# lucidrains/phenaki-pytorch

Measured on AMD Instinct MI355X. Metric: cvivit_encode_frames_per_sec, higher is better.
Workload: dtype bf16; 1 GPU; BASELINE configs[1]: C-ViViT (dim 512, patch 32, tpatch 2, depth 4+4, LFQ 65536) encode video -> token ids, (8,3,17,256,256) f32 per GPU resident in HBM; global_batch=8, parallelism=batch-shard x1, no data-path collective, hip_graph=True

## Files before the change

### include/phenaki_hip.h

```cpp
#ifndef PHENAKI_HIP_H
#define PHENAKI_HIP_H

#ifdef __cplusplus
extern "C" {
#endif

#define PK_OK 0
#define PK_EINVAL (-1)
#define PK_EALIGN (-2)
#define PK_ELAUNCH (-3)

int pk_gemm(int dtype, int a_is_f32, const void* A, int lda, const void* W, int ldw, int M, int N, int K,
            const float* bias, const float* res, int ldr, void* C, int ldc, int out_is_f32, int act,
            const int* a_rows, void* stream);

int pk_gemm_ex(int dtype, int a_is_f32, const void* A, int lda, const void* W, int ldw, int M, int N, int K,
               const float* bias, const float* res, int ldr, void* C, int ldc, int out_is_f32, int act,
               const int* a_rows, int a_nrows, int variant, void* C2, int ldc2, const float* ln_s, const float* ln_t,
               float ln_eps, const int* row_off, const int* col_off, float* stats_out, const float* ln_stats, int dup_rows,
               void* stream);
int pk_gemm_auto_variant(int dtype, int a_is_f32, int M, int N, int K, int lda, int ldw, int a_nrows);

int pk_layernorm(const float* x, int ldx, const float* gamma, const float* beta, float eps, void* out, int ldo,
                 int out_kind, float* out2, int ldo2, void* raw, int ldraw, int M, int D, int grp, int gstride,
// ... 160 lines not shown
    const float* src; void* out; long long lds, ldo; int R, K, Kp, flags, tile0, tiles_x;
} PkPackJob;
int pk_pack_multi(const void* jobs, int count, void* stream);
int pk_pack_table_prepare(void* jobs, int count);
int pk_pack_table(const void* dev_table, int count, int tiles, void* stream);
int pk_scatter_rows(const float* src, long long lds, const int* rows, float* dst, long long ldd, int M, int D, void* stream);
int pk_colsum_parts(int M);
int pk_colsum(const float* src, long long ld, int M, int N, float scale, float* out, int accumulate, float* work, void* stream);
int pk_ln_bwd_parts(int M);
int pk_layernorm_bwd(const float* x, long long ldx, const float* gamma, const float* dy, long long lddy, const float* add, long long ldadd,
                     float* dx, long long lddx, float* pg, float* pb, float eps, int M, int D, void* stream);
int pk_geglu(const float* h, long long ldh, int goff, float* out, long long ldo, int M, int F, const pk_dropout* drop, void* stream);
int pk_geglu_bwd(const float* h, long long ldh, int goff, const float* dout, long long ldd, float* dh, long long lddh, int M, int F, const pk_dropout* drop,
                 void* stream);
int pk_dropout_mask(unsigned long long seed, unsigned long long offset, int keep_thr, long long rows, int cols, unsigned char* out, void* stream);
int pk_scaled_diff(const float* a, const float* b, float scale, const float* scale_dev, float* out, long long n, void* stream);
int pk_sign(const float* z, float value, float* out, long long n, void* stream);
int pk_mul(const float* a, const float* b, float* out, long long n, void* stream);
int pk_leaky_bwd(const float* y, long long ldy, const float* dy, long long lddy, float* dz, long long lddz, int M, int N, float slope, void* stream);
int pk_peg_adjoint(const float* dy, const float* wt, float* dx, int B, int T, int H, int W, int D, int causal, void* stream);
int pk_peg_wgrad_parts(long long rows);
int pk_peg_bwd(const float* dy, const float* x, const float* wt, float* dx, float* part, int B, int T, int H, int W, int D, int causal, void* stream);
int pk_embed_bwd(const float* dy, const long long* ids, float alpha, float* dtok, float* dpos, int S, int n, int D, void* stream);
int pk_bias_gather(const float* tab, int ldt, const int* code, int off, float* out, int heads, int n, void* stream);
int pk_bias_scatter(const float* dbias, const int* code, int off, float* dtab, int ldt, int heads, int n, void* stream);
int pk_sum_batch(const float* src, long long stride, int S, float* out, long long E, void* stream);
typedef struct PkColsumJob { const float* src; float* out; long long ld; int M, N, blk0; float scale; } PkColsumJob;
int pk_colsum_multi(const void* jobs, int count, void* stream);
int pk_reduce_multi(const void* sum_jobs, int nsum, const void* col_jobs, int ncol, void* stream);
typedef struct PkSumJob { const float* src; float* out; long long stride, E4; int S, blk0; } PkSumJob;
int pk_sum_batch_multi(const void* jobs, int count, void* stream);
int pk_bce_head(const float* e, long long lde, const float* w, const float* b, const float* labels, float scale, const float* scale_dev, float* logits, float* loss_rows,
                float* de, long long ldde, float* pw, float* pb, int M, int D, void* stream);
int pk_gemm_splitk(int dtype, const void* A, int lda, const void* W, int ldw, int M, int N, int K, int splits, float* C, int ldc,
                   const float* bias, int tile, void* stream);
int pk_adamw(float* p, const float* g, float* m, float* v, float lr, float beta1, float beta2, float eps, float wd, int step, long long n, void* stream);
int pk_adamw_multi(const long long* table, int count, float lr, float beta1, float beta2, float eps, float wd, int step, void* stream);
int pk_grad_sumsq_parts(const long long* table, int count);
int pk_grad_sumsq(const long long* table, int count, float* partials, long long nparts, void* stream);
int pk_grad_clip_coef(const float* partials, long long nparts, float max_norm, float* out, void* stream);
int pk_scale_multi(const long long* table, int count, const float* coef_dev, void* stream);
int pk_adamw_multi_scaled(const long long* table, int count, float lr, float beta1, float beta2, float eps, float wd, int step,
                          const float* gscale_dev, void* stream);
int pk_ema_multi(const long long* table, int count, float weight, void* stream);
int pk_attn_train_prep(const float* q, long long ldq, const float* kv, long long ldkv, const float* null_kv, const float* q_scale, const float* k_scale,
                       float scale, float* Qh, float* Kh, float* Vh, int S, int heads, int n, int n_kv, int nnull, void* stream);
int pk_attn_train_prep_bwd(const float* q, long long ldq, const float* kv, long long ldkv, const float* null_kv, const float* q_scale, const float* k_scale,
                           float scale, const float* dQh, const float* dKh, const float* dVh, float* dq, long long lddq, float* dkv, long long lddkv,
                           float* pq, float* pk, float* dnull, int S, int heads, int n, int n_kv, int nnull, void* stream);
int pk_attn_bwd_work(int S, int heads, int n, int n_kv, int nnull);
int pk_attn_bwd_ws(const float* Qh, const float* Kh, const float* Vh, const void* O, long long ldo, int o_bf16, const float* dO, long long lddo,
                   const float* bias, const unsigned char* kmask, const float* slopes, int causal, float* dQh, float* dKh, float* dVh, float* dS,
                   float* lse, float* Drow, int S, int heads, int n, int n_kv, int nnull, int split_bf16, float* work, long long work_floats,
                   const pk_dropout* drop, void* stream);

int pk_im2col(const float* x, int B, int H, int W, int C, int kh, int kw, int stride, int pad, float* cols, long long ldc, void* stream);
int pk_col2im(const float* cols, long long ldc, int B, int H, int W, int C, int kh, int kw, int stride, int pad, float* dx, void* stream);
int pk_nchw_to_rows(const float* img, int B, int C, int H, int W, int Cp, float* rows, void* stream);
int pk_rows_to_nchw(const float* rows, int B, int C, int H, int W, int Cp, float* img, void* stream);
int pk_pick_frames(float* video, const int* frame, int B, int C, int F, int H, int W, float* img, int place, void* stream);
int pk_bmm(const float* A, long long lda, long long sA, int tA, const float* B, long long ldb, long long sB, int tB, float* C, long long ldc,
           long long sC, int batch, int M, int N, int K, int accumulate, void* stream);
int pk_row_softmax(const float* a, const float* b, const float* c, float* out, long long M, int n, int mode, void* stream);
int pk_row_l2scale(const float* x, const float* sc, const float* dz, const float* gx, const float* gsc, float* o0, float* o1, float* o2,
                   long long M, int d, int mode, void* stream);
int pk_row_ln_bwd2(const float* x, const float* gamma, const float* dy, const float* u, const float* w, float eps, float* grad_x,
                   float* grad_gamma_rows, float* grad_dy, long long M, int D, void* stream);

int pk_conv3x3(int dtype, int a_is_f32, const void* x, int B, int H, int W, int C, const void* Wm, int ldw, int Co, const float* bias, int act,
               const void* gate, int ldg, int gate_is_f32, void* y, int ldy, int out_is_f32, int tile, void* stream);
int pk_maxpool2x2(int is_f32, const void* x, int B, int H, int W, int C, void* y, void* stream);
int pk_maxpool2x2_bwd(int is_f32, const void* x, const float* dy, int B, int H, int W, int C, float* dx, void* stream);
int pk_adaptive_avgpool(int is_f32, const void* x, int B, int H, int W, int C, float* out, void* stream);
int pk_adaptive_avgpool_bwd(const float* dy, int B, int H, int W, int C, float* dx, void* stream);

int pk_frame_sqerr_parts(int H, int W);
int pk_frame_ssim_parts(int H, int W);
int pk_frame_sqerr(const float* a, const float* b, int B, int C, int F, int H, int W, float clamp_hi, float data_range, double* partials,
                   long long nparts, float* mse, float* psnr, void* stream);
int pk_frame_ssim(const float* a, const float* b, int B, int C, int F, int H, int W, float clamp_hi, float data_range, double* partials,
                  long long nparts, float* ssim, void* stream);
int pk_code_usage(const int* counts, int V, double* out, void* stream);

#ifdef __cplusplus
}
#endif
#endif
```

### phenaki_pytorch_amd/_lib.py

```python
import ctypes
import os

import torch

_HERE = os.path.dirname(os.path.abspath(__file__))
LIB_PATH = os.environ.get('PK_LIB_PATH') or os.path.join(_HERE, 'libphenaki_hip.so')

_P = ctypes.c_void_p
_I = ctypes.c_int
_F = ctypes.c_float
_L = ctypes.c_long
_LL = ctypes.c_longlong
_ULL = ctypes.c_ulonglong

SIGNATURES = {
    'pk_gemm': [_I, _I, _P, _I, _P, _I, _I, _I, _I, _P, _P, _I, _P, _I, _I, _I, _P, _P],
    'pk_gemm_ex': [_I, _I, _P, _I, _P, _I, _I, _I, _I, _P, _P, _I, _P, _I, _I, _I, _P, _I, _I, _P, _I, _P, _P, _F, _P, _P, _P, _P, _I, _P],
    'pk_gemm_auto_variant': [_I, _I, _I, _I, _I, _I, _I, _I],
    'pk_layernorm': [_P, _I, _P, _P, _F, _P, _I, _I, _P, _I, _P, _I, _I, _I, _I, _I, _I, _I, _I, _P],
    'pk_rmsnorm': [_P, _I, _P, _F, _P, _P, _I, _I, _I, _I, _P],
    'pk_gated_gelu_tanh': [_P, _I, _P, _I, _I, _I, _I, _P],
    'pk_l2norm_rows': [_P, _I, _P, _I, _I, _I, _I, _P],
    'pk_patchify_ln': [_P, _I, _I, _I, _I, _I, _I, _I, _I, _I, _I, _P, _P, _F, _P, _I, _I, _P],
    'pk_patch_embed': [_P, _I, _I, _I, _I, _I, _I, _I, _I, _F, _I,
# ... 32 lines not shown
    'pk_cpb_input': [_P, _P, _P, _I, _I, _I, _I, _I, _P],
    'pk_attn_pads': [_I, _I, _I, ctypes.POINTER(_I), ctypes.POINTER(_I)],
    'pk_attn_prep': [_I, _P, _I, _P, _I, _P, _P, _P, _F, _P, _P, _P, _I, _I, _I, _I, _I, _P],
    'pk_attn_prep_dh': [_I, _I, _P, _I, _P, _I, _P, _P, _P, _F, _P, _P, _P, _I, _I, _I, _I, _I, _P],
    'pk_qkv_project': [_I, _P, _P, _I, _P, _P, _I, _I, _I, _I, _I, _P, _P, _F, _P, _P, _P, _I, _I, _P, _P],
    'pk_qkv_attn': [_I, _P, _P, _I, _P, _P, _I, _I, _I, _I, _I, _P, _P, _F, _P, _L, _I, _P, _I, _P, _I, _P, _P],
    'pk_q_attn_cached': [_I, _P, _I, _P, _I, _I, _I, _I, _I, _P, _F, _P, _P, _P, _I, _I, _I, _P, _P, _I, _P],
    'pk_attn_fwd': [_I, _P, _P, _P, _P, _L, _I, _P, _P, _I, _P, _I, _I, _I, _I, _I, _I, _I, _P, _I, _P, _I, _I, _F, _P],
    'pk_attn_fwd_dh': [_I, _I, _P, _P, _P, _P, _L, _I, _P, _P, _I, _P, _I, _I, _I, _I, _I, _I, _I, _P, _I, _P, _I, _I, _F, _P],
    'pk_attn_fwd_lse': [_I, _P, _P, _P, _P, _L, _I, _P, _P, _I, _P, _I, _I, _I, _I, _I, _I, _I, _P, _P, _P],
    'pk_attn_fwd_lse_dh': [_I, _I, _P, _P, _P, _P, _L, _I, _P, _P, _I, _P, _I, _I, _I, _I, _I, _I, _I, _P, _P, _P],
    'pk_attn_small': [_P, _I, _P, _I, _P, _P, _F, _P, _L, _I, _P, _P, _I, _P, _I, _I, _I, _I, _I, _P],
    'pk_cfg_mix': [_P, _I, _I, _I, _I, _P, _I, _F, _I, _P, _I, _I, _I, _P],
    'pk_vocab_ntiles': [_I],
    'pk_vocab_sample_philox': [_I, _P, _I, _P, _I, _P, _I, _I, _I, _F, _P, _ULL, _ULL, ctypes.c_uint, _I, _P, _P],
    'pk_vocab_sample': [_I, _P, _I, _P, _I, _P, _I, _I, _I, _F, _P, _P, _ULL, _P, _I, _P, _P],
    'pk_vocab_reduce': [_P, _I, _I, _P, _P, _P, _P, _P, _I, _P],
    'pk_vocab_ce': [_I, _P, _I, _I, _P, _I, _P, _I, _P, _I, _P, _P, _P, _P, _P],
    'pk_vocab_eval_words': [_I],
    'pk_vocab_eval': [_I, _P, _I, _P, _I, _P, _I, _I, _I, _P, _P, _P, _P],
    'pk_vocab_eval_reduce': [_P, _I, _I, _P, _P, _P, _P, _P, _P],
    'pk_ce_grad_slab': [_I, _P, _I, _P, _P, _P, _I, _I, _I, _F, _P, _P, _I, _P, _I, _P, _P],
    'pk_topk_mask': [_P, _I, _I, _I, _LL, _P, _P, _P, _P, _P],
    'pk_critic_head': [_P, _I, _P, _P, _I, _I, _I, _I, _I, _F, _P, _F, _ULL, _P, _P, _P],
    'pk_pack': [_P, _LL, _P, _I, _I, _I, _P, _LL, _I, _I, _P],
    'pk_scatter_rows': [_P, _LL, _P, _P, _LL, _I, _I, _P],
    'pk_colsum_parts': [_I],
    'pk_colsum': [_P, _LL, _I, _I, _F, _P, _I, _P, _P],
    'pk_ln_bwd_parts': [_I],
    'pk_layernorm_bwd': [_P, _LL, _P, _P, _LL, _P, _LL, _P, _LL, _P, _P, _F, _I, _I, _P],
    'pk_geglu': [_P, _LL, _I, _P, _LL, _I, _I, _P, _P],
    'pk_geglu_bwd': [_P, _LL, _I, _P, _LL, _P, _LL, _I, _I, _P, _P],
    'pk_dropout_mask': [_ULL, _ULL, _I, _LL, _I, _P, _P],
    'pk_leaky_bwd': [_P, _LL, _P, _LL, _P, _LL, _I, _I, _F, _P],
    'pk_scaled_diff': [_P, _P, _F, _P, _P, _LL, _P],
    'pk_sign': [_P, _F, _P, _LL, _P],
    'pk_mul': [_P, _P, _P, _LL, _P],
    'pk_peg_wgrad_parts': [_LL],
    'pk_peg_bwd': [_P, _P, _P, _P, _P, _I, _I, _I, _I, _I, _I, _P],
    'pk_embed_bwd': [_P, _P, _F, _P, _P, _I, _I, _I, _P],
    'pk_bias_gather': [_P, _I, _P, _I, _P, _I, _I, _P],
    'pk_bias_scatter': [_P, _P, _I, _P, _I, _I, _I, _P],
    'pk_sum_batch': [_P, _LL, _I, _P, _LL, _P],
    'pk_sum_batch_multi': [_P, _I, _P],
    'pk_peg_adjoint': [_P, _P, _P, _I, _I, _I, _I, _I, _I, _P],
    'pk_colsum_multi': [_P, _I, _P],
    'pk_reduce_multi': [_P, _I, _P, _I, _P],
    'pk_pack_multi': [_P, _I, _P],
    'pk_pack_table_prepare': [_P, _I],
    'pk_pack_table': [_P, _I, _I, _P],
    'pk_bce_head': [_P, _LL, _P, _P, _P, _F, _P, _P, _P, _P, _LL, _P, _P, _I, _I, _P],
    'pk_attn_train_prep': [_P, _LL, _P, _LL, _P, _P, _P, _F, _P, _P, _P, _I, _I, _I, _I, _I, _P],
    'pk_attn_train_prep_bwd': [_P, _LL, _P, _LL, _P, _P, _P, _F, _P, _P, _P, _P, _LL, _P, _LL, _P, _P, _P, _I, _I, _I, _I, _I, _P],
    'pk_gemm_splitk': [_I, _P, _I, _P, _I, _I, _I, _I, _I, _P, _I, _P, _I, _P],
    'pk_adamw': [_P, _P, _P, _P, _F, _F, _F, _F, _F, _I, _LL, _P],
    'pk_adamw_multi': [_P, _I, _F, _F, _F, _F, _F, _I, _P],
    'pk_grad_sumsq_parts': [_P, _I],
    'pk_grad_sumsq': [_P, _I, _P, _LL, _P],
    'pk_grad_clip_coef': [_P, _LL, _F, _P, _P],
    'pk_scale_multi': [_P, _I, _P, _P],
    'pk_adamw_multi_scaled': [_P, _I, _F, _F, _F, _F, _F, _I, _P, _P],
    'pk_ema_multi': [_P, _I, _F, _P],
    'pk_attn_bwd_ws': [_P, _P, _P, _P, _LL, _I, _P, _LL, _P, _P, _P, _I, _P, _P, _P, _P, _P, _P, _I, _I, _I, _I, _I, _I, _P, _LL, _P, _P],
    'pk_attn_bwd_work': [_I, _I, _I, _I, _I],
    'pk_im2col': [_P, _I, _I, _I, _I, _I, _I, _I, _I, _P, _LL, _P],
    'pk_col2im': [_P, _LL, _I, _I, _I, _I, _I, _I, _I, _I, _P, _P],
    'pk_nchw_to_rows': [_P, _I, _I, _I, _I, _I, _P, _P],
    'pk_rows_to_nchw': [_P, _I, _I, _I, _I, _I, _P, _P],
    'pk_pick_frames': [_P, _P, _I, _I, _I, _I, _I, _P, _I, _P],
    'pk_bmm': [_P, _LL, _LL, _I, _P, _LL, _LL, _I, _P, _LL, _LL, _I, _I, _I, _I, _I, _P],
    'pk_row_softmax': [_P, _P, _P, _P, _LL, _I, _I, _P],
    'pk_row_l2scale': [_P, _P, _P, _P, _P, _P, _P, _P, _LL, _I, _I, _P],
    'pk_row_ln_bwd2': [_P, _P, _P, _P, _P, _F, _P, _P, _P, _LL, _I, _P],
    'pk_conv3x3': [_I, _I, _P, _I, _I, _I, _I, _P, _I, _I, _P, _I, _P, _I, _I, _P, _I, _I, _I, _P],
    'pk_maxpool2x2': [_I, _P, _I, _I, _I, _I, _P, _P],
    'pk_maxpool2x2_bwd': [_I, _P, _P, _I, _I, _I, _I, _P, _P],
    'pk_adaptive_avgpool': [_I, _P, _I, _I, _I, _I, _P, _P],
    'pk_adaptive_avgpool_bwd': [_P, _I, _I, _I, _I, _P, _P],
    'pk_frame_sqerr_parts': [_I, _I],
    'pk_frame_ssim_parts': [_I, _I],
    'pk_frame_sqerr': [_P, _P, _I, _I, _I, _I, _I, _F, _F, _P, _LL, _P, _P, _P],
    'pk_frame_ssim': [_P, _P, _I, _I, _I, _I, _I, _F, _F, _P, _LL, _P, _P],
    'pk_code_usage': [_P, _I, _P, _P],
}

_ERR = {-1: 'PK_EINVAL (bad shape/size/flag)', -2: 'PK_EALIGN (pointer/stride alignment)', -3: 'PK_ELAUNCH (HIP launch failed)'}

_lib = None


def load():
    global _lib
    if _lib is None:
        if not os.path.exists(LIB_PATH):
            raise RuntimeError(f'{LIB_PATH} is missing: run `python -m phenaki_pytorch_amd.build` '
                               '(the MI355X build has no CPU / eager fallback)')
        lib = ctypes.CDLL(LIB_PATH)
        for name, args in SIGNATURES.items():
            fn = getattr(lib, name)
            fn.argtypes = args
            fn.restype = _I
        _lib = lib
    return _lib


def _check(rc, name):
    if rc != 0:
        raise RuntimeError(f'{name} failed: {_ERR.get(rc, rc)}')


def ptr(t):
    return None if t is None else t.data_ptr()


def f32p(t, name='parameter', rows_ok=False):
    if t is None:
        return None
    if t.dtype != torch.float32 or not (t.is_contiguous() or (rows_ok and t.stride(-1) == 1)):
        raise RuntimeError(f'{name}: the MI355X kernels read this tensor as contiguous float32, got {t.dtype} '
                           f'{"contiguous" if t.is_contiguous() else "strided"} (keep the module in float32; the compute '
                           'precision is chosen with set_compute_dtype, not with .half()/.bfloat16())')
    return t.data_ptr()


def stream(t=None):
    if t is None:
        return torch.cuda.current_stream().cuda_stream
    idx = t.device.index
    cur = _current_device()
    if idx is not None and idx != cur:
        raise RuntimeError(f'operand on cuda:{idx} but the current device is cuda:{cur}: '
                           'call torch.cuda.set_device(...) first (one process per GPU)')
    return _raw_stream(cur)


_raw_stream = getattr(torch._C, '_cuda_getCurrentRawStream', None) or (lambda i: torch.cuda.current_stream(i).cuda_stream)
_current_device = getattr(torch._C, '_cuda_getDevice', None) or torch.cuda.current_device


def require_device(t, name='tensor'):
    if not t.is_cuda:
        raise RuntimeError(f'{name} is on {t.device}: the MI355X build runs on HIP devices only (no CPU fallback)')


F32, BF16, BF16X3 = 0, 1, 2
ACT_NONE, ACT_GEGLU, ACT_LEAKY, ACT_RELU = 0, 1, 2, 3


def tdtype(dtype):
    return torch.bfloat16 if dtype == BF16 else torch.float32


def split_planes(w32):
    n, k = w32.shape
    assert k % 32 == 0 and w32.dtype == torch.float32
    hi = w32.to(torch.bfloat16)
    lo = (w32 - hi.float()).to(torch.bfloat16)
    img = torch.cat((hi.view(n, k // 32, 32), lo.view(n, k // 32, 32)), dim=-1).contiguous()
    return img.view(n, 2 * k).view(torch.float32)



def gemm(dtype, A, W, M, N, K, *, C, bias=None, res=None, act=ACT_NONE, a_rows=None, lda=None, ldc=None, variant=0, C2=None, ln=None,
         scatter=None, stats_out=None, ln_stats=None, dup_rows=0):
    a_is_f32 = 1 if A.dtype == torch.float32 else 0
    out_is_f32 = 1 if C.dtype == torch.float32 else 0
    lda = A.stride(-2) if lda is None else lda
    ldc = (C.stride(-2) if scatter is None else N) if ldc is None else ldc
    ldr = res.stride(-2) if res is not None else 0
    rc = load().pk_gemm_ex(dtype, a_is_f32, ptr(A), lda, ptr(W), W.stride(0), M, N, K, f32p(bias, 'bias'), f32p(res, 'residual'), ldr,
                           ptr(C), ldc, out_is_f32, act, ptr(a_rows), A.shape[0] if a_rows is not None else M, variant,
                           ptr(C2), C2.stride(-2) if C2 is not None else 0, ptr(ln[0]) if ln else None, ptr(ln[1]) if ln else None,
                           float(ln[2]) if ln else 0., ptr(scatter[0]) if scatter else None, ptr(scatter[1]) if scatter else None,
                           ptr(stats_out) if stats_out is not None else None, ptr(ln_stats) if ln_stats is not None else None, int(dup_rows), stream(C))
    _check(rc, 'pk_gemm_ex')
    return C


def layernorm(x, gamma, beta, M, D, *, out=None, out2=None, raw=None, eps=1e-5, remap=(0, 0, 0), perm=(0, 0), ldx=None):
    tt = out if out is not None else raw
    out_kind = 1 if (tt is not None and tt.dtype == torch.bfloat16) else 0
    rc = load().pk_layernorm(f32p(x, 'x', rows_ok=True), x.stride(-2) if ldx is None else ldx, f32p(gamma, 'LayerNorm gamma'), f32p(beta, 'LayerNorm beta'), eps,
                             ptr(out), out.stride(-2) if out is not None else 0, out_kind,
                             ptr(out2), out2.stride(-2) if out2 is not None else 0,
                             ptr(raw), raw.stride(-2) if raw is not None else 0, M, D, *remap, *perm, stream(x))
    _check(rc, 'pk_layernorm')


def patchify_ln(video, f0, nt, pt, ph, pw, weight, bias, out, eps=1e-5):
    B, C, F, H, W = video.shape
    rc = load().pk_patchify_ln(f32p(video, 'video'), B, C, F, H, W, f0, nt, pt, ph, pw, f32p(weight, 'LayerNorm weight'), f32p(bias, 'LayerNorm bias'), eps,
                               ptr(out), out.stride(0), 1 if out.dtype == torch.bfloat16 else 0, stream(video))
    _check(rc, 'pk_patchify_ln')


def patch_embed(video, ph, pw, N, groups, eps=1e-5):
    B, C, F, H, W = video.shape
    flat = []
    for (Wg, s, t, out, f0, nt, pt) in groups:
        flat += [ptr(Wg), Wg.stride(0), f32p(s, 'folded s'), f32p(t, 'folded t'), ptr(out), f0, nt, pt]
    if len(groups) == 1:
        flat += [None, 0, None, None, None, 0, 0, 0]
    ldo = groups[0][3].stride(0)
    rc = load().pk_patch_embed(f32p(video, 'video'), B, C, F, H, W, ph, pw, N, eps, len(groups), *flat, ldo, stream(video))
    _check(rc, 'pk_patch_embed')


def patch_embed_slices(K):
    return load().pk_patch_embed_slices(int(K))


def patch_embed_splitk(video, ph, pw, N, groups):
    B, C, F, H, W = video.shape
    flat = []
    for (Wg, part, stats, f0, nt, pt) in groups:
        flat += [ptr(Wg), Wg.stride(0), ptr(part), ptr(stats), f0, nt, pt]
    if len(groups) == 1:
        flat += [None, 0, None, None, 0, 0, 0]
    rc = load().pk_patch_embed_splitk(f32p(video, 'video'), B, C, F, H, W, ph, pw, N, len(groups), *flat, stream(video))
    _check(rc, 'pk_patch_embed_splitk')


def patch_embed_finish(part, stats, K, s, t, eps1, gamma2, beta2, eps2, *, out2=None, out=None, remap=(0, 0, 0)):
    nslices, rows, N = part.shape
    rc = load().pk_patch_embed_finish(ptr(part), ptr(stats), nslices, rows, N, int(K), f32p(s, 'folded s'), f32p(t, 'folded t'), float(eps1),
                                      f32p(gamma2, 'LayerNorm weight'), f32p(beta2, 'LayerNorm bias'), float(eps2),
                                      ptr(out2), out2.stride(-2) if out2 is not None else 0, ptr(out), out.stride(-2) if out is not None else 0,
                                      *remap, stream(part))
    _check(rc, 'pk_patch_embed_finish')


class _PatchFinishGroup(ctypes.Structure):
    _fields_ = [('part', _P), ('stats', _P), ('nslices', _I), ('rows', _I), ('K', _I), ('s', _P), ('t', _P), ('eps1', _F), ('gamma2', _P), ('beta2', _P),
                ('eps2', _F), ('remap_in', _I), ('remap_out', _I), ('remap_off', _I)]


def patch_embed_finish_groups(groups, *, out2=None, out=None):
    arr = (_PatchFinishGroup * len(groups))()
    for d, (part, stats, K, s, t, eps1, gamma2, beta2, eps2, remap) in zip(arr, groups):
        nslices, rows, N = part.shape
        d.part, d.stats, d.nslices, d.rows, d.K = ptr(part), ptr(stats), nslices, rows, int(K)
        d.s, d.t, d.eps1 = f32p(s, 'folded s'), f32p(t, 'folded t'), float(eps1)
        d.gamma2, d.beta2, d.eps2 = f32p(gamma2, 'LayerNorm weight'), f32p(beta2, 'LayerNorm bias'), float(eps2)
# ... 850 lines not shown
```

### phenaki_pytorch_amd/csrc/common.hpp

```cpp
#pragma once
#include <hip/hip_runtime.h>
#include <stdint.h>

namespace pk {

typedef float f32x4 __attribute__((ext_vector_type(4)));
typedef float f32x2 __attribute__((ext_vector_type(2)));
typedef __bf16 bf16x8_t __attribute__((ext_vector_type(8)));
typedef unsigned short u16;
typedef u16 u16x8 __attribute__((ext_vector_type(8)));
typedef u16 u16x4 __attribute__((ext_vector_type(4)));
typedef uint32_t u32x4 __attribute__((ext_vector_type(4)));
typedef uint32_t u32x2 __attribute__((ext_vector_type(2)));

struct bf16 { u16 v; };

struct bf16x3 { float v; };
struct bf16x3p { uint32_t v; };

typedef __bf16 bf16x2_native __attribute__((ext_vector_type(2)));
__device__ __forceinline__ u16 f2bf(float f) {
    return __builtin_bit_cast(u16, (__bf16)f);
}
__device__ __forceinline__ float bf2f(u16 h) {
// ... 37 lines not shown
__device__ __forceinline__ void split8(const f32x4& a, const f32x4& b, u32x4& hi, u32x4& lo) {
    const float x[8] = {a[0], a[1], a[2], a[3], b[0], b[1], b[2], b[3]};
#pragma unroll
    for (int i = 0; i < 4; ++i) {
        const uint32_t h = pack_bf2(x[2 * i], x[2 * i + 1]);
        hi[i] = h;
        const float h0 = __builtin_bit_cast(float, h << 16), h1 = __builtin_bit_cast(float, h & 0xFFFF0000u);
        lo[i] = pack_bf2(x[2 * i] - h0, x[2 * i + 1] - h1);
    }
}

__device__ __forceinline__ void frag_load(Frag<bf16>& f, const bf16* p) {
    f.v = *reinterpret_cast<const u32x4*>(p);
}
__device__ __forceinline__ void frag_load(Frag<float>& f, const float* p) {
    f.lo = *reinterpret_cast<const f32x4*>(p);
    f.hi = *reinterpret_cast<const f32x4*>(p + 4);
}
__device__ __forceinline__ const char* split_block(const void* p, int& pos2) {
    const uintptr_t a = reinterpret_cast<uintptr_t>(p);
    pos2 = (int)(a & 127) >> 1;
    return reinterpret_cast<const char*>(a & ~(uintptr_t)127);
}
__device__ __forceinline__ void frag_load(Frag<bf16x3p>& f, const bf16x3p* p) {
    int o;
    const char* blk = split_block(p, o);
    f.hi = *reinterpret_cast<const u32x4*>(blk + o);
    f.lo = *reinterpret_cast<const u32x4*>(blk + 64 + o);
}
__device__ __forceinline__ void frag_zero(Frag<bf16x3p>& f) { f.hi = u32x4{0, 0, 0, 0}; f.lo = f.hi; }
__device__ __forceinline__ void frag_zero(Frag<bf16x3>& f) { f.hi = u32x4{0, 0, 0, 0}; f.lo = f.hi; }
__device__ __forceinline__ void frag_zero(Frag<bf16>& f) { f.v = u32x4{0, 0, 0, 0}; }
__device__ __forceinline__ void frag_zero(Frag<float>& f) { f.lo = f32x4{0, 0, 0, 0}; f.hi = f.lo; }

__device__ __forceinline__ void frag_from_f32(Frag<bf16>& f, const float (&x)[8]) {
    f.v = u32x4{pack_bf2(x[0], x[1]), pack_bf2(x[2], x[3]), pack_bf2(x[4], x[5]), pack_bf2(x[6], x[7])};
}
__device__ __forceinline__ void frag_from_f32(Frag<float>& f, const float (&x)[8]) {
    f.lo = f32x4{x[0], x[1], x[2], x[3]};
    f.hi = f32x4{x[4], x[5], x[6], x[7]};
}

__device__ __forceinline__ void frag_from_f32(Frag<bf16x3p>& f, const float (&x)[8]) {
    split8(f32x4{x[0], x[1], x[2], x[3]}, f32x4{x[4], x[5], x[6], x[7]}, f.hi, f.lo);
}
__device__ __forceinline__ void frag_from_f32(Frag<bf16x3>& f, const float (&x)[8]) {
    split8(f32x4{x[0], x[1], x[2], x[3]}, f32x4{x[4], x[5], x[6], x[7]}, f.hi, f.lo);
}

__device__ __forceinline__ void store_elem(float* p, float v) { *p = v; }
__device__ __forceinline__ void store_elem(bf16* p, float v) { p->v = f2bf(v); }
__device__ __forceinline__ float load_elem(const float* p) { return *p; }
__device__ __forceinline__ float load_elem(const bf16* p) { return bf2f(p->v); }

__device__ __forceinline__ void store_elem(bf16x3* p, float v) { p->v = v; }
__device__ __forceinline__ float load_elem(const bf16x3* p) { return p->v; }
__device__ __forceinline__ void store4(bf16x3* p, f32x4 v) { *reinterpret_cast<f32x4*>(p) = v; }
__device__ __forceinline__ void store2(bf16x3* p, float a, float b) { *reinterpret_cast<f32x2*>(p) = f32x2{a, b}; }
__device__ __forceinline__ void store4(bf16x3p* p, f32x4 v) {
    const uintptr_t a = reinterpret_cast<uintptr_t>(p);
    char* blk = reinterpret_cast<char*>(a & ~(uintptr_t)127);
    const int o = (int)(a & 127) >> 1;
    const uint32_t h0 = pack_bf2(v[0], v[1]), h1 = pack_bf2(v[2], v[3]);
    const float r0 = v[0] - __builtin_bit_cast(float, h0 << 16), r1 = v[1] - __builtin_bit_cast(float, h0 & 0xFFFF0000u);
    const float r2 = v[2] - __builtin_bit_cast(float, h1 << 16), r3 = v[3] - __builtin_bit_cast(float, h1 & 0xFFFF0000u);
    *reinterpret_cast<u32x2*>(blk + o) = u32x2{h0, h1};
    *reinterpret_cast<u32x2*>(blk + 64 + o) = u32x2{pack_bf2(r0, r1), pack_bf2(r2, r3)};
}
__device__ __forceinline__ void store_elem(bf16x3p* p, float v) {
    const uintptr_t a = reinterpret_cast<uintptr_t>(p);
    char* blk = reinterpret_cast<char*>(a & ~(uintptr_t)127);
    const int o = (int)(a & 127) >> 1;
    const u16 h = f2bf(v);
    *reinterpret_cast<u16*>(blk + o) = h;
    *reinterpret_cast<u16*>(blk + 64 + o) = f2bf(v - bf2f(h));
}
__device__ __forceinline__ void store4(float* p, f32x4 v) { *reinterpret_cast<f32x4*>(p) = v; }
__device__ __forceinline__ void store4(bf16* p, f32x4 v) {
    *reinterpret_cast<u32x2*>(p) = u32x2{pack_bf2(v[0], v[1]), pack_bf2(v[2], v[3])};
}
__device__ __forceinline__ void store2(float* p, float a, float b) { *reinterpret_cast<f32x2*>(p) = f32x2{a, b}; }
__device__ __forceinline__ void store2(bf16* p, float a, float b) { *reinterpret_cast<uint32_t*>(p) = pack_bf2(a, b); }

__device__ __forceinline__ long xcd_contiguous_block(unsigned b, unsigned nblocks_padded) {
    return (long)(b & 7u) * (nblocks_padded >> 3) + (b >> 3);
}
__host__ __device__ inline unsigned xcd_padded_grid(long nblocks) { return (unsigned)(8 * ((nblocks + 7) / 8)); }

__device__ __forceinline__ float mul_rn(float a, float b) {
#pragma clang fp contract(off)
    return a * b;
}
__device__ __forceinline__ float add_rn(float a, float b) {
#pragma clang fp contract(off)
    return a + b;
}
__device__ __forceinline__ float wave_sum(float v) {
#pragma unroll
    for (int o = 32; o > 0; o >>= 1) v += __shfl_xor(v, o, 64);
    return v;
}
__device__ __forceinline__ float wave_max(float v) {
#pragma unroll
    for (int o = 32; o > 0; o >>= 1) v = fmaxf(v, __shfl_xor(v, o, 64));
    return v;
}

__device__ __forceinline__ float gelu_erf(float x) { return 0.5f * x * (1.0f + erff(x * 0.70710678118654752440f)); }
__device__ __forceinline__ float gelu_erf_fast(float x) {
    const float z = fabsf(x) * 0.70710678118654752440f;
    const float t = __frcp_rn(fmaf(0.3275911f, z, 1.0f));
    float p = fmaf(1.061405429f, t, -1.453152027f);
    p = fmaf(p, t, 1.421413741f);
    p = fmaf(p, t, -0.284496736f);
    p = fmaf(p, t, 0.254829592f);
    const float erfz = fmaf(-p * t, __expf(-z * z), 1.0f);
    return 0.5f * x * (1.0f + copysignf(erfz, x));
}
template <typename T> __device__ __forceinline__ float gelu_for(float x);
template <> __device__ __forceinline__ float gelu_for<float>(float x) { return gelu_erf(x); }
template <> __device__ __forceinline__ float gelu_for<bf16>(float x) { return gelu_erf_fast(x); }
#ifdef PK_X3_EXACT_GELU
template <> __device__ __forceinline__ float gelu_for<bf16x3>(float x) { return gelu_erf(x); }
#else
template <> __device__ __forceinline__ float gelu_for<bf16x3>(float x) { return gelu_erf_fast(x); }
#endif

__device__ __host__ __forceinline__ uint32_t mix32(uint32_t h) {
    h ^= h >> 16; h *= 0x85ebca6bu; h ^= h >> 13; h *= 0xc2b2ae35u; h ^= h >> 16;
    return h;
}
__device__ __host__ __forceinline__ float uniform24(uint32_t seed_lo, uint32_t seed_hi, uint32_t idx_lo, uint32_t idx_hi) {
    uint32_t h = mix32(idx_lo ^ seed_lo);
    h = mix32(h + 0x9e3779b9u * (idx_hi + 1u) + seed_hi);
    return (float)(h >> 8) * (1.0f / 16777216.0f);
}

__device__ __host__ __forceinline__ void uniform24x4(uint32_t seed_lo, uint32_t seed_hi, uint32_t q_lo, uint32_t q_hi, float (&u)[4]) {
    uint32_t h = mix32(q_lo ^ seed_lo);
    h = h + 0x9e3779b9u * (q_hi + 1u) + seed_hi;
    const uint32_t w0 = mix32(h), w1 = mix32(h + 0x85EBCA77u), w2 = mix32(h + 0x0BD794EEu);
    const float k = 1.0f / 16777216.0f;
    u[0] = (float)(w0 >> 8) * k;
    u[1] = (float)(w1 >> 8) * k;
    u[2] = (float)(w2 >> 8) * k;
    u[3] = (float)(((w0 & 0xFFu) << 16) | ((w1 & 0xFFu) << 8) | (w2 & 0xFFu)) * k;
}

struct DropArgs { uint32_t k0, k1, thr; float scale; };
__device__ __host__ __forceinline__ DropArgs drop_keys(uint64_t seed, uint64_t offset, int thr, float scale) {
    DropArgs d;
    d.k0 = mix32((uint32_t)seed ^ mix32((uint32_t)offset + 0x9e3779b9u));
    d.k1 = mix32((uint32_t)(seed >> 32) + 0x85ebca6bu * ((uint32_t)(offset >> 32) + 1u) + d.k0);
    d.thr = (uint32_t)thr;
    d.scale = scale;
    return d;
}
struct pk_dropout { unsigned long long seed, offset; int keep_thr; float scale; };
inline bool drop_site_bad(const pk_dropout* d) { return d && (d->keep_thr < 1 || d->keep_thr > 256); }
inline DropArgs drop_keys(const pk_dropout& d) { return drop_keys(d.seed, d.offset, d.keep_thr, d.scale); }
template <bool DROP> struct DropParam {};
template <> struct DropParam<true> : DropArgs { __device__ __host__ DropParam(const DropArgs& d) : DropArgs(d) {} };
__device__ __host__ __forceinline__ uint32_t drop_row(const DropArgs& d, uint32_t row) { return mix32(row ^ d.k0); }
__device__ __host__ __forceinline__ uint32_t drop_word(const DropArgs& d, uint32_t rowh, uint32_t grp) { return mix32(rowh + 0x9e3779b9u * grp + d.k1); }
__device__ __host__ __forceinline__ bool drop_keep(const DropArgs& d, uint32_t word, int e) { return ((word >> (8 * e)) & 255u) >= d.thr; }

// ... 45 lines not shown
```

### phenaki_pytorch_amd/csrc/elementwise.hip

```cpp
#include "common.hpp"

namespace pk {

__global__ __launch_bounds__(256) void peg_kernel(const float* __restrict__ x, const float* __restrict__ wt,
                                                  const float* __restrict__ bias, float* __restrict__ out, bf16* __restrict__ out_t,
                                                  int B, int T, int H, int W, int D, int tfront, long total_vec) {
    const int dv = D >> 2;
    for (long idx = (long)blockIdx.x * 256 + threadIdx.x; idx < total_vec; idx += (long)gridDim.x * 256) {
        const int c = (int)(idx % dv) * 4;
        long p = idx / dv;
        const int w = (int)(p % W); p /= W;
        const int h = (int)(p % H); p /= H;
        const int t = (int)(p % T); const int b = (int)(p / T);
        f32x4 acc = *reinterpret_cast<const f32x4*>(bias + c);
        f32x4 center = f32x4{0, 0, 0, 0};
#pragma unroll
        for (int dt = 0; dt < 3; ++dt) {
            const int ts = t + dt - tfront;
            if (ts < 0 || ts >= T) continue;
#pragma unroll
            for (int dh = 0; dh < 3; ++dh) {
                const int hs = h + dh - 1;
                if (hs < 0 || hs >= H) continue;
#pragma unroll
                for (int dw = 0; dw < 3; ++dw) {
                    const int ws = w + dw - 1;
                    if (ws < 0 || ws >= W) continue;
                    const f32x4 xv = *reinterpret_cast<const f32x4*>(x + ((((size_t)b * T + ts) * H + hs) * W + ws) * D + c);
                    const f32x4 kv = *reinterpret_cast<const f32x4*>(wt + (size_t)((dt * 3 + dh) * 3 + dw) * D + c);
                    acc += xv * kv;
                    if (ts == t && hs == h && ws == w) center = xv;
                }
            }
        }
        const size_t o = ((((size_t)b * T + t) * H + h) * W + w) * D + c;
        *reinterpret_cast<f32x4*>(out + o) = acc + center;
        if (out_t) store4(out_t + o, acc + center);
    }
}

template <int WW>
__global__ __launch_bounds__(256) void peg_row_kernel(const float* __restrict__ x, const float* __restrict__ wt,
                                                      const float* __restrict__ bias, float* __restrict__ out, bf16* __restrict__ out_t,
                                                      int B, int T, int H, int D, int tfront, long total, int flip = 0) {
    const int dv = D >> 2;
    const long idx = xcd_contiguous_block(blockIdx.x, gridDim.x) * 256 + threadIdx.x;
    if (idx >= total) return;
    const int c = (int)(idx % dv) * 4;
    long p = idx / dv;
    const int h = (int)(p % H); p /= H;
    const int t = (int)(p % T); const int b = (int)(p / T);
    const f32x4 bv = bias ? *reinterpret_cast<const f32x4*>(bias + c) : f32x4{0.f, 0.f, 0.f, 0.f};
    f32x4 acc[WW];
#pragma unroll
    for (int w = 0; w < WW; ++w) acc[w] = bv;
#pragma unroll
    for (int dt = 0; dt < 3; ++dt) {
        const int ts = t + dt - tfront;
        if (ts < 0 || ts >= T) continue;
#pragma unroll
        for (int dh = 0; dh < 3; ++dh) {
            const int hs = h + dh - 1;
            if (hs < 0 || hs >= H) continue;
            const float* row = x + (((size_t)b * T + ts) * H + hs) * WW * D + c;
            f32x4 xr[WW];
#pragma unroll
            for (int w = 0; w < WW; ++w) xr[w] = *reinterpret_cast<const f32x4*>(row + (size_t)w * D);
            const int tb = (dt * 3 + dh) * 3;
            const f32x4 k0 = *reinterpret_cast<const f32x4*>(wt + (size_t)(flip ? 26 - tb : tb) * D + c);
            const f32x4 k1 = *reinterpret_cast<const f32x4*>(wt + (size_t)(flip ? 25 - tb : tb + 1) * D + c);
            const f32x4 k2 = *reinterpret_cast<const f32x4*>(wt + (size_t)(flip ? 24 - tb : tb + 2) * D + c);
#pragma unroll
            for (int w = 0; w < WW; ++w) {
                if (w > 0) acc[w] += xr[w - 1] * k0;
                acc[w] += xr[w] * k1;
                if (w + 1 < WW) acc[w] += xr[w + 1] * k2;
                if (dt == tfront && dh == 1) acc[w] += xr[w];
            }
        }
    }
    const size_t o0 = (((size_t)b * T + t) * H + h) * WW * D + c;
#pragma unroll
    for (int w = 0; w < WW; ++w) *reinterpret_cast<f32x4*>(out + o0 + (size_t)w * D) = acc[w];
    if (out_t) {
#pragma unroll
        for (int w = 0; w < WW; ++w) store4(out_t + o0 + (size_t)w * D, acc[w]);
    }
}

template <int CD>
__global__ __launch_bounds__(256) void lfq_encode_kernel(const float* __restrict__ x, int ldx, const float* __restrict__ wp,
                                                         const float* __restrict__ bp, long long* __restrict__ ids,
                                                         float* __restrict__ proj, int M, int D) {
    const int lane = threadIdx.x & 63;
    const int row = blockIdx.x * 4 + (threadIdx.x >> 6);
    if (row >= M) return;
    float part[CD];
#pragma unroll
    for (int k = 0; k < CD; ++k) part[k] = 0.f;
    const float* xr = x + (size_t)row * ldx;
    for (int c = lane * 4; c < D; c += 256) {
        const f32x4 xv = *reinterpret_cast<const f32x4*>(xr + c);
#pragma unroll
        for (int k = 0; k < CD; ++k) {
            const f32x4 wv = *reinterpret_cast<const f32x4*>(wp + (size_t)k * D + c);
            part[k] += (xv[0] * wv[0] + xv[1] * wv[1]) + (xv[2] * wv[2] + xv[3] * wv[3]);
        }
    }
    long long id = 0;
#pragma unroll
    for (int k = 0; k < CD; ++k) {
        const float v = wave_sum(part[k]) + bp[k];
        if (proj && lane == 0) proj[(size_t)row * CD + k] = v;
        id |= (long long)(v > 0.f ? 1 : 0) << (CD - 1 - k);
    }
    if (lane == 0) ids[row] = id;
}

__device__ __forceinline__ long long lfq_row_id(const long long* __restrict__ ids_prime, int n_prime, const long long* __restrict__ ids, int n, int row) {
    if (!ids_prime) return ids[row];
    const int n_tot = n_prime + n, b = row / n_tot, i = row - b * n_tot;
    return i < n_prime ? ids_prime[(size_t)b * n_prime + i] : ids[(size_t)b * n + (i - n_prime)];
}
__device__ __forceinline__ int lfq_out_row(int r, int pb, int pc) {
    if (pb <= 0) return r;
    const int c = r % pc, ab = r / pc, b = ab % pb, a = ab / pb;
    return (a * pc + c) * pb + b;
}

template <int CD>
__global__ __launch_bounds__(256) void lfq_decode_kernel(const long long* __restrict__ ids_prime, int n_prime, const long long* __restrict__ ids, int n,
                                                         const float* __restrict__ wo,
                                                         const float* __restrict__ bo, float* __restrict__ out,
                                                         int M, int D, int row_stride, int pb, int pc) {
    const int dv = D >> 2;
    const int lanes = blockDim.x;
    const int cg = threadIdx.x % dv, rl = threadIdx.x / dv;
    float w[4][CD];
    f32x4 b4 = *reinterpret_cast<const f32x4*>(bo + cg * 4);
    {
        const f32x4* src = reinterpret_cast<const f32x4*>(wo + (size_t)cg * 4 * CD);
#pragma unroll
        for (int q = 0; q < CD; ++q) {
            const f32x4 t = src[q];
#pragma unroll
            for (int r = 0; r < 4; ++r) w[(q * 4 + r) / CD][(q * 4 + r) % CD] = t[r];
        }
    }
    for (int row = blockIdx.x * (lanes / dv) + rl; row < M; row += row_stride) {
        const unsigned long long id = (unsigned long long)lfq_row_id(ids_prime, n_prime, ids, n, row);
        f32x4 acc = b4;
#pragma unroll
        for (int k = 0; k < CD; ++k) {
            const bool on = (id >> (CD - 1 - k)) & 1ull;
#pragma unroll
            for (int e = 0; e < 4; ++e) acc[e] += on ? w[e][k] : -w[e][k];
        }
        *reinterpret_cast<f32x4*>(out + (size_t)lfq_out_row(row, pb, pc) * D + cg * 4) = acc;
    }
}

__global__ __launch_bounds__(256) void lfq_decode_generic_kernel(const long long* __restrict__ ids_prime, int n_prime, const long long* __restrict__ ids, int n,
                                                                 const float* __restrict__ wo,
                                                                 const float* __restrict__ bo, float* __restrict__ out,
                                                                 int M, int D, int cd, int pb, int pc) {
    const long total = (long)M * D;
    for (long idx = (long)blockIdx.x * 256 + threadIdx.x; idx < total; idx += (long)gridDim.x * 256) {
        const int d = (int)(idx % D);
        const int row = (int)(idx / D);
        const long long id = lfq_row_id(ids_prime, n_prime, ids, n, row);
// ... 15 lines not shown
        const int c = (int)(idx % dv) * 4;
        const long r = idx / dv;
        const int i = (int)(r % n_tot);
        const int b = (int)((r / n_tot) % nb);
        const long long id = i < n_prime ? ids_prime[(size_t)b * n_prime + i] : ids[(size_t)b * n + (i - n_prime)];
        const f32x4 a = *reinterpret_cast<const f32x4*>(pos + (size_t)i * D + c);
        const f32x4 t = *reinterpret_cast<const f32x4*>(tok + (size_t)id * D + c);
        *reinterpret_cast<f32x4*>(out + (size_t)r * D + c) = a + t;
        if (out_t) store4(out_t + (size_t)r * D + c, a + t);
    }
}

__global__ __launch_bounds__(256) void cpb_input_kernel(const float* __restrict__ w0, const float* __restrict__ b0,
                                                        float* __restrict__ out, int d0, int d1, int d2, int nd, int D, long total) {
    const int n = d0 * d1 * d2;
    for (long idx = (long)blockIdx.x * 256 + threadIdx.x; idx < total; idx += (long)gridDim.x * 256) {
        const int c = (int)(idx % D);
        const long pr = idx / D;
        const int j = (int)(pr % n), i = (int)(pr / n);
        int pi[3] = {i / (d1 * d2), (i / d2) % d1, i % d2};
        int pj[3] = {j / (d1 * d2), (j / d2) % d1, j % d2};
        float acc = b0[c];
        for (int a = 0; a < nd; ++a) {
            const int q = 3 - nd + a;
            const float rel = (float)(pi[q] - pj[q]);
            const float sg = rel > 0.f ? 1.f : (rel < 0.f ? -1.f : 0.f);
            acc += w0[(size_t)c * nd + a] * (sg * logf(fabsf(rel) + 1.f));
        }
        out[idx] = acc > 0.f ? acc : 0.1f * acc;
    }
}

__global__ __launch_bounds__(256) void critic_head_kernel(const float* __restrict__ x, int ldx, const float* __restrict__ w,
                                                          const float* __restrict__ bptr, int D, int nb, int n_tot, int n_prime, int has_null,
                                                          float scale, const float* __restrict__ u, float noise_mult,
                                                          unsigned long long seed, const unsigned long long* __restrict__ seed_dev,
                                                          float* __restrict__ out) {
    const int lane = threadIdx.x & 63;
    const int n = n_tot - n_prime;
    const int r = blockIdx.x * 4 + (threadIdx.x >> 6);
    if (r >= nb * n) return;
    const int bi = r / n, i = r % n + n_prime;
    const float b = bptr ? bptr[0] : 0.f;
    auto dot = [&](const float* xr) {
        float s = 0.f;
        for (int c = lane * 4; c < D; c += 256) {
            const f32x4 xv = *reinterpret_cast<const f32x4*>(xr + c);
            const f32x4 wv = *reinterpret_cast<const f32x4*>(w + c);
            s += (xv[0] * wv[0] + xv[1] * wv[1]) + (xv[2] * wv[2] + xv[3] * wv[3]);
        }
        return wave_sum(s) + b;
    };
    float s = dot(x + ((size_t)bi * n_tot + i) * ldx);
    if (has_null) {
        const float sn = dot(x + ((size_t)(nb + bi) * n_tot + i) * ldx);
        s = sn + (s - sn) * scale;
    }
    if (u) s += noise_mult * (u[r] - 0.5f);
    else if (noise_mult != 0.f) {
        const unsigned long long sd = seed + (seed_dev ? *seed_dev : 0ull);
        s += noise_mult * (uniform24((uint32_t)sd, (uint32_t)(sd >> 32), (uint32_t)r, 0xC817u) - 0.5f);
    }
    if (lane == 0) out[r] = s;
}

template <typename TO>
__global__ __launch_bounds__(256) void gated_gelu_tanh_kernel(const float* __restrict__ h, int ldh, TO* __restrict__ out, int ldo, int M, int Fd) {
    const int fv = Fd >> 2;
    const long total = (long)M * fv;
    for (long idx = (long)blockIdx.x * 256 + threadIdx.x; idx < total; idx += (long)gridDim.x * 256) {
        const int c = (int)(idx % fv) * 4;
        const long m = idx / fv;
        const f32x4 a = *reinterpret_cast<const f32x4*>(h + m * ldh + c), b = *reinterpret_cast<const f32x4*>(h + m * ldh + Fd + c);
        f32x4 y;
#pragma unroll
        for (int r = 0; r < 4; ++r) {
            const float x = a[r];
            y[r] = 0.5f * x * (1.0f + tanhf(0.7978845608028654f * (x + 0.044715f * x * x * x))) * b[r];
        }
        store4(out + m * ldo + c, y);
    }
}

}
using namespace pk;

static inline int nblocks(long total) { long b = (total + 255) / 256; return (int)(b < 16384 ? (b > 0 ? b : 1) : 16384); }
#define STREAM(s) reinterpret_cast<hipStream_t>(s)

extern "C" int pk_peg(const float* x, const float* wt, const float* bias, float* out, void* out_t, int B, int T, int H, int W, int D,
                      int causal, void* stream) {
    if (!x || !wt || !bias || !out || B <= 0 || T <= 0 || H <= 0 || W <= 0 || D <= 0) return PK_EINVAL;
    if (D & 3) return PK_EALIGN;
    if (x == out) return PK_EINVAL;
    const long total = (long)B * T * H * W * (D >> 2);
    const long rows = (long)B * T * H * (D >> 2);
    const dim3 rgrid(xcd_padded_grid((rows + 255) / 256));
    bf16* ot = reinterpret_cast<bf16*>(out_t);
    if (ot && (reinterpret_cast<uintptr_t>(ot) & 7)) return PK_EALIGN;
    if (W == 8) hipLaunchKernelGGL((peg_row_kernel<8>), rgrid, dim3(256), 0, STREAM(stream), x, wt, bias, out, ot, B, T, H, D, causal ? 2 : 1, rows);
    else if (W == 4) hipLaunchKernelGGL((peg_row_kernel<4>), rgrid, dim3(256), 0, STREAM(stream), x, wt, bias, out, ot, B, T, H, D, causal ? 2 : 1, rows);
    else if (W == 16) hipLaunchKernelGGL((peg_row_kernel<16>), rgrid, dim3(256), 0, STREAM(stream), x, wt, bias, out, ot, B, T, H, D, causal ? 2 : 1, rows);
    else hipLaunchKernelGGL(peg_kernel, dim3(nblocks(total)), dim3(256), 0, STREAM(stream), x, wt, bias, out, ot, B, T, H, W, D, causal ? 2 : 1, total);
    PK_CHECK_LAUNCH();
    return PK_OK;
}

extern "C" int pk_peg_adjoint(const float* dy, const float* wt, float* dx, int B, int T, int H, int W, int D, int causal, void* stream) {
    if (!dy || !wt || !dx || B <= 0 || T <= 0 || H <= 0 || D <= 0 || dy == dx) return PK_EINVAL;
    if (D & 3) return PK_EALIGN;
    const long rows = (long)B * T * H * (D >> 2);
    const dim3 rgrid(xcd_padded_grid((rows + 255) / 256));
    const int tf = 2 - (causal ? 2 : 1);
    if (W == 8) hipLaunchKernelGGL((peg_row_kernel<8>), rgrid, dim3(256), 0, STREAM(stream), dy, wt, nullptr, dx, nullptr, B, T, H, D, tf, rows, 1);
    else if (W == 4) hipLaunchKernelGGL((peg_row_kernel<4>), rgrid, dim3(256), 0, STREAM(stream), dy, wt, nullptr, dx, nullptr, B, T, H, D, tf, rows, 1);
    else if (W == 16) hipLaunchKernelGGL((peg_row_kernel<16>), rgrid, dim3(256), 0, STREAM(stream), dy, wt, nullptr, dx, nullptr, B, T, H, D, tf, rows, 1);
    else return PK_EINVAL;
    PK_CHECK_LAUNCH();
    return PK_OK;
}

extern "C" int pk_lfq_encode(const float* x, int ldx, const float* wp, const float* bp, long long* ids, float* proj,
                             int M, int D, int cd, void* stream) {
    if (!x || !wp || !bp || !ids || M <= 0 || D <= 0) return PK_EINVAL;
    if ((D & 3) || (ldx & 3)) return PK_EALIGN;
    dim3 grid((M + 3) / 4), block(256);
    hipStream_t s = STREAM(stream);
    switch (cd) {
#define PK_CASE(N) case N: hipLaunchKernelGGL((lfq_encode_kernel<N>), grid, block, 0, s, x, ldx, wp, bp, ids, proj, M, D); break;
        PK_CASE(4) PK_CASE(6) PK_CASE(8) PK_CASE(10) PK_CASE(12) PK_CASE(13) PK_CASE(14) PK_CASE(16) PK_CASE(18)
#undef PK_CASE
        default: return PK_EINVAL;
    }
    PK_CHECK_LAUNCH();
    return PK_OK;
}

extern "C" int pk_lfq_decode(const long long* ids, const float* wo, const float* bo, float* out, int M, int D, int cd,
                             const long long* ids_prime, int n_prime, int n, int pb, int pc, void* stream) {
    if (!ids || !wo || !bo || !out || M <= 0 || D <= 0 || cd <= 0 || cd > 62) return PK_EINVAL;
    if (ids_prime && (n_prime <= 0 || n <= 0 || M % (n_prime + n))) return PK_EINVAL;
    if (!ids_prime) { n_prime = 0; n = 0; }
    if ((pb > 0) != (pc > 0) || (pb > 0 && M % (pb * pc))) return PK_EINVAL;
    hipStream_t s = STREAM(stream);
    const int dv = D >> 2;
    const bool fast = (D & 3) == 0 && dv <= 256 && (256 % dv == 0 || dv == 256) && (cd == 8 || cd == 16) &&
                      (reinterpret_cast<uintptr_t>(out) & 15) == 0 && (reinterpret_cast<uintptr_t>(bo) & 15) == 0 &&
                      (reinterpret_cast<uintptr_t>(wo) & 15) == 0;
    if (fast) {
        const int rpb = 256 / dv;
        int blocks = (M + rpb - 1) / rpb;
        if (blocks > 512) blocks = 512;
        if (cd == 16) hipLaunchKernelGGL((lfq_decode_kernel<16>), dim3(blocks), dim3(256), 0, s, ids_prime, n_prime, ids, n, wo, bo, out, M, D, blocks * rpb, pb, pc);
        else hipLaunchKernelGGL((lfq_decode_kernel<8>), dim3(blocks), dim3(256), 0, s, ids_prime, n_prime, ids, n, wo, bo, out, M, D, blocks * rpb, pb, pc);
    } else {
        hipLaunchKernelGGL(lfq_decode_generic_kernel, dim3(nblocks((long)M * D)), dim3(256), 0, s, ids_prime, n_prime, ids, n, wo, bo, out, M, D, cd, pb, pc);
    }
    PK_CHECK_LAUNCH();
    return PK_OK;
}

extern "C" int pk_embed(const long long* ids_prime, int n_prime, const long long* ids, int n, int nb, const float* tok,
                        const float* pos, float* out, void* out_t, int S, int D, void* stream) {
    if (!ids || !tok || !pos || !out || S <= 0 || n <= 0 || nb <= 0 || D <= 0 || n_prime < 0 || (n_prime > 0 && !ids_prime)) return PK_EINVAL;
    if (D & 3) return PK_EALIGN;
    const long total = (long)S * (n_prime + n) * (D >> 2);
    hipLaunchKernelGGL(embed_kernel, dim3(nblocks(total)), dim3(256), 0, STREAM(stream), ids_prime, n_prime, ids, n, nb, tok, pos, out, reinterpret_cast<bf16*>(out_t), D, total);
    PK_CHECK_LAUNCH();
    return PK_OK;
}

extern "C" int pk_cpb_input(const float* w0, const float* b0, float* out, int d0, int d1, int d2, int nd, int D, void* stream) {
    if (!w0 || !b0 || !out || d0 <= 0 || d1 <= 0 || d2 <= 0 || nd < 1 || nd > 3 || D <= 0) return PK_EINVAL;
    const long n = (long)d0 * d1 * d2;
    const long total = n * n * D;
    hipLaunchKernelGGL(cpb_input_kernel, dim3(nblocks(total)), dim3(256), 0, STREAM(stream), w0, b0, out, d0, d1, d2, nd, D, total);
    PK_CHECK_LAUNCH();
    return PK_OK;
}

extern "C" int pk_critic_head(const float* x, int ldx, const float* w, const float* b, int D, int nb, int n_tot, int n_prime,
                              int has_null, float scale, const float* u, float noise_mult, unsigned long long seed,
                              const unsigned long long* seed_dev, float* out, void* stream) {
    if (!x || !w || !out || D <= 0 || nb <= 0 || n_tot <= n_prime || n_prime < 0) return PK_EINVAL;
    if ((D & 3) || (ldx & 3)) return PK_EALIGN;
// ... 17 lines not shown
```

### phenaki_pytorch_amd/csrc/gemm.hip

```cpp
#include "gemm_dma.hpp"
#include "gemm_p8.hpp"

namespace pk {

enum { ACT_NONE = 0, ACT_GEGLU = 1, ACT_LEAKY = 2, ACT_RELU = 3 };

struct GemmEpilogue {
    const float* bias;
    const float* res;
    void* C;
    int ldr, ldc;
    int out_f32;
    int act;
    int vec_ok;
    void* C2;
    int ldc2;
    const float* ln_s; const float* ln_t; float ln_eps;
    const int* row_off; const int* col_off;
    float* stats_out; const float* ln_stats; int stats_np;
    int dup_rows;
};

constexpr int STATS_CHUNK = 32;

template <typename T, int TM, int TN, int WN>
__device__ __forceinline__ void gemm_epilogue_scalar(const f32x4 (&acc)[TM][TN], int M, int N, const GemmEpilogue& e, int m0, int n0) {
    const int lane = threadIdx.x & 63, wave = threadIdx.x >> 6;
    const int wm = wave / WN, wn = wave % WN, g = lane >> 4, lr = lane & 15;
    float* Cf = reinterpret_cast<float*>(e.C);
    T* Ct = reinterpret_cast<T*>(e.C);
#pragma unroll
    for (int i = 0; i < TM; ++i) {
        const int m = m0 + wm * 16 * TM + i * 16 + lr;
        if (m >= M) continue;
#pragma unroll
        for (int j = 0; j < TN; ++j) {
            const int n = n0 + wn * 16 * TN + j * 16 + g * 4;
            const f32x4 v = acc[i][j];
#pragma unroll
            for (int r = 0; r < 4; ++r) {
                const int nn = n + r;
                if (nn >= N) break;
                float x = v[r] + (e.bias ? e.bias[nn] : 0.f);
                if (e.act == ACT_GEGLU) {
                    if (r & 1) continue;
                    const float gate = (nn + 1 < N) ? v[r + 1] + (e.bias ? e.bias[nn + 1] : 0.f) : 0.f;
                    x = gelu_for<T>(gate) * x;
                    const size_t o = (size_t)m * e.ldc + (nn >> 1);
                    if (e.out_f32) Cf[o] = x; else store_elem(Ct + o, x);
                    continue;
                }
                if (e.act == ACT_LEAKY) x = x > 0.f ? x : 0.1f * x;
                if (e.act == ACT_RELU) x = fmaxf(x, 0.f);
                if (e.res) x += e.res[(size_t)m * e.ldr + nn];
                const size_t o = (size_t)m * e.ldc + nn;
                if (e.out_f32) Cf[o] = x; else store_elem(Ct + o, x);
            }
        }
    }
}

template <int TM> constexpr int epi_rows_per_round() { return TM > 2 ? 2 : TM; }

template <typename T, int TM, int TN, int WN = 2, bool LNF = false>
__device__ __forceinline__ void gemm_epilogue(const f32x4 (&acc)[TM][TN], int M, int N, const GemmEpilogue& e, int m0, int n0,
                                              const float* rsum = nullptr, const float* rsq = nullptr, int K = 1) {
    if (!e.vec_ok) {
        if (!LNF) gemm_epilogue_scalar<T, TM, TN, WN>(acc, M, N, e, m0, n0);
        return;
    }
    const int lane = threadIdx.x & 63, wave = threadIdx.x >> 6;
    const int wm = wave / WN, wn = wave % WN, g = lane >> 4, lr = lane & 15;
    float* __restrict__ Cf = reinterpret_cast<float*>(e.C);
    T* __restrict__ Ct = reinterpret_cast<T*>(e.C);
    const int mb = m0 + wm * 16 * TM + lr, nb = n0 + wn * 16 * TN + g * 4;
    f32x4 b4[TN], s4[TN], t4[TN];
    int coff[TN];
#pragma unroll
    for (int j = 0; j < TN; ++j) {
        const int nj = min(nb + j * 16, N - 4);
        b4[j] = e.bias ? *reinterpret_cast<const f32x4*>(e.bias + nj) : f32x4{0, 0, 0, 0};
        if (LNF) {
            s4[j] = *reinterpret_cast<const f32x4*>(e.ln_s + nj);
            t4[j] = *reinterpret_cast<const f32x4*>(e.ln_t + nj);
        }
        coff[j] = e.row_off ? e.col_off[nj] : nj;
    }
    constexpr int IB = epi_rows_per_round<TM>();
#pragma unroll
    for (int i0 = 0; i0 < TM; i0 += IB) {
        f32x4 r4[IB][TN];
        int roff[IB];
#pragma unroll
        for (int ii = 0; ii < IB; ++ii) {
            const int mi = min(mb + (i0 + ii) * 16, M - 1);
            roff[ii] = e.row_off ? e.row_off[mi] : 0;
            if (!LNF && e.res && e.act != ACT_GEGLU) {
#pragma unroll
                for (int j = 0; j < TN; ++j) r4[ii][j] = *reinterpret_cast<const f32x4*>(e.res + (size_t)mi * e.ldr + min(nb + j * 16, N - 4));
            } else {
#pragma unroll
                for (int j = 0; j < TN; ++j) r4[ii][j] = f32x4{0, 0, 0, 0};
            }
        }
#pragma unroll
        for (int ii = 0; ii < IB; ++ii) {
            const int i = i0 + ii, m = mb + i * 16;
            float mean = 0.f, rstd = 1.f;
            if (LNF) {
                const float inv_k = 1.0f / (float)K;
                mean = rsum[i] * inv_k;
                rstd = __builtin_amdgcn_rsqf(fmaxf(rsq[i] * inv_k - mean * mean, 0.f) + e.ln_eps);
            }
            float ps = 0.f, pq = 0.f;
#pragma unroll
            for (int j = 0; j < TN; ++j) {
                const int n = nb + j * 16;
                const bool live = m < M && n < N;
                f32x4 v = acc[i][j];
                if (LNF) {
#pragma unroll
                    for (int r = 0; r < 4; ++r) v[r] = rstd * (v[r] - mean * s4[j][r]) + t4[j][r];
                }
                v += b4[j];
                if (e.act == ACT_GEGLU) {
                    const float o0 = gelu_for<T>(v[1]) * v[0], o1 = gelu_for<T>(v[3]) * v[2];
                    const size_t o = (size_t)m * e.ldc + (n >> 1);
                    if (live) { if (e.out_f32) store2(Cf + o, o0, o1); else store2(Ct + o, o0, o1); }
                    continue;
                }
                if (e.act == ACT_LEAKY) {
#pragma unroll
                    for (int r = 0; r < 4; ++r) v[r] = v[r] > 0.f ? v[r] : 0.1f * v[r];
                }
                if (e.act == ACT_RELU) {
#pragma unroll
                    for (int r = 0; r < 4; ++r) v[r] = fmaxf(v[r], 0.f);
                }
                if (!LNF) v += r4[ii][j];
                else if (e.res && live) v += *reinterpret_cast<const f32x4*>(e.res + (size_t)m * e.ldr + n);
                if (live) {
                    const size_t o = e.row_off ? (size_t)((long)roff[ii] + (long)coff[j]) : (size_t)m * e.ldc + n;
                    if (e.out_f32) store4(Cf + o, v); else store4(Ct + o, v);
                    if (e.C2) store4(reinterpret_cast<bf16*>(e.C2) + (size_t)m * e.ldc2 + n, v);
                    if (e.dup_rows) {
                        const size_t od = o + (size_t)e.dup_rows * e.ldc;
                        if (e.out_f32) store4(Cf + od, v); else store4(Ct + od, v);
                        if (e.C2) store4(reinterpret_cast<bf16*>(e.C2) + (size_t)(m + e.dup_rows) * e.ldc2 + n, v);
                    }
                    if (TN == 2 && e.stats_out) {
#pragma unroll
                        for (int r = 0; r < 4; ++r) {
                            const float x = (sizeof(T) == 2 && (e.C2 || !e.out_f32)) ? bf2f(f2bf(v[r])) : v[r];
                            ps += x; pq += x * x;
                        }
                    }
                }
            }
            if (TN == 2 && e.stats_out) {
                ps += __shfl_xor(ps, 16); pq += __shfl_xor(pq, 16);
                ps += __shfl_xor(ps, 32); pq += __shfl_xor(pq, 32);
                const int chunk = (n0 + wn * 16 * TN) / STATS_CHUNK;
                if (g == 0 && m < M && chunk < e.stats_np)
                    reinterpret_cast<float2*>(e.stats_out)[(size_t)m * e.stats_np + chunk] = float2{ps, pq};
            }
        }
    }
}

template <typename T, typename TA, int TM, int TN>
__global__ __launch_bounds__(256) void gemm_kernel(const GemmOperands p, const GemmEpilogue e) {
    using Tile = GemmTile<T, TA, TM, TN>;
    extern __shared__ __attribute__((aligned(16))) char smem[];
    const int m0 = blockIdx.x * Tile::BM, n0 = blockIdx.y * Tile::BN;
    f32x4 acc[TM][TN];
#pragma unroll
    for (int i = 0; i < TM; ++i)
#pragma unroll
        for (int j = 0; j < TN; ++j) acc[i][j] = f32x4{0, 0, 0, 0};
    Tile::run(p, m0, n0, smem, acc);
    gemm_epilogue<T, TM, TN>(acc, p.M, p.N, e, m0, n0);
}

template <typename Tile>
constexpr int lds_waves_per_simd() {
    const int wgs = 163840 / Tile::SMEM, w = wgs * (Tile::THREADS / 64) / 4;
    return w < 1 ? 1 : (w > 8 ? 8 : w);
}

template <typename T, int TM, int TN, int WM, int WN, int STAGES, int ROWB, int PW, int LNF = 0>
__global__ __launch_bounds__(64 * (WM * WN + PW))
__attribute__((amdgpu_waves_per_eu(lds_waves_per_simd<GemmDma<T, TM, TN, WM, WN, STAGES, ROWB, PW>>(), 8)))
void gemm_dma_kernel(const GemmOperands p, const GemmEpilogue e, int a_nrows) {
    using Tile = GemmDma<T, TM, TN, WM, WN, STAGES, ROWB, PW>;
    extern __shared__ __attribute__((aligned(16))) char smem[];
    const int MT = (p.M + Tile::BM - 1) / Tile::BM, cmax = (MT + 7) / 8, NTn = (p.N + Tile::BN - 1) / Tile::BN;
    const int xcd = blockIdx.x & 7, idx = blockIdx.x >> 3;
    const int mstart = xcd * MT / 8, mcount = (xcd + 1) * MT / 8 - mstart;
    int m0, n0;
    if (p.plain_map) {
        if ((int)blockIdx.x >= MT * NTn) return;
        m0 = (blockIdx.x % MT) * Tile::BM;
        n0 = (blockIdx.x / MT) * Tile::BN;
    } else {
        int ml, ntile;
        if (!xcd_panel_tile(idx, cmax, mcount, NTn, p.panel, ml, ntile)) return;
        m0 = (mstart + ml) * Tile::BM;
        n0 = ntile * Tile::BN;
    }
    PK_TL_KERNEL(0);
    f32x4 acc[TM][TN];
#pragma unroll
    for (int i = 0; i < TM; ++i)
#pragma unroll
        for (int j = 0; j < TN; ++j) acc[i][j] = f32x4{0, 0, 0, 0};
    if constexpr (LNF == 1) {
        float rsum[TM], rsq[TM];
        if (!Tile::template run_stats<2>(p, a_nrows, m0, n0, smem, acc, rsum, rsq)) return;
        gemm_epilogue<T, TM, TN, WN, true>(acc, p.M, p.N, e, m0, n0, rsum, rsq, p.K);
    } else if constexpr (LNF == 2) {
        constexpr int TPR = Tile::THREADS / Tile::BM;
        static_assert(Tile::THREADS == TPR * Tile::BM && (TPR == 2 || TPR == 4), "2 or 4 threads per tile row");
        constexpr int NPRE = 16 / TPR;
        const int srow = threadIdx.x / TPR, sq4 = threadIdx.x % TPR;
        const int per = (e.stats_np + TPR - 1) / TPR, c0 = sq4 * per, c1 = min(c0 + per, e.stats_np);
        const float2* st = reinterpret_cast<const float2*>(e.ln_stats) + (size_t)min(m0 + srow, p.M - 1) * e.stats_np;
        float su = 0.f, sq = 0.f;
        for (int c = c0 + NPRE; c < c1; ++c) { const float2 pr = st[c]; su += pr.x; sq += pr.y; }
        float2 pre[NPRE];
#pragma unroll
        for (int u = 0; u < NPRE; ++u) pre[u] = c0 + u < c1 ? st[c0 + u] : float2{0.f, 0.f};
        if (!Tile::run(p, a_nrows, m0, n0, smem, acc)) return;
#pragma unroll
        for (int u = 0; u < NPRE; ++u) { su += pre[u].x; sq += pre[u].y; }
        su += __shfl_xor(su, 1); sq += __shfl_xor(sq, 1);
        if (TPR == 4) { su += __shfl_xor(su, 2); sq += __shfl_xor(sq, 2); }
        __syncthreads();
        float2* ls = reinterpret_cast<float2*>(smem);
        if (sq4 == 0) ls[srow] = float2{su, sq};
        __syncthreads();
        float rsum[TM], rsq[TM];
        const int lane = threadIdx.x & 63, wm = (threadIdx.x >> 6) / WN;
#pragma unroll
        for (int i = 0; i < TM; ++i) { const float2 pr = ls[wm * 16 * TM + i * 16 + (lane & 15)]; rsum[i] = pr.x; rsq[i] = pr.y; }
        gemm_epilogue<T, TM, TN, WN, true>(acc, p.M, p.N, e, m0, n0, rsum, rsq, p.K);
    } else {
        if (!Tile::run(p, a_nrows, m0, n0, smem, acc)) return;
        PK_TL_KERNEL(1);
        gemm_epilogue<T, TM, TN, WN>(acc, p.M, p.N, e, m0, n0);
        asm volatile("s_waitcnt vmcnt(0)" ::: "memory");
        PK_TL_KERNEL(2);
    }
}

template <typename T, int TM, int TN, int WM, int WN, int STAGES>
__global__ __launch_bounds__(64 * WM * WN)
__attribute__((amdgpu_waves_per_eu(lds_waves_per_simd<GemmDma<T, TM, TN, WM, WN, STAGES, 128, 0>>(), 8)))
void gemm_dma_splitk_kernel(GemmOperands p, GemmEpilogue e, int a_nrows, long batch_a, long batch_w, long batch_c) {
    using Tile = GemmDma<T, TM, TN, WM, WN, STAGES, 128, 0>;
    extern __shared__ __attribute__((aligned(16))) char smem[];
    const int z = blockIdx.y;
    p.A = reinterpret_cast<const char*>(p.A) + (size_t)z * batch_a;
    p.W = reinterpret_cast<const char*>(p.W) + (size_t)z * batch_w;
    e.C = reinterpret_cast<char*>(e.C) + (size_t)z * batch_c;
    if (z != 0) e.bias = nullptr;
    const int MT = (p.M + Tile::BM - 1) / Tile::BM, NTn = (p.N + Tile::BN - 1) / Tile::BN;
    if ((int)blockIdx.x >= MT * NTn) return;
    const int m0 = (blockIdx.x % MT) * Tile::BM, n0 = (blockIdx.x / MT) * Tile::BN;
    f32x4 acc[TM][TN];
#pragma unroll
    for (int i = 0; i < TM; ++i)
#pragma unroll
        for (int j = 0; j < TN; ++j) acc[i][j] = f32x4{0, 0, 0, 0};
    if (!Tile::run(p, a_nrows, m0, n0, smem, acc)) return;
    gemm_epilogue<T, TM, TN, WN>(acc, p.M, p.N, e, m0, n0);
}

template <typename T, int TM = 2, int TN = 2>
static int launch_splitk(const GemmOperands& p, const GemmEpilogue& e, int a_nrows, int splits, long ba, long bw, long bc, hipStream_t s) {
    using Tile = GemmDma<T, TM, TN, 2, 2, 2, 128, 0>;
    constexpr int lds = Tile::SMEM;
    const int MT = (p.M + Tile::BM - 1) / Tile::BM, NT = (p.N + Tile::BN - 1) / Tile::BN;
    hipLaunchKernelGGL((gemm_dma_splitk_kernel<T, TM, TN, 2, 2, 2>), dim3(MT * NT, splits), dim3(Tile::THREADS), lds, s, p, e, a_nrows, ba, bw, bc);
    PK_CHECK_LAUNCH();
    return PK_OK;
}

template <typename T, typename TA, int TM, int TN>
static int launch_v1(const GemmOperands& p, const GemmEpilogue& e, hipStream_t s) {
    using Tile = GemmTile<T, TA, TM, TN>;
    dim3 grid((p.M + Tile::BM - 1) / Tile::BM, (p.N + Tile::BN - 1) / Tile::BN);
    hipLaunchKernelGGL((gemm_kernel<T, TA, TM, TN>), grid, dim3(256), Tile::SMEM, s, p, e);
    PK_CHECK_LAUNCH();
    return PK_OK;
}

template <typename T, int TM, int TN, int STAGES, int WM = 2, int WN = 2, int ROWB = 128, int PW = 0, int LNF = 0>
static int launch_dma(const GemmOperands& p, const GemmEpilogue& e, int a_nrows, hipStream_t s) {
    using Tile = GemmDma<T, TM, TN, WM, WN, STAGES, ROWB, PW>;
    if (Tile::SMEM > 65536) {
        static LdsOptIn lds;
        if (lds.raise(reinterpret_cast<const void*>(&gemm_dma_kernel<T, TM, TN, WM, WN, STAGES, ROWB, PW, LNF>), Tile::SMEM) != PK_OK) return PK_ELAUNCH;
    }
    const int MT = (p.M + Tile::BM - 1) / Tile::BM, NT = (p.N + Tile::BN - 1) / Tile::BN;
    dim3 grid(8 * ((MT + 7) / 8) * NT);
    GemmOperands pp = p;
    static const int panel_env = [] { const char* e_ = getenv("PK_GEMM_PANEL"); return e_ ? atoi(e_) : -1; }();
    pp.panel = panel_env >= 0 ? panel_env : xcd_panel_rows(Tile::BM, p.K, (int)sizeof(T));
    hipLaunchKernelGGL((gemm_dma_kernel<T, TM, TN, WM, WN, STAGES, ROWB, PW, LNF>), grid, dim3(Tile::THREADS), Tile::SMEM, s, pp, e, a_nrows);
    PK_CHECK_LAUNCH();
    return PK_OK;
}

__global__ __launch_bounds__(512) __attribute__((amdgpu_waves_per_eu(2, 2)))
void gemm_p8_kernel(const GemmOperands p, const GemmEpilogue e, int a_nrows) {
    using Tile = GemmP8;
    extern __shared__ __attribute__((aligned(16))) char smem[];
    const int MT = (p.M + Tile::BM - 1) / Tile::BM, cmax = (MT + 7) / 8, NTn = (p.N + Tile::BN - 1) / Tile::BN;
    const int xcd = blockIdx.x & 7, idx = blockIdx.x >> 3;
    const int mstart = xcd * MT / 8, mcount = (xcd + 1) * MT / 8 - mstart;
    int m0, n0;
    if (p.plain_map) {
        if ((int)blockIdx.x >= MT * NTn) return;
        m0 = (blockIdx.x % MT) * Tile::BM;
        n0 = (blockIdx.x / MT) * Tile::BN;
    } else {
        int ml, ntile;
        if (!xcd_panel_tile(idx, cmax, mcount, NTn, p.panel, ml, ntile)) return;
        m0 = (mstart + ml) * Tile::BM;
        n0 = ntile * Tile::BN;
    }
    Tile::Acc acc;
#pragma unroll
// ... 36 lines not shown
    if (z != 0) e.bias = nullptr;
    const int MT = (p.M + Tile::BM - 1) / Tile::BM, NTn = (p.N + Tile::BN - 1) / Tile::BN;
    if ((int)blockIdx.x >= MT * NTn) return;
    const int m0 = (blockIdx.x % MT) * Tile::BM, n0 = (blockIdx.x / MT) * Tile::BN;
    Tile::Acc acc;
#pragma unroll
    for (int a = 0; a < 2; ++a)
#pragma unroll
        for (int b = 0; b < 2; ++b)
#pragma unroll
            for (int i = 0; i < 4; ++i)
#pragma unroll
                for (int j = 0; j < 2; ++j) acc[a][b][i][j] = f32x4{0, 0, 0, 0};
    Tile::run(p, a_nrows, m0, n0, smem, acc);
    gemm_epilogue<bf16, 4, 2, 4>(acc[0][0], p.M, p.N, e, m0, n0);
    gemm_epilogue<bf16, 4, 2, 4>(acc[0][1], p.M, p.N, e, m0, n0 + 128);
    gemm_epilogue<bf16, 4, 2, 4>(acc[1][0], p.M, p.N, e, m0 + 128, n0);
    gemm_epilogue<bf16, 4, 2, 4>(acc[1][1], p.M, p.N, e, m0 + 128, n0 + 128);
}

static int launch_p8_splitk(const GemmOperands& p, const GemmEpilogue& e, int a_nrows, int splits, long ba, long bw, long bc, hipStream_t s) {
    using Tile = GemmP8;
    static LdsOptIn lds;
    if (lds.raise(reinterpret_cast<const void*>(&gemm_p8_splitk_kernel), Tile::SMEM) != PK_OK) return PK_ELAUNCH;
    const int MT = (p.M + Tile::BM - 1) / Tile::BM, NT = (p.N + Tile::BN - 1) / Tile::BN;
    hipLaunchKernelGGL(gemm_p8_splitk_kernel, dim3(MT * NT, splits), dim3(Tile::THREADS), Tile::SMEM, s, p, e, a_nrows, ba, bw, bc);
    PK_CHECK_LAUNCH();
    return PK_OK;
}

}

using namespace pk;

static inline bool al16(const void* p) { return (reinterpret_cast<uintptr_t>(p) & 15) == 0; }

static bool dma_possible(int dtype, int a_is_f32, int N, int K, int lda, int ldw, int a_nrows) {
    const int bk = dtype == 1 ? 64 : 32;
    const int kpad = (K + bk - 1) / bk * bk;
    const size_t el = dtype == 1 ? 2 : 4;
    return !(dtype == 1 && a_is_f32) && ldw >= kpad &&
           (size_t)a_nrows * lda * el < 0xFFFFFFF0ull && (size_t)N * ldw * el < 0xFFFFFFF0ull;
}

static int auto_variant(int dtype, int a_is_f32, int M, int N, int K, int lda, int ldw, int a_nrows) {
    const long blocks128 = (long)((M + 127) / 128) * ((N + 127) / 128);
    if (!dma_possible(dtype, a_is_f32, N, K, lda, ldw, a_nrows)) return blocks128 >= 384 ? 2 : 1;
    static const long t128 = getenv("PK_GEMM_T128") ? atol(getenv("PK_GEMM_T128")) : 256;
    if (dtype != 0 && blocks128 >= t128 && blocks128 < 384 && K <= 1024) return 27;
    if (dtype == 1 && K >= 2048 && (long)((M + 255) / 256) * ((N + 255) / 256) >= 512) return 50;
    if (blocks128 >= t128) return dtype == 2 ? 9 : 24;
    if (K >= 2048) return dtype == 1 ? 33 : 3;
    return 8;
}

extern "C" int pk_gemm_auto_variant(int dtype, int a_is_f32, int M, int N, int K, int lda, int ldw, int a_nrows) {
    return auto_variant(dtype, a_is_f32, M, N, K, lda, ldw, a_nrows);
}

extern "C" int pk_gemm_ex(int dtype, int a_is_f32, const void* A, int lda, const void* W, int ldw,
                          int M, int N, int K, const float* bias, const float* res, int ldr,
                          void* C, int ldc, int out_is_f32, int act, const int* a_rows, int a_nrows,
                          int variant, void* C2, int ldc2, const float* ln_s, const float* ln_t, float ln_eps,
                          const int* row_off, const int* col_off, float* stats_out, const float* ln_stats, int dup_rows, void* stream) {
    if (M <= 0 || N <= 0 || K <= 0 || !A || !W || !C) return PK_EINVAL;
    if (dtype != 0 && dtype != 1 && dtype != 2) return PK_EINVAL;
    if (act < 0 || act > 3) return PK_EINVAL;
    const int eps_w = dtype == 1 ? 8 : 4;
    const int eps_a = (dtype == 1 && !a_is_f32) ? 8 : 4;
    if (K % eps_w || ldw % eps_w || lda % eps_a) return PK_EALIGN;
    if (dtype == 1 && a_is_f32 && (K % 8)) return PK_EALIGN;
    if (!al16(A) || !al16(W)) return PK_EALIGN;
    if (dtype != 1 && !a_is_f32) return PK_EINVAL;
    if (dtype == 2 && C2) return PK_EINVAL;
    if (act == ACT_GEGLU && (N & 1)) return PK_EINVAL;
    if (a_rows && a_nrows <= 0) return PK_EINVAL;
    if (!a_rows) a_nrows = M;
    GemmOperands p{A, W, a_rows, lda, ldw, M, N, K, 0, N >= 8192 ? krot_default() : 0};
    GemmEpilogue e{bias, res, C, ldr, ldc, out_is_f32, act, 0, C2, ldc2, ln_s, ln_t, ln_eps, row_off, col_off, stats_out, ln_stats,
                   ((ln_stats ? K : N) + STATS_CHUNK - 1) / STATS_CHUNK, dup_rows};
    bool v = (N % 4 == 0) && (ldc % 4 == 0) && al16(C) && (!bias || al16(bias)) && (!res || (al16(res) && ldr % 4 == 0));
    if (act == ACT_GEGLU) v = v && (ldc % 2 == 0) && ((reinterpret_cast<uintptr_t>(C) & 7) == 0);
    e.vec_ok = v ? 1 : 0;
    if (C2 && (!v || !out_is_f32 || act == ACT_GEGLU || dtype != 1 || (ldc2 & 3) || (reinterpret_cast<uintptr_t>(C2) & 7))) return PK_EINVAL;
    if ((ln_s == nullptr) != (ln_t == nullptr)) return PK_EINVAL;
    if ((row_off == nullptr) != (col_off == nullptr)) return PK_EINVAL;
    if (row_off && (!v || !out_is_f32 || act == ACT_GEGLU || res || C2)) return PK_EINVAL;
    if (ln_stats && (!ln_s || stats_out || (reinterpret_cast<uintptr_t>(ln_stats) & 7))) return PK_EINVAL;
    if (stats_out && (!v || act == ACT_GEGLU || row_off || (reinterpret_cast<uintptr_t>(stats_out) & 7))) return PK_EINVAL;
    if (dup_rows < 0 || (dup_rows && (!v || act == ACT_GEGLU || row_off || stats_out || dup_rows < M))) return PK_EINVAL;
    hipStream_t s = reinterpret_cast<hipStream_t>(stream);

    const bool dma_ok = dma_possible(dtype, a_is_f32, N, K, lda, ldw, a_nrows);
    if (variant >= 100) { p.plain_map = 1; variant -= 100; }
    if (variant == 0) variant = auto_variant(dtype, a_is_f32, M, N, K, lda, ldw, a_nrows);
    if (variant >= 3 && !dma_ok) return PK_EINVAL;
    if (ln_s) {
        if (!dma_ok || !v || !al16(ln_s) || !al16(ln_t) || a_rows) return PK_EINVAL;
        const bool big = variant == 24 || variant == 2 || variant == 9 || variant == 50;
        if (ln_stats) {
            if (dtype == 1) return big ? launch_dma<bf16, 4, 2, 2, 2, 4, 128, 0, 2>(p, e, a_nrows, s) : launch_dma<bf16, 2, 2, 2, 2, 2, 128, 0, 2>(p, e, a_nrows, s);
            if (dtype == 2) return big ? launch_dma<bf16x3, 4, 4, 2, 2, 2, 128, 0, 2>(p, e, a_nrows, s) : launch_dma<bf16x3, 2, 2, 2, 2, 2, 128, 0, 2>(p, e, a_nrows, s);
            return big ? launch_dma<float, 4, 2, 2, 2, 4, 128, 0, 2>(p, e, a_nrows, s) : launch_dma<float, 2, 2, 2, 2, 2, 128, 0, 2>(p, e, a_nrows, s);
        }
        if (dtype == 1) return big ? launch_dma<bf16, 4, 2, 2, 2, 4, 128, 0, 1>(p, e, a_nrows, s) : launch_dma<bf16, 2, 2, 2, 2, 2, 128, 0, 1>(p, e, a_nrows, s);
        if (dtype == 2) return big ? launch_dma<bf16x3, 4, 4, 2, 2, 2, 128, 0, 1>(p, e, a_nrows, s) : launch_dma<bf16x3, 2, 2, 2, 2, 2, 128, 0, 1>(p, e, a_nrows, s);
        return big ? launch_dma<float, 4, 2, 2, 2, 4, 128, 0, 1>(p, e, a_nrows, s) : launch_dma<float, 2, 2, 2, 2, 2, 128, 0, 1>(p, e, a_nrows, s);
    }
    if (stats_out && !(dma_ok && (variant == 8 || variant == 24 || variant == 27 || variant == 33 || variant == 50 || (variant == 3 && dtype != 1)))) return PK_EINVAL;
    if (dtype == 1) {
        switch (variant) {
            case 1: return a_is_f32 ? launch_v1<bf16, float, 2, 2>(p, e, s) : launch_v1<bf16, bf16, 2, 2>(p, e, s);
            case 2: return a_is_f32 ? launch_v1<bf16, float, 4, 4>(p, e, s) : launch_v1<bf16, bf16, 4, 4>(p, e, s);
            case 8: return launch_dma<bf16, 2, 2, 2>(p, e, a_nrows, s);
            case 9: return launch_dma<bf16, 4, 4, 2>(p, e, a_nrows, s);
            case 24: return launch_dma<bf16, 4, 2, 2, 2, 4>(p, e, a_nrows, s);
            case 33: return launch_dma<bf16, 2, 2, 3, 2, 2, 128, 2>(p, e, a_nrows, s);
            case 27: return launch_dma<bf16, 4, 2, 2, 2, 2>(p, e, a_nrows, s);
            case 50: return launch_p8(p, e, a_nrows, s);
            default: return PK_EINVAL;
        }
    }
    if (dtype == 2) {
        if (!dma_ok) return PK_EINVAL;
        switch (variant) {
            case 3: return launch_dma<bf16x3, 2, 2, 4>(p, e, a_nrows, s);
            case 8: return launch_dma<bf16x3, 2, 2, 2>(p, e, a_nrows, s);
            case 9: return launch_dma<bf16x3, 4, 4, 2>(p, e, a_nrows, s);
            case 24: return launch_dma<bf16x3, 4, 2, 2, 2, 4>(p, e, a_nrows, s);
            case 27: return launch_dma<bf16x3, 4, 2, 2, 2, 2>(p, e, a_nrows, s);
            default: return PK_EINVAL;
        }
    }
    switch (variant) {
        case 1: return launch_v1<float, float, 2, 2>(p, e, s);
        case 2: return launch_v1<float, float, 4, 4>(p, e, s);
        case 3: return launch_dma<float, 2, 2, 4>(p, e, a_nrows, s);
        case 8: return launch_dma<float, 2, 2, 2>(p, e, a_nrows, s);
        case 9: return launch_dma<float, 4, 4, 2>(p, e, a_nrows, s);
        case 24: return launch_dma<float, 4, 2, 2, 2, 4>(p, e, a_nrows, s);
        default: return PK_EINVAL;
    }
}

#ifdef PK_TIMELINE
extern "C" int pk_debug_timeline(unsigned long long* out, int n) {
    if (hipDeviceSynchronize() != hipSuccess) return PK_ELAUNCH;
    return hipMemcpyFromSymbol(out, HIP_SYMBOL(pk_tl), sizeof(unsigned long long) * n) == hipSuccess ? PK_OK : PK_ELAUNCH;
}
extern "C" int pk_debug_timeline_clear() {
    static unsigned long long z[8 * 5 * 40] = {};
    return hipMemcpyToSymbol(HIP_SYMBOL(pk_tl), z, sizeof(z)) == hipSuccess ? PK_OK : PK_ELAUNCH;
}
#endif

extern "C" int pk_gemm(int dtype, int a_is_f32, const void* A, int lda, const void* W, int ldw,
                       int M, int N, int K, const float* bias, const float* res, int ldr,
                       void* C, int ldc, int out_is_f32, int act, const int* a_rows, void* stream) {
    if (a_rows) {
        const long blocks128 = (long)((M + 127) / 128) * ((N + 127) / 128);
        return pk_gemm_ex(dtype, a_is_f32, A, lda, W, ldw, M, N, K, bias, res, ldr, C, ldc, out_is_f32, act, a_rows,
                          0x7fffffff / (lda > 0 ? lda : 1) / 4, blocks128 >= 384 ? 2 : 1, nullptr, 0, nullptr, nullptr, 0.f, nullptr, nullptr, nullptr, nullptr, 0, stream);
    }
    return pk_gemm_ex(dtype, a_is_f32, A, lda, W, ldw, M, N, K, bias, res, ldr, C, ldc, out_is_f32, act, nullptr, M, 0,
                      nullptr, 0, nullptr, nullptr, 0.f, nullptr, nullptr, nullptr, nullptr, 0, stream);
}
// ... 25 lines not shown
```

### phenaki_pytorch_amd/csrc/norm.hip

```cpp
#include "common.hpp"

namespace pk {

struct LnArgs {
    const float* x; int ldx;
    const float* gamma; const float* beta; float eps;
    void* out; int ldo;
    float* out2; int ldo2;
    void* raw; int ldraw;
    int M, D;
    int grp, gstride, goff;
    int pb, pc;
};

template <typename TO, int VMAX>
__global__ __launch_bounds__(256) void ln_rows_kernel(const LnArgs p) {
    const int lane = threadIdx.x & 63;
    const int row = blockIdx.x * 4 + (threadIdx.x >> 6);
    if (row >= p.M) return;
    int orow = row;
    if (p.grp > 0) orow = (row / p.grp) * p.gstride + p.goff + row % p.grp;
    else if (p.pb > 0) {
        const int c = row % p.pc, b = (row / p.pc) % p.pb, a = row / (p.pc * p.pb);
        orow = (a * p.pc + c) * p.pb + b;
    }
    const float* xr = p.x + (size_t)row * p.ldx;
    TO* out = reinterpret_cast<TO*>(p.out);
    TO* raw = reinterpret_cast<TO*>(p.raw);
    const int nv = p.D >> 2;
    constexpr bool HOIST = VMAX <= 2;
    constexpr int NH = HOIST ? VMAX : 1;
    f32x4 v[VMAX], gm[NH], bt[NH];
    float s = 0.f;
#pragma unroll
    for (int i = 0; i < VMAX; ++i) {
        const int c = lane + i * 64;
        if (c < nv) {
            v[i] = *reinterpret_cast<const f32x4*>(xr + c * 4);
            if constexpr (HOIST) {
                gm[i] = *reinterpret_cast<const f32x4*>(p.gamma + c * 4);
                bt[i] = p.beta ? *reinterpret_cast<const f32x4*>(p.beta + c * 4) : f32x4{0, 0, 0, 0};
            }
        }
    }
#pragma unroll
    for (int i = 0; i < VMAX; ++i)
        if (lane + i * 64 < nv) s += (v[i][0] + v[i][1]) + (v[i][2] + v[i][3]);
    const float mean = wave_sum(s) / (float)p.D;
    float q = 0.f;
#pragma unroll
    for (int i = 0; i < VMAX; ++i) {
        const int c = lane + i * 64;
        if (c < nv) {
#pragma unroll
            for (int r = 0; r < 4; ++r) { const float d = v[i][r] - mean; q += d * d; }
        }
    }
    const float rstd = 1.0f / sqrtf(wave_sum(q) / (float)p.D + p.eps);
#pragma unroll
    for (int i = 0; i < VMAX; ++i) {
        const int c = lane + i * 64;
        if (c < nv) {
            f32x4 g4, b4;
            if constexpr (HOIST) { g4 = gm[i]; b4 = bt[i]; }
            else {
                g4 = *reinterpret_cast<const f32x4*>(p.gamma + c * 4);
                b4 = p.beta ? *reinterpret_cast<const f32x4*>(p.beta + c * 4) : f32x4{0, 0, 0, 0};
            }
            f32x4 y;
#pragma unroll
            for (int r = 0; r < 4; ++r) y[r] = (v[i][r] - mean) * rstd * g4[r] + b4[r];
            if (out) store4(out + (size_t)orow * p.ldo + c * 4, y);
            if (p.out2) store4(p.out2 + (size_t)orow * p.ldo2 + c * 4, y);
            if (raw) store4(raw + (size_t)orow * p.ldraw + c * 4, v[i]);
        }
    }
}

template <int VMAX, int R>
__global__ __launch_bounds__(256) void ln_lfq_kernel(const LnArgs p, const float* __restrict__ wp, const float* __restrict__ bp,
                                                      int cd, long long* __restrict__ ids, float* __restrict__ proj) {
    const int lane = threadIdx.x & 63;
    const int row0 = (blockIdx.x * 4 + (threadIdx.x >> 6)) * R;
    if (row0 >= p.M) return;
    const int nv = p.D >> 2;
    f32x4 y[R][VMAX];
    float mean[R], rstd[R];
#pragma unroll
    for (int r = 0; r < R; ++r) {
        const int row = row0 + r < p.M ? row0 + r : p.M - 1;
        const float* xr = p.x + (size_t)row * p.ldx;
#pragma unroll
        for (int i = 0; i < VMAX; ++i) {
            const int c = lane + i * 64;
            y[r][i] = c < nv ? *reinterpret_cast<const f32x4*>(xr + c * 4) : f32x4{0, 0, 0, 0};
        }
    }
#pragma unroll
    for (int r = 0; r < R; ++r) {
        float s = 0.f;
#pragma unroll
        for (int i = 0; i < VMAX; ++i) s += (y[r][i][0] + y[r][i][1]) + (y[r][i][2] + y[r][i][3]);
        mean[r] = wave_sum(s) / (float)p.D;
        float q = 0.f;
#pragma unroll
        for (int i = 0; i < VMAX; ++i)
            if (lane + i * 64 < nv) {
#pragma unroll
                for (int e = 0; e < 4; ++e) { const float d = y[r][i][e] - mean[r]; q += d * d; }
            }
        rstd[r] = 1.0f / sqrtf(wave_sum(q) / (float)p.D + p.eps);
    }
#pragma unroll
    for (int i = 0; i < VMAX; ++i) {
        const int c = lane + i * 64;
        if (c < nv) {
            const f32x4 g4 = *reinterpret_cast<const f32x4*>(p.gamma + c * 4);
            const f32x4 b4 = p.beta ? *reinterpret_cast<const f32x4*>(p.beta + c * 4) : f32x4{0, 0, 0, 0};
#pragma unroll
            for (int r = 0; r < R; ++r)
#pragma unroll
                for (int e = 0; e < 4; ++e) y[r][i][e] = (y[r][i][e] - mean[r]) * rstd[r] * g4[e] + b4[e];
        } else {
#pragma unroll
            for (int r = 0; r < R; ++r) y[r][i] = f32x4{0, 0, 0, 0};
        }
    }
    float part[R][16];
#pragma unroll
    for (int r = 0; r < R; ++r)
#pragma unroll
        for (int k = 0; k < 16; ++k) part[r][k] = 0.f;
#pragma unroll
    for (int k = 0; k < 16; ++k) {
        if (k < cd) {
#pragma unroll
            for (int i = 0; i < VMAX; ++i) {
                const int c = lane + i * 64;
                const f32x4 wv = c < nv ? *reinterpret_cast<const f32x4*>(wp + (size_t)k * p.D + c * 4) : f32x4{0, 0, 0, 0};
#pragma unroll
                for (int r = 0; r < R; ++r)
                    part[r][k] += (y[r][i][0] * wv[0] + y[r][i][1] * wv[1]) + (y[r][i][2] * wv[2] + y[r][i][3] * wv[3]);
            }
        }
    }
#pragma unroll
    for (int r = 0; r < R; ++r) {
        const int row = row0 + r;
        if (row >= p.M) break;
        int orow = row;
        if (p.pb > 0) {
            const int c = row % p.pc, b = (row / p.pc) % p.pb, a = row / (p.pc * p.pb);
            orow = (a * p.pc + c) * p.pb + b;
        }
        if (p.out2) {
#pragma unroll
            for (int i = 0; i < VMAX; ++i)
                if (lane + i * 64 < nv) store4(p.out2 + (size_t)orow * p.ldo2 + (lane + i * 64) * 4, y[r][i]);
        }
        float h8[8], h4[4], h2[2], h1;
        {
            const bool hi = lane & 32;
#pragma unroll
            for (int i = 0; i < 8; ++i) {
                const float keep = hi ? part[r][i + 8] : part[r][i], send = hi ? part[r][i] : part[r][i + 8];
                h8[i] = keep + __shfl_xor(send, 32, 64);
            }
        }
        {
            const bool hi = lane & 16;
#pragma unroll
            for (int i = 0; i < 4; ++i) {
                const float keep = hi ? h8[i + 4] : h8[i], send = hi ? h8[i] : h8[i + 4];
                h4[i] = keep + __shfl_xor(send, 16, 64);
            }
        }
        {
            const bool hi = lane & 8;
#pragma unroll
            for (int i = 0; i < 2; ++i) {
                const float keep = hi ? h4[i + 2] : h4[i], send = hi ? h4[i] : h4[i + 2];
                h2[i] = keep + __shfl_xor(send, 8, 64);
            }
        }
        {
            const bool hi = lane & 4;
            const float keep = hi ? h2[1] : h2[0], send = hi ? h2[0] : h2[1];
            h1 = keep + __shfl_xor(send, 4, 64);
        }
        h1 += __shfl_xor(h1, 2, 64);
        h1 += __shfl_xor(h1, 1, 64);
        const int k = lane >> 2;
        const float val = h1 + (k < cd ? bp[k] : 0.f);
        if (proj && k < cd && (lane & 3) == 0) proj[(size_t)orow * cd + k] = val;
        const unsigned long long bal = __ballot(val > 0.f);
        if (lane == 0) {
            long long id = 0;
            for (int kk = 0; kk < cd; ++kk) id |= (long long)((bal >> (4 * kk)) & 1ull) << (cd - 1 - kk);
            ids[orow] = id;
        }
    }
}

template <typename TO>
__global__ __launch_bounds__(256) void l2norm_rows_kernel(const float* __restrict__ x, int ldx, TO* __restrict__ out, int ldo, int M, int D) {
    const int lane = threadIdx.x & 63;
    const int row = blockIdx.x * 4 + (threadIdx.x >> 6);
    if (row >= M) return;
    const float* xr = x + (size_t)row * ldx;
    float ss = 0.f;
    for (int c = lane * 4; c < D; c += 256) {
        const f32x4 v = *reinterpret_cast<const f32x4*>(xr + c);
        ss += (v[0] * v[0] + v[1] * v[1]) + (v[2] * v[2] + v[3] * v[3]);
    }
    const float inv = 1.0f / fmaxf(sqrtf(wave_sum(ss)), 1e-12f);
    for (int c = lane * 4; c < D; c += 256) {
        const f32x4 v = *reinterpret_cast<const f32x4*>(xr + c);
        store4(out + (size_t)row * ldo + c, v * inv);
    }
}

template <typename TO>
__global__ __launch_bounds__(256) void rmsnorm_rows_kernel(const float* __restrict__ x, int ldx, const float* __restrict__ w, float eps,
                                                           const unsigned char* __restrict__ rowmask, TO* __restrict__ out, int ldo, int M, int D) {
    const int lane = threadIdx.x & 63;
    const int row = blockIdx.x * 4 + (threadIdx.x >> 6);
    if (row >= M) return;
    const float* xr = x + (size_t)row * ldx;
    const bool keep = !rowmask || rowmask[row] != 0;
    float q = 0.f;
    for (int c = lane * 4; c < D; c += 256) {
        const f32x4 v = *reinterpret_cast<const f32x4*>(xr + c);
        q += (v[0] * v[0] + v[1] * v[1]) + (v[2] * v[2] + v[3] * v[3]);
    }
    const float rstd = 1.0f / sqrtf(wave_sum(q) / (float)D + eps);
    for (int c = lane * 4; c < D; c += 256) {
        const f32x4 v = *reinterpret_cast<const f32x4*>(xr + c), g = *reinterpret_cast<const f32x4*>(w + c);
        f32x4 y;
#pragma unroll
        for (int r = 0; r < 4; ++r) y[r] = keep ? v[r] * rstd * g[r] : 0.f;
        store4(out + (size_t)row * ldo + c, y);
    }
}

}
using namespace pk;

extern "C" int pk_rmsnorm(const float* x, int ldx, const float* w, float eps, const unsigned char* rowmask, void* out, int ldo,
                          int out_kind, int M, int D, void* stream) {
    if (!x || !w || !out || M <= 0 || D <= 0) return PK_EINVAL;
    if ((D & 3) || (ldx & 3) || (ldo & 3) || (reinterpret_cast<uintptr_t>(x) & 15) || (reinterpret_cast<uintptr_t>(w) & 15)) return PK_EALIGN;
    hipStream_t s = reinterpret_cast<hipStream_t>(stream);
    dim3 grid((M + 3) / 4), block(256);
    if (out_kind == 0) hipLaunchKernelGGL((rmsnorm_rows_kernel<float>), grid, block, 0, s, x, ldx, w, eps, rowmask, (float*)out, ldo, M, D);
    else hipLaunchKernelGGL((rmsnorm_rows_kernel<bf16>), grid, block, 0, s, x, ldx, w, eps, rowmask, (bf16*)out, ldo, M, D);
    PK_CHECK_LAUNCH();
    return PK_OK;
}

extern "C" int pk_l2norm_rows(const float* x, int ldx, void* out, int ldo, int out_kind, int M, int D, void* stream) {
    if (!x || !out || M <= 0 || D <= 0) return PK_EINVAL;
    if ((D & 3) || (ldx & 3) || (ldo & 3)) return PK_EALIGN;
    hipStream_t s = reinterpret_cast<hipStream_t>(stream);
    dim3 grid((M + 3) / 4), block(256);
    if (out_kind == 0) hipLaunchKernelGGL((l2norm_rows_kernel<float>), grid, block, 0, s, x, ldx, (float*)out, ldo, M, D);
    else hipLaunchKernelGGL((l2norm_rows_kernel<bf16>), grid, block, 0, s, x, ldx, (bf16*)out, ldo, M, D);
    PK_CHECK_LAUNCH();
    return PK_OK;
}


extern "C" int pk_layernorm_lfq(const float* x, int ldx, const float* gamma, const float* beta, float eps, const float* wp,
                                const float* bp, long long* ids, float* tokens, int ldt, float* proj, int M, int D, int cd,
                                int pb, int pc, void* stream) {
    if (M <= 0 || D <= 0 || !x || !gamma || !wp || !bp || !ids || cd <= 0 || cd > 16) return PK_EINVAL;
    if ((D & 3) || (ldx & 3) || (tokens && (ldt & 3))) return PK_EALIGN;
    if (D > 64 * 4 * 8) return PK_EINVAL;
    if (pb > 0 && (pc <= 0 || M % (pb * pc))) return PK_EINVAL;
    LnArgs p{x, ldx, gamma, beta, eps, nullptr, 0, tokens, ldt, nullptr, 0, M, D, 0, 0, 0, pb, pc};
    hipStream_t s = reinterpret_cast<hipStream_t>(stream);
    dim3 block(256);
    if (D <= 64 * 4 * 2 && M >= 32768) hipLaunchKernelGGL((ln_lfq_kernel<2, 2>), dim3((M + 7) / 8), block, 0, s, p, wp, bp, cd, ids, proj);
    else if (D <= 64 * 4 * 2) hipLaunchKernelGGL((ln_lfq_kernel<2, 1>), dim3((M + 3) / 4), block, 0, s, p, wp, bp, cd, ids, proj);
    else hipLaunchKernelGGL((ln_lfq_kernel<8, 1>), dim3((M + 3) / 4), block, 0, s, p, wp, bp, cd, ids, proj);
    PK_CHECK_LAUNCH();
    return PK_OK;
}

extern "C" int pk_layernorm(const float* x, int ldx, const float* gamma, const float* beta, float eps,
                            void* out, int ldo, int out_kind, float* out2, int ldo2, void* raw, int ldraw,
                            int M, int D, int grp, int gstride, int goff, int pb, int pc, void* stream) {
    if (M <= 0 || D <= 0 || !x || !gamma || (!out && !out2)) return PK_EINVAL;
    if ((D & 3) || (ldx & 3) || (out && (ldo & 3)) || (out2 && (ldo2 & 3)) || (raw && (ldraw & 3))) return PK_EALIGN;
    if (D > 64 * 4 * 8) return PK_EINVAL;
    if (pb > 0 && (pc <= 0 || M % (pb * pc))) return PK_EINVAL;
    if (grp > 0 && pb > 0) return PK_EINVAL;
    LnArgs p{x, ldx, gamma, beta, eps, out, ldo, out2, ldo2, raw, ldraw, M, D, grp, gstride, goff, pb, pc};
    hipStream_t s = reinterpret_cast<hipStream_t>(stream);
    dim3 grid((M + 3) / 4), block(256);
    const bool small = D <= 64 * 4 * 2;
    if (out_kind == 0) {
        if (small) hipLaunchKernelGGL((ln_rows_kernel<float, 2>), grid, block, 0, s, p);
        else hipLaunchKernelGGL((ln_rows_kernel<float, 8>), grid, block, 0, s, p);
    } else {
        if (small) hipLaunchKernelGGL((ln_rows_kernel<bf16, 2>), grid, block, 0, s, p);
        else hipLaunchKernelGGL((ln_rows_kernel<bf16, 8>), grid, block, 0, s, p);
    }
    PK_CHECK_LAUNCH();
    return PK_OK;
}
```

### phenaki_pytorch_amd/csrc/patch_embed.hip

```cpp
#include <cstdlib>
#include "gemm_dma.hpp"

extern "C" {
typedef struct {
    const float* part; const float* stats; int nslices, rows, K;
    const float* s; const float* t; float eps1;
    const float* gamma2; const float* beta2; float eps2;
    int remap_in, remap_out, remap_off;
} pk_patch_finish_group;
}

namespace pk {

struct PatchGroup {
    const void* W;
    const float* s;
    const float* t;
    float* out;
    int ldw, K;
    int f0, nt, pt;
    int rows;
    int mtiles;
};

struct PatchEmbedArgs {
    const float* video;
    int B, C, F, H, W, ph, pw, nh, nw;
    int N, ldo;
    float eps;
    uint32_t video_bytes;
    int ngroups;
    int rot_mult;
    PatchGroup g[2];
};

constexpr int PE_BM = 128, PE_WAVES = 8, PE_ASTAGE = PE_BM * 128, PE_WRING = 4;
template <int TN> struct PeGeom {
    static constexpr int BN = 32 * TN, WSTAGE = BN * 128, IW = BN / 64, SMEM = 2 * PE_ASTAGE + PE_WRING * WSTAGE, WAITN = 2 * (IW + 4);
};

typedef __attribute__((address_space(3))) void* pe_lds_ptr;

__device__ __forceinline__ void pe_load16(f32x4& dst, uint32_t voff, const u32x4& rsrc, uint32_t soff) {
    asm volatile("buffer_load_dwordx4 %0, %1, %2, %3 offen" : "=v"(dst) : "v"(voff), "s"(rsrc), "s"(soff) : "memory");
}
template <int N>
__device__ __forceinline__ void pe_wait(f32x4 (&r)[4]) {
    asm volatile("s_waitcnt vmcnt(%[cnt])" : "+v"(r[0]), "+v"(r[1]), "+v"(r[2]), "+v"(r[3]) : [cnt] "n"(N) : "memory");
}

template <int TN>
__device__ __forceinline__ void patch_embed_body(const PatchEmbedArgs& a, char* smem) {
    constexpr int PE_BN = PeGeom<TN>::BN, PE_WSTAGE = PeGeom<TN>::WSTAGE, IW = PeGeom<TN>::IW, WAITN = PeGeom<TN>::WAITN;
    const int tid = threadIdx.x, lane = tid & 63;
    const int wave = __builtin_amdgcn_readfirstlane(tid >> 6);
    const int NT = (a.N + PE_BN - 1) / PE_BN;
    const int MT = a.g[0].mtiles + (a.ngroups > 1 ? a.g[1].mtiles : 0), cmax = (MT + 7) / 8;
    const int xcd = blockIdx.x & 7, idx = blockIdx.x >> 3;
    const int mstart = xcd * MT / 8, mcount = (xcd + 1) * MT / 8 - mstart;
    const int ml = idx % cmax;
    if (ml >= mcount) return;
    int mt = mstart + ml;
    const int n0 = (idx / cmax) * PE_BN;
    const int gi = (a.ngroups > 1 && mt >= a.g[0].mtiles) ? 1 : 0;
    if (gi) mt -= a.g[0].mtiles;
    const PatchGroup& G = a.g[gi];
    const int m0 = mt * PE_BM;
    const int K = G.K, nt = K >> 6;
    const int rot = (mt * a.rot_mult) % nt;

    const int o = lane >> 3, p = lane & 7;
    const int rr = ((o & 1) << 2) | (o >> 1);
    const int pw = a.pw;
    const int dline = pw < 32 ? (p * 4) / pw : 0, xin = pw < 32 ? (p * 4) % pw : p * 4;
    const int per_b = G.nt * a.nh * a.nw;
    uint32_t rowoff[2];
    float cen[2];
#pragma unroll
    for (int hrow = 0; hrow < 2; ++hrow) {
        const int r = m0 + wave * 16 + hrow * 8 + rr;
        const bool ok = r < G.rows;
        const int rc = ok ? r : 0;
        const int b = rc / per_b, rem = rc - b * per_b;
        const int tt = rem / (a.nh * a.nw), hw = rem - tt * (a.nh * a.nw);
        const int hh = hw / a.nw, ww = hw - hh * a.nw;
        const uint32_t org = (((uint32_t)(b * a.C) * a.F + (G.f0 + tt * G.pt)) * a.H + hh * a.ph) * a.W + ww * a.pw;
        const f32x4 c4 = *reinterpret_cast<const f32x4*>(a.video + org + (uint32_t)dline * a.W + xin);
        float cs = (c4[0] + c4[1]) + (c4[2] + c4[3]);
#pragma unroll
        for (int off = 1; off < 8; off <<= 1) cs += __shfl_xor(cs, off, 64);
        cen[hrow] = ok ? cs * (1.0f / 32.0f) : 0.f;
        rowoff[hrow] = ok ? (org + (uint32_t)dline * a.W + xin) * 4u : a.video_bytes;
    }
    const uintptr_t vb = reinterpret_cast<uintptr_t>(a.video);
    const u32x4 rsrc = u32x4{(uint32_t)vb, (uint32_t)(vb >> 32) & 0xFFFFu, a.video_bytes, 0x00020000u};

    const int lph = pw < 32 ? 32 / pw : 1;
    int hx0, hy, hdt, hcc;
    {
        const int e0 = rot * 64, line0 = e0 / pw;
        hx0 = e0 - line0 * pw;
        hy = line0 % a.ph;
        const int r2 = line0 / a.ph;
        hdt = r2 % G.pt; hcc = r2 / G.pt;
    }
    auto next_soff = [&]() {
        const uint32_t so = ((((uint32_t)hcc * a.F + hdt) * a.H + hy) * a.W + hx0) * 4u;
        hx0 += 32;
        if (hx0 >= pw) {
            hx0 = 0; hy += lph;
            if (hy >= a.ph) { hy = 0; if (++hdt == G.pt) { hdt = 0; if (++hcc == a.C) hcc = 0; } }
        }
        return so;
    };
    auto issue_a = [&](f32x4 (&r)[4]) {
#pragma unroll
        for (int half = 0; half < 2; ++half) {
            const uint32_t so = next_soff();
            pe_load16(r[half * 2 + 0], rowoff[0], rsrc, so);
            pe_load16(r[half * 2 + 1], rowoff[1], rsrc, so);
        }
    };

    char* const wring = smem + 2 * PE_ASTAGE;
    const int lrow = lane >> 3, lslot = lane & 7;
    const uint32_t bytesW = (uint32_t)a.N * (uint32_t)G.ldw * 2u;
    __amdgpu_buffer_rsrc_t rsW = __builtin_amdgcn_make_buffer_rsrc(const_cast<void*>(G.W), 0, bytesW, 0x00020000);
// ... 70 lines not shown
    auto iteration = [&](int j, f32x4 (&nxt_regs)[4], f32x4 (&wait_regs)[4]) {
        if (j + 1 < nt) convert_store(nxt_regs, (j + 1) & 1);
        issue_w(j + 3);
        issue_a(nxt_regs);
        compute(j);
        pe_wait<WAITN>(wait_regs);
        asm volatile("s_waitcnt lgkmcnt(0)" ::: "memory");
        __builtin_amdgcn_s_barrier();
        __builtin_amdgcn_sched_barrier(0);
    };
    for (int j = 0; j < nt; j += 3) {
        iteration(j, r1, r2);
        iteration(j + 1, r2, r0);
        iteration(j + 2, r0, r1);
    }
    pe_wait<0>(r0);
    pe_wait<0>(r1);
    pe_wait<0>(r2);
    __builtin_amdgcn_sched_barrier(0);

    float2* st = reinterpret_cast<float2*>(smem);
#pragma unroll
    for (int hrow = 0; hrow < 2; ++hrow) {
        float s = rs[hrow], q = rq[hrow];
#pragma unroll
        for (int off = 1; off < 8; off <<= 1) { s += __shfl_xor(s, off, 64); q += __shfl_xor(q, off, 64); }
        const float inv_k = 1.0f / (float)K;
        const float mean = s * inv_k;
        const float rstd = __builtin_amdgcn_rsqf(fmaxf(q * inv_k - mean * mean, 0.f) + a.eps);
        if (p == 0) st[wave * 16 + hrow * 8 + rr] = float2{mean, rstd};
    }
    __syncthreads();
    f32x4 s4[TN], t4[TN];
#pragma unroll
    for (int j = 0; j < TN; ++j) {
        const int n = min(n0 + wn * 16 * TN + j * 16 + g * 4, a.N - 4);
        s4[j] = *reinterpret_cast<const f32x4*>(G.s + n);
        t4[j] = *reinterpret_cast<const f32x4*>(G.t + n);
    }
#pragma unroll
    for (int i = 0; i < 2; ++i) {
        const int rl = wm * 32 + i * 16 + lr, m = m0 + rl;
        const float2 ms = st[rl];
#pragma unroll
        for (int j = 0; j < TN; ++j) {
            const int n = n0 + wn * 16 * TN + j * 16 + g * 4;
            if (m < G.rows && n < a.N) {
                f32x4 v;
#pragma unroll
                for (int r = 0; r < 4; ++r) v[r] = ms.y * (acc[i][j][r] - ms.x * s4[j][r]) + t4[j][r];
                store4(G.out + (size_t)m * a.ldo + n, v);
            }
        }
    }
}

__global__ __launch_bounds__(64 * PE_WAVES) __attribute__((amdgpu_waves_per_eu(4, 8)))
void patch_embed_kernel_n64(const PatchEmbedArgs a) {
    extern __shared__ __attribute__((aligned(16))) char smem[];
    patch_embed_body<2>(a, smem);
}
__global__ __launch_bounds__(64 * PE_WAVES) __attribute__((amdgpu_waves_per_eu(2, 8)))
void patch_embed_kernel_n128(const PatchEmbedArgs a) {
    extern __shared__ __attribute__((aligned(16))) char smem[];
    patch_embed_body<4>(a, smem);
}


constexpr int PW_BN = 512, PW_WSTAGE = PW_BN * 128, PW_KS = 1024, PW_SMEM = 2 * PE_ASTAGE + 2 * PW_WSTAGE;

struct PatchWideGroup {
    const void* W; int ldw, K;
    int f0, nt, pt, rows, mtiles, nslices;
    float* part;
    float* stats;
};
struct PatchWideArgs {
    const float* video;
    int B, C, F, H, W, ph, pw, nh, nw;
    int N;
    uint32_t video_bytes;
    int ngroups;
    int dbg;
    PatchWideGroup g[2];
};

__device__ __forceinline__ void patch_embed_wide_body(const PatchWideArgs& a, char* smem) {
    const int tid = threadIdx.x, lane = tid & 63;
    const int wave = __builtin_amdgcn_readfirstlane(tid >> 6);
    const int n0w = a.g[0].mtiles * a.g[0].nslices;
    const int nwork = n0w + (a.ngroups > 1 ? a.g[1].mtiles * a.g[1].nslices : 0);
    const int xcd = blockIdx.x & 7, idx = blockIdx.x >> 3;
    const int wstart = xcd * nwork / 8, wcount = (xcd + 1) * nwork / 8 - wstart;
    if (idx >= wcount) return;
    int w = wstart + idx;
    const int gi = (a.ngroups > 1 && w >= n0w) ? 1 : 0;
    if (gi) w -= n0w;
    const PatchWideGroup& G = a.g[gi];
    const int slice = w / G.mtiles, mt = w - slice * G.mtiles;
    const int m0 = mt * PE_BM;
    const int K = G.K, ntk = K >> 6;
    const int kt0 = slice * (PW_KS >> 6);
    const int nts = min(PW_KS >> 6, ntk - kt0);

    const int o = lane >> 3, p = lane & 7;
    const int rr = ((o & 1) << 2) | (o >> 1);
    const int pw = a.pw;
    const int dline = pw < 32 ? (p * 4) / pw : 0, xin = pw < 32 ? (p * 4) % pw : p * 4;
    const int per_b = G.nt * a.nh * a.nw;
    uint32_t rowoff[2];
    float cen[2];
#pragma unroll
    for (int hrow = 0; hrow < 2; ++hrow) {
        const int r = m0 + wave * 16 + hrow * 8 + rr;
        const bool ok = r < G.rows;
        const int rc = ok ? r : 0;
        const int b = rc / per_b, rem = rc - b * per_b;
        const int tt = rem / (a.nh * a.nw), hw = rem - tt * (a.nh * a.nw);
        const int hh = hw / a.nw, ww = hw - hh * a.nw;
        const uint32_t org = (((uint32_t)(b * a.C) * a.F + (G.f0 + tt * G.pt)) * a.H + hh * a.ph) * a.W + ww * a.pw;
        const f32x4 c4 = *reinterpret_cast<const f32x4*>(a.video + org + (uint32_t)dline * a.W + xin);
        float cs = (c4[0] + c4[1]) + (c4[2] + c4[3]);
#pragma unroll
        for (int off = 1; off < 8; off <<= 1) cs += __shfl_xor(cs, off, 64);
        cen[hrow] = ok ? cs * (1.0f / 32.0f) : 0.f;
        rowoff[hrow] = ok ? (org + (uint32_t)dline * a.W + xin) * 4u : a.video_bytes;
    }
    const uintptr_t vb = reinterpret_cast<uintptr_t>(a.video);
    const u32x4 rsrc = u32x4{(uint32_t)vb, (uint32_t)(vb >> 32) & 0xFFFFu, a.video_bytes, 0x00020000u};
    const int lph = pw < 32 ? 32 / pw : 1;
    int hx0, hy, hdt, hcc;
    {
        const int e0 = kt0 * 64, line0 = e0 / pw;
        hx0 = e0 - line0 * pw;
        hy = line0 % a.ph;
        const int r2 = line0 / a.ph;
        hdt = r2 % G.pt; hcc = r2 / G.pt;
    }
    auto next_soff = [&]() {
        const uint32_t so = ((((uint32_t)hcc * a.F + hdt) * a.H + hy) * a.W + hx0) * 4u;
        hx0 += 32;
        if (hx0 >= pw) {
            hx0 = 0; hy += lph;
            if (hy >= a.ph) { hy = 0; if (++hdt == G.pt) { hdt = 0; if (++hcc == a.C) hcc = 0; } }
        }
        return so;
    };
    auto issue_a = [&](f32x4 (&r)[4]) {
#pragma unroll
        for (int half = 0; half < 2; ++half) {
            const uint32_t so = next_soff();
            pe_load16(r[half * 2 + 0], rowoff[0], rsrc, so);
            pe_load16(r[half * 2 + 1], rowoff[1], rsrc, so);
        }
    };

    char* const wring = smem + 2 * PE_ASTAGE;
    const int lrow = lane >> 3, lslot = lane & 7;
    const uint32_t bytesW = (uint32_t)a.N * (uint32_t)G.ldw * 2u;
    __amdgpu_buffer_rsrc_t rsW = __builtin_amdgcn_make_buffer_rsrc(const_cast<void*>(G.W), 0, bytesW, 0x00020000);
    uint32_t offW[8];
#pragma unroll
    for (int i = 0; i < 8; ++i) {
        const int gn = (wave * 8 + i) * 8 + lrow;
        offW[i] = gn < a.N ? (uint32_t)gn * (uint32_t)G.ldw * 2u + (uint32_t)((lslot ^ (lrow & 7)) * 16) : bytesW;
    }
    int wk = kt0;
    auto issue_w = [&](int j) {
#pragma unroll
        for (int i = 0; i < 8; ++i)
            __builtin_amdgcn_raw_ptr_buffer_load_lds(rsW, (pe_lds_ptr)(wring + (j & 1) * PW_WSTAGE + (wave * 8 + i) * 1024), 16, offW[i], wk * 128, 0, 0);
        if (++wk == ntk) wk = 0;
    };

    float rs[2] = {0.f, 0.f}, rq[2] = {0.f, 0.f};
    auto convert_store = [&](const f32x4 (&r)[4], int stage) {
        char* at = smem + stage * PE_ASTAGE;
#pragma unroll
        for (int half = 0; half < 2; ++half)
#pragma unroll
            for (int hrow = 0; hrow < 2; ++hrow) {
                f32x4 x = r[half * 2 + hrow];
#pragma unroll
                for (int e = 0; e < 4; ++e) {
                    x[e] -= cen[hrow];
                    rs[hrow] += x[e];
                    rq[hrow] = fmaf(x[e], x[e], rq[hrow]);
                }
                const int row = wave * 16 + hrow * 8 + rr;
                const int slot = (half * 4 + (p >> 1)) ^ (row & 7);
                *reinterpret_cast<u32x2*>(at + row * 128 + (slot << 4) + ((p & 1) << 3)) = u32x2{pack_bf2(x[0], x[1]), pack_bf2(x[2], x[3])};
            }
    };

    const int g = lane >> 4, lr = lane & 15;
    const int wm = wave >> 2, wn = wave & 3;
    f32x4 acc[4][8];
#pragma unroll
    for (int i = 0; i < 4; ++i)
#pragma unroll
        for (int j = 0; j < 8; ++j) acc[i][j] = f32x4{0, 0, 0, 0};
    auto compute_half = [&](int j, int c) {
        const char* at = smem + (j & 1) * PE_ASTAGE;
        const char* wt = wring + (j & 1) * PW_WSTAGE;
        Frag<bf16> fa[4];
#pragma unroll
        for (int i = 0; i < 4; ++i) lds_frag(fa[i], at, wm * 64 + i * 16 + lr, c, g);
#pragma unroll
        for (int jj = 0; jj < 8; ++jj) {
            Frag<bf16> fw;
            lds_frag(fw, wt, wn * 128 + jj * 16 + lr, c, g);
#pragma unroll
            for (int i = 0; i < 4; ++i) acc[i][jj] = mma(fw, fa[i], acc[i][jj]);
        }
    };

    f32x4 r0[4], r1[4], r2[4];
    issue_a(r0);
    issue_w(0);
    issue_a(r1);
    issue_a(r2);
    pe_wait<8>(r0);
    __builtin_amdgcn_sched_barrier(0);
    convert_store(r0, 0);
    issue_a(r0);
    pe_wait<8>(r1);
    asm volatile("s_waitcnt lgkmcnt(0)" ::: "memory");
    __builtin_amdgcn_s_barrier();
    __builtin_amdgcn_sched_barrier(0);
    auto iteration = [&](int j, f32x4 (&nxt_regs)[4], f32x4 (&wait_regs)[4]) {
        if (j + 1 < nts && !(a.dbg & 4)) convert_store(nxt_regs, (j + 1) & 1);
        if (!(a.dbg & 2)) issue_w(j + 1);
        issue_a(nxt_regs);
        if (j < nts && !(a.dbg & 1)) { compute_half(j, 0); compute_half(j, 1); }
        pe_wait<4>(wait_regs);
        asm volatile("s_waitcnt lgkmcnt(0)" ::: "memory");
        __builtin_amdgcn_s_barrier();
        __builtin_amdgcn_sched_barrier(0);
    };
    for (int j = 0; j < nts; j += 3) {
        iteration(j, r1, r2);
        iteration(j + 1, r2, r0);
        iteration(j + 2, r0, r1);
    }
    pe_wait<0>(r0);
    pe_wait<0>(r1);
    pe_wait<0>(r2);
    __builtin_amdgcn_sched_barrier(0);

#pragma unroll
    for (int hrow = 0; hrow < 2; ++hrow) {
        float s = rs[hrow], q = rq[hrow];
#pragma unroll
        for (int off = 1; off < 8; off <<= 1) { s += __shfl_xor(s, off, 64); q += __shfl_xor(q, off, 64); }
        const int m = m0 + wave * 16 + hrow * 8 + rr;
        if (p == 0 && m < G.rows) reinterpret_cast<float2*>(G.stats)[(size_t)slice * G.rows + m] = float2{s, q};
    }
    float* part = G.part + (size_t)slice * G.rows * a.N;
#pragma unroll
    for (int i = 0; i < 4; ++i) {
        const int m = m0 + wm * 64 + i * 16 + lr;
        if (m >= G.rows) continue;
#pragma unroll
        for (int j = 0; j < 8; ++j) {
            const int n = wn * 128 + j * 16 + g * 4;
            if (n < a.N) store4(part + (size_t)m * a.N + n, acc[i][j]);
        }
    }
}

__global__ __launch_bounds__(64 * PE_WAVES) __attribute__((amdgpu_waves_per_eu(2, 2)))
void patch_embed_wide_kernel(const PatchWideArgs a) {
    extern __shared__ __attribute__((aligned(16))) char smem[];
    patch_embed_wide_body(a, smem);
}

struct PatchFinishArgs {
    const float* part; const float* stats; int nslices, rows, N, K;
    const float* s; const float* t; float eps1;
    const float* gamma2; const float* beta2; float eps2;
    float* out2; bf16* out; int ldo2, ldo;
    int remap_in, remap_out, remap_off;
};
__device__ __forceinline__ void patch_embed_finish_rows(const PatchFinishArgs& a, int block) {
    const int lane = threadIdx.x & 63;
    const int row = block * 4 + (threadIdx.x >> 6);
    if (row >= a.rows) return;
    float su = 0.f, sq = 0.f;
    for (int sl = 0; sl < a.nslices; ++sl) {
        const float2 st = reinterpret_cast<const float2*>(a.stats)[(size_t)sl * a.rows + row];
        su += st.x; sq += st.y;
    }
    const float inv_k = 1.0f / (float)a.K;
    const float mean = su * inv_k;
    const float rstd = 1.0f / sqrtf(fmaxf(sq * inv_k - mean * mean, 0.f) + a.eps1);
    f32x4 y[2];
    float ls = 0.f;
#pragma unroll
    for (int q = 0; q < 2; ++q) {
        const int n = lane * 4 + q * 256;
        y[q] = f32x4{0, 0, 0, 0};
        if (n < a.N) {
            f32x4 acc = f32x4{0, 0, 0, 0};
            for (int sl = 0; sl < a.nslices; ++sl) acc += *reinterpret_cast<const f32x4*>(a.part + ((size_t)sl * a.rows + row) * a.N + n);
            const f32x4 s4 = *reinterpret_cast<const f32x4*>(a.s + n), t4 = *reinterpret_cast<const f32x4*>(a.t + n);
#pragma unroll
            for (int r = 0; r < 4; ++r) { y[q][r] = rstd * (acc[r] - mean * s4[r]) + t4[r]; ls += y[q][r]; }
        }
    }
    const float m2 = wave_sum(ls) / (float)a.N;
    float lq = 0.f;
#pragma unroll
    for (int q = 0; q < 2; ++q)
        if (lane * 4 + q * 256 < a.N)
#pragma unroll
            for (int r = 0; r < 4; ++r) { const float d = y[q][r] - m2; lq = fmaf(d, d, lq); }
    const float r2 = 1.0f / sqrtf(wave_sum(lq) / (float)a.N + a.eps2);
    const int orow = a.remap_in > 0 ? (row / a.remap_in) * a.remap_out + a.remap_off + row % a.remap_in : row;
#pragma unroll
    for (int q = 0; q < 2; ++q) {
        const int n = lane * 4 + q * 256;
        if (n >= a.N) continue;
        const f32x4 g4 = *reinterpret_cast<const f32x4*>(a.gamma2 + n), b4 = *reinterpret_cast<const f32x4*>(a.beta2 + n);
        f32x4 v;
#pragma unroll
        for (int r = 0; r < 4; ++r) v[r] = (y[q][r] - m2) * r2 * g4[r] + b4[r];
        if (a.out2) store4(a.out2 + (size_t)orow * a.ldo2 + n, v);
        if (a.out) store4(a.out + (size_t)orow * a.ldo + n, v);
    }
}
__global__ __launch_bounds__(256) void patch_embed_finish_kernel(const PatchFinishArgs a) { patch_embed_finish_rows(a, blockIdx.x); }
struct PatchFinishPair { PatchFinishArgs g[2]; int blocks0; };
__global__ __launch_bounds__(256) void patch_embed_finish_pair_kernel(const PatchFinishPair p) {
    if ((int)blockIdx.x < p.blocks0) patch_embed_finish_rows(p.g[0], blockIdx.x);
    else patch_embed_finish_rows(p.g[1], blockIdx.x - p.blocks0);
}

}
using namespace pk;

extern "C" int pk_patch_embed(const float* video, int B, int C, int F, int H, int W, int ph, int pw, int N, float eps, int ngroups,
                              const void* W0, int ldw0, const float* s0, const float* t0, float* out0, int f00, int nt0, int pt0,
                              const void* W1, int ldw1, const float* s1, const float* t1, float* out1, int f01, int nt1, int pt1,
                              int ldo, void* stream) {
    if (!video || B <= 0 || C <= 0 || F <= 0 || H <= 0 || W <= 0 || ph <= 0 || pw <= 0 || N <= 0 || (ngroups != 1 && ngroups != 2)) return PK_EINVAL;
    if (H % ph || W % pw || (pw & (pw - 1)) || pw < 8 || pw > 128 || (W & 3) || (N & 3) || (ldo & 3)) return PK_EINVAL;
    if (pw < 32 && ph % (32 / pw)) return PK_EINVAL;
    const size_t vbytes = (size_t)B * C * F * H * W * 4;
    if (vbytes >= 0xFFFFFFF0ull) return PK_EINVAL;
    auto mis = [](const void* p) { return (reinterpret_cast<uintptr_t>(p) & 15) != 0; };
    PatchEmbedArgs a;
    a.video = video; a.B = B; a.C = C; a.F = F; a.H = H; a.W = W; a.ph = ph; a.pw = pw; a.nh = H / ph; a.nw = W / pw;
    a.N = N; a.ldo = ldo; a.eps = eps; a.video_bytes = (uint32_t)vbytes; a.ngroups = ngroups;
    static const int rot_env = [] { const char* e = getenv("PK_PATCH_ROT"); return e ? atoi(e) : 0; }();
    a.rot_mult = rot_env;
    const void* Ws[2] = {W0, W1}; const int ldws[2] = {ldw0, ldw1}; const float* ss[2] = {s0, s1}; const float* ts[2] = {t0, t1};
    float* outs[2] = {out0, out1}; const int f0s[2] = {f00, f01}, nts[2] = {nt0, nt1}, pts[2] = {pt0, pt1};
    int MT = 0;
    for (int gi = 0; gi < ngroups; ++gi) {
        PatchGroup& G = a.g[gi];
        if (!Ws[gi] || !ss[gi] || !ts[gi] || !outs[gi] || nts[gi] <= 0 || pts[gi] <= 0 || f0s[gi] < 0 || f0s[gi] + nts[gi] * pts[gi] > F) return PK_EINVAL;
        if (mis(video) || mis(Ws[gi]) || mis(ss[gi]) || mis(ts[gi]) || mis(outs[gi])) return PK_EALIGN;
        G.W = Ws[gi]; G.s = ss[gi]; G.t = ts[gi]; G.out = outs[gi]; G.ldw = ldws[gi];
        G.K = C * pts[gi] * ph * pw;
        if (G.K % 192 || G.ldw < G.K || (G.ldw & 7) || (size_t)N * G.ldw * 2 >= 0xFFFFFFF0ull) return PK_EINVAL;
        G.f0 = f0s[gi]; G.nt = nts[gi]; G.pt = pts[gi];
        G.rows = B * nts[gi] * a.nh * a.nw;
        G.mtiles = (G.rows + PE_BM - 1) / PE_BM;
        MT += G.mtiles;
    }
    if (ngroups == 1) a.g[1] = a.g[0];
    static const int tn_env = [] { const char* e = getenv("PK_PATCH_TN"); return e ? atoi(e) : 0; }();
    const bool wide = tn_env ? tn_env == 4 : N >= 128;
    hipStream_t st = reinterpret_cast<hipStream_t>(stream);
    if (wide) {
        static pk::LdsOptIn lds;
        if (lds.raise(reinterpret_cast<const void*>(&patch_embed_kernel_n128), PeGeom<4>::SMEM) != PK_OK) return PK_ELAUNCH;
        const int NT = (N + PeGeom<4>::BN - 1) / PeGeom<4>::BN;
        hipLaunchKernelGGL(patch_embed_kernel_n128, dim3(8 * ((MT + 7) / 8) * NT), dim3(64 * PE_WAVES), PeGeom<4>::SMEM, st, a);
    } else {
        const int NT = (N + PeGeom<2>::BN - 1) / PeGeom<2>::BN;
        hipLaunchKernelGGL(patch_embed_kernel_n64, dim3(8 * ((MT + 7) / 8) * NT), dim3(64 * PE_WAVES), PeGeom<2>::SMEM, st, a);
    }
    PK_CHECK_LAUNCH();
    return PK_OK;
}


extern "C" int pk_patch_embed_slices(int K) { return K <= 0 ? 0 : (K + PW_KS - 1) / PW_KS; }

extern "C" int pk_patch_embed_splitk(const float* video, int B, int C, int F, int H, int W, int ph, int pw, int N, int ngroups,
                                     const void* W0, int ldw0, float* part0, float* stats0, int f00, int nt0, int pt0,
                                     const void* W1, int ldw1, float* part1, float* stats1, int f01, int nt1, int pt1, void* stream) {
    if (!video || B <= 0 || C <= 0 || F <= 0 || H <= 0 || W <= 0 || ph <= 0 || pw <= 0 || N <= 0 || N > PW_BN || (ngroups != 1 && ngroups != 2)) return PK_EINVAL;
    if (H % ph || W % pw || (pw & (pw - 1)) || pw < 8 || pw > 128 || (W & 3) || (N & 3)) return PK_EINVAL;
    if (pw < 32 && ph % (32 / pw)) return PK_EINVAL;
    const size_t vbytes = (size_t)B * C * F * H * W * 4;
    if (vbytes >= 0xFFFFFFF0ull) return PK_EINVAL;
    auto mis = [](const void* p) { return (reinterpret_cast<uintptr_t>(p) & 15) != 0; };
    PatchWideArgs a;
    a.video = video; a.B = B; a.C = C; a.F = F; a.H = H; a.W = W; a.ph = ph; a.pw = pw; a.nh = H / ph; a.nw = W / pw;
    a.N = N; a.video_bytes = (uint32_t)vbytes; a.ngroups = ngroups;
    static const int dbg_env = [] { const char* e = getenv("PK_PATCH_DBG"); return e ? atoi(e) : 0; }();
    a.dbg = dbg_env;
    const void* Ws[2] = {W0, W1}; const int ldws[2] = {ldw0, ldw1}; float* parts[2] = {part0, part1}; float* stt[2] = {stats0, stats1};
    const int f0s[2] = {f00, f01}, nts[2] = {nt0, nt1}, pts[2] = {pt0, pt1};
    int work = 0;
    for (int gi = 0; gi < ngroups; ++gi) {
        PatchWideGroup& G = a.g[gi];
        if (!Ws[gi] || !parts[gi] || !stt[gi] || nts[gi] <= 0 || pts[gi] <= 0 || f0s[gi] < 0 || f0s[gi] + nts[gi] * pts[gi] > F) return PK_EINVAL;
        if (mis(video) || mis(Ws[gi]) || mis(parts[gi]) || (reinterpret_cast<uintptr_t>(stt[gi]) & 7)) return PK_EALIGN;
        G.W = Ws[gi]; G.ldw = ldws[gi]; G.part = parts[gi]; G.stats = stt[gi];
        G.K = C * pts[gi] * ph * pw;
        if (G.K % 64 || G.ldw < G.K || (G.ldw & 7) || (size_t)N * G.ldw * 2 >= 0xFFFFFFF0ull) return PK_EINVAL;
        G.f0 = f0s[gi]; G.nt = nts[gi]; G.pt = pts[gi];
        G.rows = B * nts[gi] * a.nh * a.nw;
        G.mtiles = (G.rows + PE_BM - 1) / PE_BM;
        G.nslices = (G.K + PW_KS - 1) / PW_KS;
        work += G.mtiles * G.nslices;
    }
    if (ngroups == 1) a.g[1] = a.g[0];
    static pk::LdsOptIn lds;
    if (lds.raise(reinterpret_cast<const void*>(&patch_embed_wide_kernel), PW_SMEM) != PK_OK) return PK_ELAUNCH;
    hipLaunchKernelGGL(patch_embed_wide_kernel, dim3(8 * ((work + 7) / 8)), dim3(64 * PE_WAVES), PW_SMEM, reinterpret_cast<hipStream_t>(stream), a);
    PK_CHECK_LAUNCH();
    return PK_OK;
}

extern "C" int pk_patch_embed_finish(const float* part, const float* stats, int nslices, int rows, int N, int K, const float* s, const float* t,
                                     float eps1, const float* gamma2, const float* beta2, float eps2, float* out2, int ldo2, void* out, int ldo,
                                     int remap_in, int remap_out, int remap_off, void* stream) {
    if (!part || !stats || !s || !t || !gamma2 || !beta2 || (!out2 && !out) || nslices <= 0 || rows <= 0 || N <= 0 || N > 512 || (N & 3) || K <= 0) return PK_EINVAL;
    auto mis = [](const void* p) { return (reinterpret_cast<uintptr_t>(p) & 15) != 0; };
    if (mis(part) || mis(s) || mis(t) || mis(gamma2) || mis(beta2) || (out2 && (mis(out2) || (ldo2 & 3))) || (out && ((reinterpret_cast<uintptr_t>(out) & 7) || (ldo & 3))) ||
        (reinterpret_cast<uintptr_t>(stats) & 7)) return PK_EALIGN;
    if (remap_in < 0 || (remap_in > 0 && (remap_out < remap_in || remap_off < 0))) return PK_EINVAL;
    PatchFinishArgs a{part, stats, nslices, rows, N, K, s, t, eps1, gamma2, beta2, eps2, out2, reinterpret_cast<bf16*>(out), ldo2, ldo, remap_in, remap_out, remap_off};
    hipLaunchKernelGGL(patch_embed_finish_kernel, dim3((rows + 3) / 4), dim3(256), 0, reinterpret_cast<hipStream_t>(stream), a);
    PK_CHECK_LAUNCH();
    return PK_OK;
}

extern "C" int pk_patch_embed_finish_groups(const pk_patch_finish_group* g, int ngroups, int N, float* out2, int ldo2, void* out, int ldo, void* stream) {
    if (!g || (ngroups != 1 && ngroups != 2) || (!out2 && !out) || N <= 0 || N > 512 || (N & 3)) return PK_EINVAL;
    auto mis = [](const void* p) { return (reinterpret_cast<uintptr_t>(p) & 15) != 0; };
    if ((out2 && (mis(out2) || (ldo2 & 3))) || (out && ((reinterpret_cast<uintptr_t>(out) & 7) || (ldo & 3)))) return PK_EALIGN;
    PatchFinishPair p;
    for (int i = 0; i < ngroups; ++i) {
        const pk_patch_finish_group& d = g[i];
        if (!d.part || !d.stats || !d.s || !d.t || !d.gamma2 || !d.beta2 || d.nslices <= 0 || d.rows <= 0 || d.K <= 0) return PK_EINVAL;
        if (mis(d.part) || mis(d.s) || mis(d.t) || mis(d.gamma2) || mis(d.beta2) || (reinterpret_cast<uintptr_t>(d.stats) & 7)) return PK_EALIGN;
        if (d.remap_in < 0 || (d.remap_in > 0 && (d.remap_out < d.remap_in || d.remap_off < 0))) return PK_EINVAL;
        p.g[i] = PatchFinishArgs{d.part, d.stats, d.nslices, d.rows, N, d.K, d.s, d.t, d.eps1, d.gamma2, d.beta2, d.eps2, out2, reinterpret_cast<bf16*>(out), ldo2, ldo,
                                 d.remap_in, d.remap_out, d.remap_off};
    }
    if (ngroups == 1) p.g[1] = p.g[0];
    p.blocks0 = (p.g[0].rows + 3) / 4;
    const int blocks = p.blocks0 + (ngroups == 2 ? (p.g[1].rows + 3) / 4 : 0);
    hipLaunchKernelGGL(patch_embed_finish_pair_kernel, dim3(blocks), dim3(256), 0, reinterpret_cast<hipStream_t>(stream), p);
    PK_CHECK_LAUNCH();
    return PK_OK;
}
```

### phenaki_pytorch_amd/csrc/qkv_attn.hip

```cpp
#include "gemm_dma.hpp"

namespace pk {

struct QkvAttnArgs {
    const void* xq; const void* xkv;
    const void* wq; const void* wkv;
    int ld, ldw;
    int S, n, h, K;
    int spt;
    const float* q_scale; const float* k_scale; float scale;
    const float* bias; long bias_hstride; int bias_ld;
    const float* slopes; int causal;
    void* O; int ldo;
    uint32_t recip;
    const float* q_ln_s;
};

template <typename T> using QaTile = GemmDma<T, 1, 4, 4, 1, 2, 128>;
template <typename T> using QaKvTile = GemmDma<T, 1, 8, 4, 1, 2, 128>;
constexpr int QA_SMEM = QaKvTile<bf16>::SMEM;
static_assert(QaKvTile<bf16x3>::SMEM == QA_SMEM, "the split-bf16 ring has the same bytes");

constexpr int QA_PLANE = 8192;
template <typename T> struct QaImg { static constexpr int PLANES = 1; };
template <> struct QaImg<bf16x3> { static constexpr int PLANES = 2; };
__device__ __forceinline__ void qa_put4(bf16, char* img, int off, f32x4 v) {
    *reinterpret_cast<u32x2*>(img + off) = u32x2{pack_bf2(v[0], v[1]), pack_bf2(v[2], v[3])};
}
__device__ __forceinline__ void qa_put4(bf16x3, char* img, int off, f32x4 v) {
    const uint32_t h0 = pack_bf2(v[0], v[1]), h1 = pack_bf2(v[2], v[3]);
    const float r0 = v[0] - __builtin_bit_cast(float, h0 << 16), r1 = v[1] - __builtin_bit_cast(float, h0 & 0xFFFF0000u);
    const float r2 = v[2] - __builtin_bit_cast(float, h1 << 16), r3 = v[3] - __builtin_bit_cast(float, h1 & 0xFFFF0000u);
    *reinterpret_cast<u32x2*>(img + off) = u32x2{h0, h1};
    *reinterpret_cast<u32x2*>(img + QA_PLANE + off) = u32x2{pack_bf2(r0, r1), pack_bf2(r2, r3)};
}
__device__ __forceinline__ void qa_put1(bf16, char* img, int off, float v) { *reinterpret_cast<u16*>(img + off) = f2bf(v); }
__device__ __forceinline__ void qa_put1(bf16x3, char* img, int off, float v) {
    const u16 h = f2bf(v);
    *reinterpret_cast<u16*>(img + off) = h;
    *reinterpret_cast<u16*>(img + QA_PLANE + off) = f2bf(v - bf2f(h));
}
__device__ __forceinline__ void qa_get(Frag<bf16>& f, const char* img, int off) { f.v = *reinterpret_cast<const u32x4*>(img + off); }
__device__ __forceinline__ void qa_get(Frag<bf16x3>& f, const char* img, int off) {
    f.hi = *reinterpret_cast<const u32x4*>(img + off);
    f.lo = *reinterpret_cast<const u32x4*>(img + QA_PLANE + off);
}

__device__ __forceinline__ int qa_kperm(int f, int i) { return (f >> 1) * 32 + (i >> 2) * 8 + (f & 1) * 4 + (i & 3); }
__device__ __forceinline__ int qa_ksw(int row) { return ((row >> 1) & 1) | (((row >> 3) & 3) << 1); }

template <typename T>
__device__ __forceinline__ void qa_project_q(const GemmOperands& p, int M, int m0, int hh, int K, const float* q_scale, float scale,
                                             const float* q_ln_s, char* smem, char* Qs) {
    const int lane = threadIdx.x & 63, g = lane >> 4, lr = lane & 15;
    const int rq = __builtin_amdgcn_readfirstlane(threadIdx.x >> 6) * 16 + lr;
    f32x4 acc[1][4];
#pragma unroll
    for (int j = 0; j < 4; ++j) acc[0][j] = f32x4{0, 0, 0, 0};
    if (q_ln_s) {
        float rsum[1], rsq[1];
        (void)QaTile<T>::template run_stats<1>(p, M, m0, hh * 64, smem, acc, rsum, rsq);
        const float mean = rsum[0] / (float)K;
#pragma unroll
        for (int j = 0; j < 4; ++j) {
            const f32x4 s4 = *reinterpret_cast<const f32x4*>(q_ln_s + hh * 64 + j * 16 + g * 4);
#pragma unroll
            for (int r = 0; r < 4; ++r) acc[0][j][r] -= mean * s4[r];
        }
    } else {
        (void)QaTile<T>::run(p, M, m0, hh * 64, smem, acc);
    }
    float ss = 0.f;
#pragma unroll
    for (int j = 0; j < 4; ++j)
#pragma unroll
        for (int r = 0; r < 4; ++r) ss += acc[0][j][r] * acc[0][j][r];
    ss += __shfl_xor(ss, 16, 64);
    ss += __shfl_xor(ss, 32, 64);
    const float inv = scale / fmaxf(sqrtf(ss), 1e-12f);
#pragma unroll
    for (int j = 0; j < 4; ++j) {
        const f32x4 sc = *reinterpret_cast<const f32x4*>(q_scale + j * 16 + g * 4);
        f32x4 v = acc[0][j];
#pragma unroll
        for (int r = 0; r < 4; ++r) v[r] *= inv * sc[r];
        const int slot = (2 * j + (g >> 1)) ^ (rq & 7);
        qa_put4(T{}, Qs, rq * 128 + (slot << 4) + (g & 1) * 8, v);
    }
}

template <typename T>
__global__ __launch_bounds__(256) void qkv_attn_kernel(const QkvAttnArgs a) {
    extern __shared__ __attribute__((aligned(16))) char smem[];
    constexpr int NPL = QaImg<T>::PLANES;
    char* Qs = smem;
    char* Ks = smem;
    char* Vts = smem + NPL * QA_PLANE;
    const int R = a.spt * a.n;
// ... 53 lines not shown
            for (int r = 0; r < 4; ++r) {
                const int d = j * 16 + g * 4 + r;
                qa_put1(T{}, Vts, d * 128 + ((((rq >> 3) ^ (d & 7))) << 4) + (rq & 7) * 2, acc[0][4 + j][r]);
            }
    }
    asm volatile("s_waitcnt lgkmcnt(0)" ::: "memory");
    __builtin_amdgcn_s_barrier();

    f32x4 st[4];
#pragma unroll
    for (int f = 0; f < 4; ++f) st[f] = f32x4{0, 0, 0, 0};
#pragma unroll
    for (int f = 0; f < 4; ++f) {
        const int krow = qa_kperm(f, lr);
#pragma unroll
        for (int c = 0; c < 2; ++c) {
            Frag<T> fk;
            qa_get(fk, Ks, krow * 128 + (((c * 4 + g) ^ qa_ksw(krow)) << 4));
            st[f] = mma(fk, fq[c], st[f]);
        }
    }
    const int seq_q = (int)(((uint32_t)rq * a.recip) >> 16), pos_q = rq - seq_q * a.n;
    const bool qvalid = rq < R && tile * a.spt + seq_q < a.S;
    const float slope = (a.causal && a.slopes) ? a.slopes[hh] : 0.f;
    const float* brow = a.bias ? a.bias + (size_t)hh * a.bias_hstride + (size_t)pos_q * a.bias_ld : nullptr;
    const bool whole = a.n == 64 && !a.causal;
    float pr[16];
    float mx = -INFINITY;
#pragma unroll
    for (int f = 0; f < 4; ++f) {
        const int k0 = qa_kperm(f, g * 4);
        f32x4 bz = f32x4{0, 0, 0, 0};
        if (whole && brow && (a.bias_ld & 3) == 0) bz = *reinterpret_cast<const f32x4*>(brow + k0);
#pragma unroll
        for (int r = 0; r < 4; ++r) {
            float sv = st[f][r];
            if (whole) {
                if (brow) sv += (a.bias_ld & 3) == 0 ? bz[r] : brow[k0 + r];
            } else {
                const int kk = k0 + r;
                const int seq_k = (int)(((uint32_t)kk * a.recip) >> 16), pos_k = kk - seq_k * a.n;
                if (kk >= R || seq_k != seq_q) sv = -INFINITY;
                else {
                    if (brow) sv += brow[pos_k];
                    if (a.causal) {
                        const int dj = pos_k - pos_q;
                        sv -= fabsf((float)dj) * slope;
                        if (dj > 0) sv = NEG_MAX;
                    }
                }
            }
            pr[f * 4 + r] = sv;
            mx = fmaxf(mx, sv);
        }
    }
    mx = fmaxf(mx, __shfl_xor(mx, 16, 64));
    mx = fmaxf(mx, __shfl_xor(mx, 32, 64));
    if (!qvalid) mx = 0.f;
    float ls = 0.f;
#pragma unroll
    for (int e = 0; e < 16; ++e) { pr[e] = __expf(pr[e] - mx); ls += pr[e]; }
    ls += __shfl_xor(ls, 16, 64);
    ls += __shfl_xor(ls, 32, 64);
    f32x4 o[4];
#pragma unroll
    for (int df = 0; df < 4; ++df) o[df] = f32x4{0, 0, 0, 0};
#pragma unroll
    for (int kc = 0; kc < 2; ++kc) {
        Frag<T> fp;
        {
            const float p8[8] = {pr[kc * 8 + 0], pr[kc * 8 + 1], pr[kc * 8 + 2], pr[kc * 8 + 3], pr[kc * 8 + 4], pr[kc * 8 + 5], pr[kc * 8 + 6], pr[kc * 8 + 7]};
            frag_from_f32(fp, p8);
        }
#pragma unroll
        for (int df = 0; df < 4; ++df) {
            const int d = df * 16 + lr;
            Frag<T> fv;
            qa_get(fv, Vts, d * 128 + (((kc * 4 + g) ^ (d & 7)) << 4));
            o[df] = mma(fv, fp, o[df]);
        }
    }
    if (!qvalid) return;
    const float inv = 1.0f / ls;
    T* orow = reinterpret_cast<T*>(a.O) + (size_t)(m0 + rq) * a.ldo + hh * 64;
#pragma unroll
    for (int df = 0; df < 4; ++df) store4(orow + df * 16 + g * 4, o[df] * inv);
}

struct QAttnCachedArgs {
    const void* xq; const void* wq; int ld, ldw;
    int S, n, h, K;
    const float* q_scale; float scale; const float* q_ln_s;
    const void* Kp; const void* Vt; int nk_pad, nk, nnull;
    const unsigned char* kmask; int n_kv;
    void* O; int ldo;
};

template <typename T, bool NK64>
__global__ __launch_bounds__(256) void q_attn_cached_kernel(const QAttnCachedArgs a) {
    extern __shared__ __attribute__((aligned(16))) char smem[];
    constexpr int NPL = QaImg<T>::PLANES;
    char* Qs = smem + QaTile<T>::SMEM;
    char* Ks = Qs + NPL * QA_PLANE;
    char* Vts = smem;
    const int M = a.S * a.n;
    const int tiles = M / 64;
    const int xcd = blockIdx.x & 7, idx = blockIdx.x >> 3;
    const int tile = (idx / a.h) * 8 + xcd, hh = idx % a.h;
    if (tile >= tiles) return;
    const int m0 = tile * 64;
    const int s = m0 / a.n;
    const int lane = threadIdx.x & 63, g = lane >> 4, lr = lane & 15;
    const int wave = __builtin_amdgcn_readfirstlane(threadIdx.x >> 6);
    const int rq = wave * 16 + lr;

    GemmOperands p;
    p.a_rows = nullptr;
    p.lda = a.ld; p.ldw = a.ldw;
    p.M = M; p.K = a.K;
    p.plain_map = 0; p.krot = 0;
    p.w_gap_from = 0; p.w_gap_rows = 0;
    p.A = a.xq; p.W = a.wq; p.N = a.h * 64;
    qa_project_q<T>(p, M, m0, hh, a.K, a.q_scale, a.scale, a.q_ln_s, smem, Qs);

    {
        const size_t sh = (size_t)s * a.h + hh;
        const int row = threadIdx.x >> 2, part = threadIdx.x & 3;
        const u32x4 zero = u32x4{0, 0, 0, 0};
        if constexpr (NPL == 1) {
            const bf16* krow = reinterpret_cast<const bf16*>(a.Kp) + (sh * a.nk_pad + row) * 64;
            const bf16* vrow = reinterpret_cast<const bf16*>(a.Vt) + (sh * 64 + row) * a.nk_pad;
#pragma unroll
            for (int q = 0; q < 2; ++q) {
                const int slot = part * 2 + q;
                const u32x4 kv = row < a.nk_pad ? *reinterpret_cast<const u32x4*>(krow + slot * 8) : zero;
                *reinterpret_cast<u32x4*>(Ks + row * 128 + ((slot ^ qa_ksw(row)) << 4)) = kv;
                const u32x4 vv = slot * 8 < a.nk_pad ? *reinterpret_cast<const u32x4*>(vrow + slot * 8) : zero;
                *reinterpret_cast<u32x4*>(Vts + row * 128 + ((slot ^ (row & 7)) << 4)) = vv;
            }
        } else {
            const char* krow = reinterpret_cast<const char*>(a.Kp) + (sh * a.nk_pad + row) * 256;
            const char* vrow = reinterpret_cast<const char*>(a.Vt) + (sh * 64 + row) * (size_t)a.nk_pad * 4;
            u32x4 kv[4], vv[4];
#pragma unroll
            for (int q = 0; q < 4; ++q) {
                const int sp = part * 4 + q;
                kv[q] = row < a.nk_pad ? *reinterpret_cast<const u32x4*>(krow + sp * 16) : zero;
                vv[q] = (sp >> 3) * 32 < a.nk_pad ? *reinterpret_cast<const u32x4*>(vrow + sp * 16) : zero;
            }
#pragma unroll
            for (int q = 0; q < 4; ++q) {
                const int sp = part * 4 + q;
                const int plane = (sp >> 2) & 1, slot = (sp >> 3) * 4 + (sp & 3);
                *reinterpret_cast<u32x4*>(Ks + plane * QA_PLANE + row * 128 + ((slot ^ qa_ksw(row)) << 4)) = kv[q];
                *reinterpret_cast<u32x4*>(Vts + plane * QA_PLANE + row * 128 + ((slot ^ (row & 7)) << 4)) = vv[q];
            }
        }
    }
    asm volatile("s_waitcnt lgkmcnt(0)" ::: "memory");
    __builtin_amdgcn_s_barrier();

    constexpr int NF = NK64 ? 4 : 2;
    Frag<T> fq[2];
#pragma unroll
    for (int c = 0; c < 2; ++c) qa_get(fq[c], Qs, rq * 128 + (((c * 4 + g) ^ (rq & 7)) << 4));
    f32x4 st[NF];
#pragma unroll
    for (int f = 0; f < NF; ++f) {
        st[f] = f32x4{0, 0, 0, 0};
        const int krow = qa_kperm(f, lr);
#pragma unroll
        for (int c = 0; c < 2; ++c) {
            Frag<T> fk;
            qa_get(fk, Ks, krow * 128 + (((c * 4 + g) ^ qa_ksw(krow)) << 4));
            st[f] = mma(fk, fq[c], st[f]);
        }
    }
    const unsigned char* km = a.kmask ? a.kmask + (size_t)s * a.n_kv : nullptr;
    float pr[4 * NF];
    float mx = -INFINITY;
#pragma unroll
    for (int f = 0; f < NF; ++f)
#pragma unroll
        for (int r = 0; r < 4; ++r) {
            const int kk = qa_kperm(f, g * 4 + r);
            float sv = st[f][r];
            if (kk >= a.nk) sv = -INFINITY;
            else if (km && kk >= a.nnull && !km[kk - a.nnull]) sv = NEG_MAX;
            pr[f * 4 + r] = sv;
            mx = fmaxf(mx, sv);
        }
    mx = fmaxf(mx, __shfl_xor(mx, 16, 64));
    mx = fmaxf(mx, __shfl_xor(mx, 32, 64));
    float ls = 0.f;
#pragma unroll
    for (int e = 0; e < 4 * NF; ++e) { pr[e] = __expf(pr[e] - mx); ls += pr[e]; }
    ls += __shfl_xor(ls, 16, 64);
    ls += __shfl_xor(ls, 32, 64);
    f32x4 o[4];
#pragma unroll
    for (int df = 0; df < 4; ++df) o[df] = f32x4{0, 0, 0, 0};
#pragma unroll
    for (int kc = 0; kc < NF / 2; ++kc) {
        Frag<T> fp;
        {
            const float p8[8] = {pr[kc * 8 + 0], pr[kc * 8 + 1], pr[kc * 8 + 2], pr[kc * 8 + 3], pr[kc * 8 + 4], pr[kc * 8 + 5], pr[kc * 8 + 6], pr[kc * 8 + 7]};
            frag_from_f32(fp, p8);
        }
#pragma unroll
        for (int df = 0; df < 4; ++df) {
            const int d = df * 16 + lr;
            Frag<T> fv;
            qa_get(fv, Vts, d * 128 + (((kc * 4 + g) ^ (d & 7)) << 4));
            o[df] = mma(fv, fp, o[df]);
        }
    }
    const float inv = 1.0f / ls;
    T* orow = reinterpret_cast<T*>(a.O) + (size_t)(m0 + rq) * a.ldo + hh * 64;
#pragma unroll
    for (int df = 0; df < 4; ++df) store4(orow + df * 16 + g * 4, o[df] * inv);
}

}
using namespace pk;

extern "C" int pk_qkv_attn(int dtype, const void* xq, const void* xkv, int ld, const void* wq, const void* wkv, int ldw, int S, int n, int h,
                           int K, const float* q_scale, const float* k_scale, float scale, const float* bias, long bias_hstride,
                           int bias_ld, const float* slopes, int causal, void* O, int ldo, const float* q_ln_s, void* stream) {
    if (dtype != 1 && dtype != 2) return PK_EINVAL;
    if (!xq || !xkv || !wq || !wkv || !q_scale || !k_scale || !O || S <= 0 || n <= 0 || n > 64 || h <= 0 || K <= 0) return PK_EINVAL;
    auto mis = [](const void* ptr) { return (reinterpret_cast<uintptr_t>(ptr) & 15) != 0; };
    const int q = dtype == 1 ? 7 : 3, bk = dtype == 1 ? 64 : 32, esz = dtype == 1 ? 2 : 4;
    if ((K & q) || (ld & q) || (ldw & q) || (ldo & 3) || mis(xq) || mis(xkv) || mis(wq) || mis(wkv) || mis(q_scale) || mis(k_scale) ||
        (reinterpret_cast<uintptr_t>(O) & (dtype == 1 ? 7 : 15)) || (bias && mis(bias))) return PK_EALIGN;
    if (ldw < (K + bk - 1) / bk * bk) return PK_EINVAL;
    const long M = (long)S * n;
    if ((size_t)M * ld * esz >= 0xFFFFFFF0ull || (size_t)2 * h * 64 * ldw * esz >= 0xFFFFFFF0ull) return PK_EINVAL;
    QkvAttnArgs a;
    a.xq = xq; a.xkv = xkv; a.wq = wq; a.wkv = wkv; a.ld = ld; a.ldw = ldw;
    a.S = S; a.n = n; a.h = h; a.K = K; a.spt = 64 / n;
    a.q_scale = q_scale; a.k_scale = k_scale; a.scale = scale;
    a.bias = bias; a.bias_hstride = bias_hstride; a.bias_ld = bias_ld;
    a.slopes = slopes; a.causal = causal;
    a.O = O; a.ldo = ldo;
    a.recip = (65536u + (uint32_t)n - 1u) / (uint32_t)n;
    a.q_ln_s = q_ln_s;
    if (q_ln_s && mis(q_ln_s)) return PK_EALIGN;
    const int tiles = (S + a.spt - 1) / a.spt;
    dim3 grid(8 * ((tiles + 7) / 8) * h);
    hipStream_t st = reinterpret_cast<hipStream_t>(stream);
    if (dtype == 1) hipLaunchKernelGGL(qkv_attn_kernel<bf16>, grid, dim3(256), QA_SMEM, st, a);
    else hipLaunchKernelGGL(qkv_attn_kernel<bf16x3>, grid, dim3(256), QA_SMEM, st, a);
    PK_CHECK_LAUNCH();
    return PK_OK;
}

extern "C" int pk_q_attn_cached(int dtype, const void* xq, int ld, const void* wq, int ldw, int S, int n, int h, int K, const float* q_scale,
                                float scale, const float* q_ln_s, const void* Kp, const void* Vt, int nk_pad, int n_kv, int nnull,
                                const unsigned char* kmask, void* O, int ldo, void* stream) {
    if (dtype != 1 && dtype != 2) return PK_EINVAL;
    if (!xq || !wq || !q_scale || !Kp || !Vt || !O || S <= 0 || n <= 0 || (n & 63) || h <= 0 || K <= 0 || n_kv <= 0 || nnull < 0) return PK_EINVAL;
    const int nk = nnull + n_kv;
    if (nk > 64 || nk_pad < nk || nk_pad > 64 || (nk_pad & 31)) return PK_EINVAL;
    auto mis = [](const void* ptr) { return (reinterpret_cast<uintptr_t>(ptr) & 15) != 0; };
    const int q = dtype == 1 ? 7 : 3, bk = dtype == 1 ? 64 : 32, esz = dtype == 1 ? 2 : 4;
    if ((K & q) || (ld & q) || (ldw & q) || (ldo & 3) || mis(xq) || mis(wq) || mis(q_scale) || mis(Kp) || mis(Vt) ||
        (reinterpret_cast<uintptr_t>(O) & (dtype == 1 ? 7 : 15)) || (q_ln_s && mis(q_ln_s))) return PK_EALIGN;
    if (dtype == 2 && ((reinterpret_cast<uintptr_t>(Kp) | reinterpret_cast<uintptr_t>(Vt)) & 127)) return PK_EALIGN;
    if (ldw < (K + bk - 1) / bk * bk) return PK_EINVAL;
    const long M = (long)S * n;
    if ((size_t)M * ld * esz >= 0xFFFFFFF0ull || (size_t)h * 64 * ldw * esz >= 0xFFFFFFF0ull) return PK_EINVAL;
    QAttnCachedArgs a{xq, wq, ld, ldw, S, n, h, K, q_scale, scale, q_ln_s, Kp, Vt, nk_pad, nk, nnull, kmask, n_kv, O, ldo};
    const int tiles = (int)(M / 64);
    dim3 grid(8 * ((tiles + 7) / 8) * h);
    hipStream_t st = reinterpret_cast<hipStream_t>(stream);
    if (dtype == 1) {
        constexpr int lds = QaTile<bf16>::SMEM + 2 * QA_PLANE;
        if (nk_pad > 32) hipLaunchKernelGGL((q_attn_cached_kernel<bf16, true>), grid, dim3(256), lds, st, a);
        else hipLaunchKernelGGL((q_attn_cached_kernel<bf16, false>), grid, dim3(256), lds, st, a);
    } else {
        constexpr int lds = QaTile<bf16x3>::SMEM + 4 * QA_PLANE;
        if (nk_pad > 32) hipLaunchKernelGGL((q_attn_cached_kernel<bf16x3, true>), grid, dim3(256), lds, st, a);
        else hipLaunchKernelGGL((q_attn_cached_kernel<bf16x3, false>), grid, dim3(256), lds, st, a);
    }
    PK_CHECK_LAUNCH();
    return PK_OK;
}
```

Baseline: 169,000 frames/s.

## Add per-site cache-policy stores/loads with nontemporal video loads by default

Adds a runtime-configurable cache policy mask (env var or API) that selects plain, write-through (buffer store with cache bits) or nontemporal stores and loads at several kernel sites: GEMM epilogue, attention output, PEG, patch-embed partials and finish, and residual loads. The default enables only nontemporal loads of the input video in the patch-embed kernel, which streams the large video once and should pollute the cache less. It also drops an unconditional s_waitcnt at the end of the GEMM epilogue outside timeline builds. Every kernel gains template branches on a runtime policy, which adds code size and complexity.

New measurement: 174,400 frames/s, median of 6. 1.03x the previous value.

```diff
diff --git a/include/phenaki_hip.h b/include/phenaki_hip.h
--- a/include/phenaki_hip.h
+++ b/include/phenaki_hip.h
@@ -266,6 +266,9 @@
                   long long nparts, float* ssim, void* stream);
 int pk_code_usage(const int* counts, int V, double* out, void* stream);
 
+int pk_set_cache_policy(unsigned mask);
+int pk_get_cache_policy();
+
 #ifdef __cplusplus
 }
 #endif
diff --git a/phenaki_pytorch_amd/_lib.py b/phenaki_pytorch_amd/_lib.py
--- a/phenaki_pytorch_amd/_lib.py
+++ b/phenaki_pytorch_amd/_lib.py
@@ -138,11 +138,14 @@
     'pk_frame_sqerr': [_P, _P, _I, _I, _I, _I, _I, _F, _F, _P, _LL, _P, _P, _P],
     'pk_frame_ssim': [_P, _P, _I, _I, _I, _I, _I, _F, _F, _P, _LL, _P, _P],
     'pk_code_usage': [_P, _I, _P, _P],
+    'pk_set_cache_policy': [ctypes.c_uint],
+    'pk_get_cache_policy': [],
 }
 
 _ERR = {-1: 'PK_EINVAL (bad shape/size/flag)', -2: 'PK_EALIGN (pointer/stride alignment)', -3: 'PK_ELAUNCH (HIP launch failed)'}
 
 _lib = None
+_AB_OPTIONAL = ('pk_set_cache_policy', 'pk_get_cache_policy')
 
 
 def load():
@@ -153,6 +156,8 @@
                                '(the MI355X build has no CPU / eager fallback)')
         lib = ctypes.CDLL(LIB_PATH)
         for name, args in SIGNATURES.items():
+            if name in _AB_OPTIONAL and 'PK_LIB_PATH' in os.environ and not hasattr(lib, name):
+                continue
             fn = getattr(lib, name)
             fn.argtypes = args
             fn.restype = _I
@@ -215,6 +220,27 @@
     img = torch.cat((hi.view(n, k // 32, 32), lo.view(n, k // 32, 32)), dim=-1).contiguous()
     return img.view(n, 2 * k).view(torch.float32)
 
+
+
+CP_PLAIN, CP_WT, CP_NT = 0, 1, 2
+CP_STORE_SITES = ('gemm', 'qkv_attn', 'peg', 'ln', 'patch_wide', 'patch_finish')
+CP_LOAD_SITES = ('ld_video', 'ld_partials', 'ld_residual')
+CP_SITES = CP_STORE_SITES + CP_LOAD_SITES
+
+
+def cache_policy_mask(**sites):
+    mask = 0
+    for name, pol in sites.items():
+        mask |= int(pol) << (2 * CP_SITES.index(name))
+    return mask
+
+
+def set_cache_policy(mask):
+    _check(load().pk_set_cache_policy(int(mask)), 'pk_set_cache_policy')
+
+
+def get_cache_policy():
+    return load().pk_get_cache_policy()
 
 
 def gemm(dtype, A, W, M, N, K, *, C, bias=None, res=None, act=ACT_NONE, a_rows=None, lda=None, ldc=None, variant=0, C2=None, ln=None,
diff --git a/phenaki_pytorch_amd/csrc/common.hpp b/phenaki_pytorch_amd/csrc/common.hpp
--- a/phenaki_pytorch_amd/csrc/common.hpp
+++ b/phenaki_pytorch_amd/csrc/common.hpp
@@ -143,6 +143,67 @@
 __device__ __forceinline__ void store2(float* p, float a, float b) { *reinterpret_cast<f32x2*>(p) = f32x2{a, b}; }
 __device__ __forceinline__ void store2(bf16* p, float a, float b) { *reinterpret_cast<uint32_t*>(p) = pack_bf2(a, b); }
 
+enum { CP_PLAIN = 0, CP_WT = 1, CP_NT = 2 };
+enum {
+    CPS_GEMM = 0,
+    CPS_QKV_ATTN = 1,
+    CPS_PEG = 2,
+    CPS_LN = 3,
+    CPS_PATCH_WIDE = 4,
+    CPS_PATCH_FINISH = 5,
+    CPS_LD_VIDEO = 6,
+    CPS_LD_PART = 7,
+    CPS_LD_RES = 8,
+    CPS_COUNT = 9
+};
+unsigned cache_policy_mask();
+inline int cache_policy(int site) { return (int)((cache_policy_mask() >> (2 * site)) & 3u); }
+inline int cache_policy_for(int site, size_t bytes) {
+    const int pol = cache_policy(site);
+    return (pol == CP_WT && bytes >= 0xFFFFFFF0ull) ? CP_PLAIN : pol;
+}
+
+struct CpOn { static constexpr bool on = true; };
+struct CpOff { static constexpr bool on = false; };
+template <typename C> __device__ __forceinline__ int cp_pick(C, int pol) { return C::on ? pol : (int)CP_PLAIN; }
+
+typedef uint32_t u32x4_gcc __attribute__((__vector_size__(16)));
+struct PolOut { __amdgpu_buffer_rsrc_t rs; int pol; };
+__device__ __forceinline__ PolOut pol_out(void* base, int pol) {
+    return PolOut{__builtin_amdgcn_make_buffer_rsrc(base, 0, (int)0xFFFFFFFFu, 0x00020000), pol};
+}
+__device__ __forceinline__ void pol_store16(const PolOut& po, void* base, size_t boff, u32x4 v) {
+    if (po.pol == CP_WT) __builtin_amdgcn_raw_buffer_store_b128(__builtin_bit_cast(u32x4_gcc, v), po.rs, (int)(uint32_t)boff, 0, 16);
+    else if (po.pol == CP_NT) __builtin_nontemporal_store(v, reinterpret_cast<u32x4*>(reinterpret_cast<char*>(base) + boff));
+    else *reinterpret_cast<u32x4*>(reinterpret_cast<char*>(base) + boff) = v;
+}
+__device__ __forceinline__ void pol_store8(int pol, void* p, u32x2 v) {
+    if (pol == CP_WT) __hip_atomic_store(reinterpret_cast<unsigned long long*>(p), __builtin_bit_cast(unsigned long long, v), __ATOMIC_RELAXED, __HIP_MEMORY_SCOPE_AGENT);
+    else if (pol == CP_NT) __builtin_nontemporal_store(v, reinterpret_cast<u32x2*>(p));
+    else *reinterpret_cast<u32x2*>(p) = v;
+}
+__device__ __forceinline__ void pol_store4(int pol, void* p, uint32_t v) {
+    if (pol == CP_WT) __hip_atomic_store(reinterpret_cast<uint32_t*>(p), v, __ATOMIC_RELAXED, __HIP_MEMORY_SCOPE_AGENT);
+    else if (pol == CP_NT) __builtin_nontemporal_store(v, reinterpret_cast<uint32_t*>(p));
+    else *reinterpret_cast<uint32_t*>(p) = v;
+}
+__device__ __forceinline__ void store4(const PolOut& po, float* base, size_t o, f32x4 v) { pol_store16(po, base, o * 4, __builtin_bit_cast(u32x4, v)); }
+__device__ __forceinline__ void store4(const PolOut& po, bf16x3* base, size_t o, f32x4 v) { pol_store16(po, base, o * 4, __builtin_bit_cast(u32x4, v)); }
+__device__ __forceinline__ void store4(int pol, bf16* base, size_t o, f32x4 v) {
+    pol_store8(pol, base + o, u32x2{pack_bf2(v[0], v[1]), pack_bf2(v[2], v[3])});
+}
+__device__ __forceinline__ void store2(int pol, float* base, size_t o, float a, float b) {
+    pol_store8(pol, base + o, u32x2{__builtin_bit_cast(uint32_t, a), __builtin_bit_cast(uint32_t, b)});
+}
+__device__ __forceinline__ void store2(int pol, bf16x3* base, size_t o, float a, float b) { store2(pol, reinterpret_cast<float*>(base), o, a, b); }
+__device__ __forceinline__ void store2(int pol, bf16* base, size_t o, float a, float b) { pol_store4(pol, base + o, pack_bf2(a, b)); }
+__device__ __forceinline__ void store4(const PolOut& po, bf16* base, size_t o, f32x4 v) { store4(po.pol, base, o, v); }
+template <typename T> __device__ __forceinline__ void store2(const PolOut& po, T* base, size_t o, float a, float b) { store2(po.pol, base, o, a, b); }
+__device__ __forceinline__ f32x4 pol_load16(int pol, const float* p) {
+    if (pol == CP_NT) return __builtin_nontemporal_load(reinterpret_cast<const f32x4*>(p));
+    return *reinterpret_cast<const f32x4*>(p);
+}
+
 __device__ __forceinline__ long xcd_contiguous_block(unsigned b, unsigned nblocks_padded) {
     return (long)(b & 7u) * (nblocks_padded >> 3) + (b >> 3);
 }
diff --git a/phenaki_pytorch_amd/csrc/elementwise.hip b/phenaki_pytorch_amd/csrc/elementwise.hip
--- a/phenaki_pytorch_amd/csrc/elementwise.hip
+++ b/phenaki_pytorch_amd/csrc/elementwise.hip
@@ -42,7 +42,7 @@
 template <int WW>
 __global__ __launch_bounds__(256) void peg_row_kernel(const float* __restrict__ x, const float* __restrict__ wt,
                                                       const float* __restrict__ bias, float* __restrict__ out, bf16* __restrict__ out_t,
-                                                      int B, int T, int H, int D, int tfront, long total, int flip = 0) {
+                                                      int B, int T, int H, int D, int tfront, long total, int flip = 0, int pol = CP_PLAIN) {
     const int dv = D >> 2;
     const long idx = xcd_contiguous_block(blockIdx.x, gridDim.x) * 256 + threadIdx.x;
     if (idx >= total) return;
@@ -80,12 +80,16 @@
         }
     }
     const size_t o0 = (((size_t)b * T + t) * H + h) * WW * D + c;
-#pragma unroll
-    for (int w = 0; w < WW; ++w) *reinterpret_cast<f32x4*>(out + o0 + (size_t)w * D) = acc[w];
-    if (out_t) {
-#pragma unroll
-        for (int w = 0; w < WW; ++w) store4(out_t + o0 + (size_t)w * D, acc[w]);
-    }
+    auto emit = [&](auto polc) {
+        const PolOut po = pol_out(out, cp_pick(polc, pol));
+#pragma unroll
+        for (int w = 0; w < WW; ++w) store4(po, out, o0 + (size_t)w * D, acc[w]);
+        if (out_t) {
+#pragma unroll
+            for (int w = 0; w < WW; ++w) store4(po, out_t, o0 + (size_t)w * D, acc[w]);
+        }
+    };
+    if (pol) emit(CpOn{}); else emit(CpOff{});
 }
 
 template <int CD>
@@ -267,8 +271,34 @@
     }
 }
 
+constexpr unsigned CACHE_POLICY_DEFAULT = (unsigned)CP_NT << (2 * CPS_LD_VIDEO);
+static bool cache_policy_ok(unsigned mask) {
+    if (mask >> (2 * CPS_COUNT)) return false;
+    for (int s = 0; s < CPS_COUNT; ++s) {
+        const unsigned pol = (mask >> (2 * s)) & 3u;
+        if (pol == 3u || (s >= CPS_LD_VIDEO && pol == CP_WT)) return false;
+    }
+    return true;
+}
+static unsigned& cache_policy_word() {
+    static unsigned mask = [] {
+        const char* e = getenv("PK_CACHE_POLICY");
+        const unsigned m = e ? (unsigned)strtoul(e, nullptr, 0) : CACHE_POLICY_DEFAULT;
+        return cache_policy_ok(m) ? m : CACHE_POLICY_DEFAULT;
+    }();
+    return mask;
+}
+unsigned cache_policy_mask() { return cache_policy_word(); }
+
 }
 using namespace pk;
+
+extern "C" int pk_set_cache_policy(unsigned mask) {
+    if (!cache_policy_ok(mask)) return PK_EINVAL;
+    cache_policy_word() = mask;
+    return PK_OK;
+}
+extern "C" int pk_get_cache_policy() { return (int)cache_policy_word(); }
 
 static inline int nblocks(long total) { long b = (total + 255) / 256; return (int)(b < 16384 ? (b > 0 ? b : 1) : 16384); }
 #define STREAM(s) reinterpret_cast<hipStream_t>(s)
@@ -283,9 +313,10 @@
     const dim3 rgrid(xcd_padded_grid((rows + 255) / 256));
     bf16* ot = reinterpret_cast<bf16*>(out_t);
     if (ot && (reinterpret_cast<uintptr_t>(ot) & 7)) return PK_EALIGN;
-    if (W == 8) hipLaunchKernelGGL((peg_row_kernel<8>), rgrid, dim3(256), 0, STREAM(stream), x, wt, bias, out, ot, B, T, H, D, causal ? 2 : 1, rows);
-    else if (W == 4) hipLaunchKernelGGL((peg_row_kernel<4>), rgrid, dim3(256), 0, STREAM(stream), x, wt, bias, out, ot, B, T, H, D, causal ? 2 : 1, rows);
-    else if (W == 16) hipLaunchKernelGGL((peg_row_kernel<16>), rgrid, dim3(256), 0, STREAM(stream), x, wt, bias, out, ot, B, T, H, D, causal ? 2 : 1, rows);
+    const int pol = cache_policy_for(CPS_PEG, (size_t)total * 16);
+    if (W == 8) hipLaunchKernelGGL((peg_row_kernel<8>), rgrid, dim3(256), 0, STREAM(stream), x, wt, bias, out, ot, B, T, H, D, causal ? 2 : 1, rows, 0, pol);
+    else if (W == 4) hipLaunchKernelGGL((peg_row_kernel<4>), rgrid, dim3(256), 0, STREAM(stream), x, wt, bias, out, ot, B, T, H, D, causal ? 2 : 1, rows, 0, pol);
+    else if (W == 16) hipLaunchKernelGGL((peg_row_kernel<16>), rgrid, dim3(256), 0, STREAM(stream), x, wt, bias, out, ot, B, T, H, D, causal ? 2 : 1, rows, 0, pol);
     else hipLaunchKernelGGL(peg_kernel, dim3(nblocks(total)), dim3(256), 0, STREAM(stream), x, wt, bias, out, ot, B, T, H, W, D, causal ? 2 : 1, total);
     PK_CHECK_LAUNCH();
     return PK_OK;
diff --git a/phenaki_pytorch_amd/csrc/gemm.hip b/phenaki_pytorch_amd/csrc/gemm.hip
--- a/phenaki_pytorch_amd/csrc/gemm.hip
+++ b/phenaki_pytorch_amd/csrc/gemm.hip
@@ -19,6 +19,7 @@
     const int* row_off; const int* col_off;
     float* stats_out; const float* ln_stats; int stats_np;
     int dup_rows;
+    int pol, pol_res;
 };
 
 constexpr int STATS_CHUNK = 32;
@@ -62,18 +63,17 @@
 
 template <int TM> constexpr int epi_rows_per_round() { return TM > 2 ? 2 : TM; }
 
-template <typename T, int TM, int TN, int WN = 2, bool LNF = false>
-__device__ __forceinline__ void gemm_epilogue(const f32x4 (&acc)[TM][TN], int M, int N, const GemmEpilogue& e, int m0, int n0,
-                                              const float* rsum = nullptr, const float* rsq = nullptr, int K = 1) {
-    if (!e.vec_ok) {
-        if (!LNF) gemm_epilogue_scalar<T, TM, TN, WN>(acc, M, N, e, m0, n0);
-        return;
-    }
+template <typename T, int TM, int TN, int WN, bool LNF, typename POLC>
+__device__ __forceinline__ void gemm_epilogue_vec(const f32x4 (&acc)[TM][TN], int M, int N, const GemmEpilogue& e, int m0, int n0,
+                                                  const float* rsum, const float* rsq, int K) {
+    const int e_pol = cp_pick(POLC{}, e.pol), e_pol_res = cp_pick(POLC{}, e.pol_res);
     const int lane = threadIdx.x & 63, wave = threadIdx.x >> 6;
     const int wm = wave / WN, wn = wave % WN, g = lane >> 4, lr = lane & 15;
     float* __restrict__ Cf = reinterpret_cast<float*>(e.C);
     T* __restrict__ Ct = reinterpret_cast<T*>(e.C);
     const int mb = m0 + wm * 16 * TM + lr, nb = n0 + wn * 16 * TN + g * 4;
+    const PolOut po = pol_out(e.C, e_pol);
+    bf16* const C2 = reinterpret_cast<bf16*>(e.C2);
     f32x4 b4[TN], s4[TN], t4[TN];
     int coff[TN];
 #pragma unroll
@@ -97,7 +97,7 @@
             roff[ii] = e.row_off ? e.row_off[mi] : 0;
             if (!LNF && e.res && e.act != ACT_GEGLU) {
 #pragma unroll
-                for (int j = 0; j < TN; ++j) r4[ii][j] = *reinterpret_cast<const f32x4*>(e.res + (size_t)mi * e.ldr + min(nb + j * 16, N - 4));
+                for (int j = 0; j < TN; ++j) r4[ii][j] = pol_load16(e_pol_res, e.res + (size_t)mi * e.ldr + min(nb + j * 16, N - 4));
             } else {
 #pragma unroll
                 for (int j = 0; j < TN; ++j) r4[ii][j] = f32x4{0, 0, 0, 0};
@@ -126,7 +126,7 @@
                 if (e.act == ACT_GEGLU) {
                     const float o0 = gelu_for<T>(v[1]) * v[0], o1 = gelu_for<T>(v[3]) * v[2];
                     const size_t o = (size_t)m * e.ldc + (n >> 1);
-                    if (live) { if (e.out_f32) store2(Cf + o, o0, o1); else store2(Ct + o, o0, o1); }
+                    if (live) { if (e.out_f32) store2(po, Cf, o, o0, o1); else store2(po, Ct, o, o0, o1); }
                     continue;
                 }
                 if (e.act == ACT_LEAKY) {
@@ -138,15 +138,16 @@
                     for (int r = 0; r < 4; ++r) v[r] = fmaxf(v[r], 0.f);
                 }
                 if (!LNF) v += r4[ii][j];
-                else if (e.res && live) v += *reinterpret_cast<const f32x4*>(e.res + (size_t)m * e.ldr + n);
+                else if (e.res && live) v += pol_load16(e_pol_res, e.res + (size_t)m * e.ldr + n);
                 if (live) {
                     const size_t o = e.row_off ? (size_t)((long)roff[ii] + (long)coff[j]) : (size_t)m * e.ldc + n;
-                    if (e.out_f32) store4(Cf + o, v); else store4(Ct + o, v);
-                    if (e.C2) store4(reinterpret_cast<bf16*>(e.C2) + (size_t)m * e.ldc2 + n, v);
+                    if (POLC::on && e.row_off && o >= ((size_t)1 << 30)) store4(Cf + o, v);
+                    else if (e.out_f32) store4(po, Cf, o, v); else store4(po, Ct, o, v);
+                    if (e.C2) store4(e_pol, C2, (size_t)m * e.ldc2 + n, v);
                     if (e.dup_rows) {
                         const size_t od = o + (size_t)e.dup_rows * e.ldc;
-                        if (e.out_f32) store4(Cf + od, v); else store4(Ct + od, v);
-                        if (e.C2) store4(reinterpret_cast<bf16*>(e.C2) + (size_t)(m + e.dup_rows) * e.ldc2 + n, v);
+                        if (e.out_f32) store4(po, Cf, od, v); else store4(po, Ct, od, v);
+                        if (e.C2) store4(e_pol, C2, (size_t)(m + e.dup_rows) * e.ldc2 + n, v);
                     }
                     if (TN == 2 && e.stats_out) {
 #pragma unroll
@@ -162,10 +163,21 @@
                 ps += __shfl_xor(ps, 32); pq += __shfl_xor(pq, 32);
                 const int chunk = (n0 + wn * 16 * TN) / STATS_CHUNK;
                 if (g == 0 && m < M && chunk < e.stats_np)
-                    reinterpret_cast<float2*>(e.stats_out)[(size_t)m * e.stats_np + chunk] = float2{ps, pq};
+                    store2(e_pol, e.stats_out, ((size_t)m * e.stats_np + chunk) * 2, ps, pq);
             }
         }
     }
+}
+
+template <typename T, int TM, int TN, int WN = 2, bool LNF = false>
+__device__ __forceinline__ void gemm_epilogue(const f32x4 (&acc)[TM][TN], int M, int N, const GemmEpilogue& e, int m0, int n0,
+                                              const float* rsum = nullptr, const float* rsq = nullptr, int K = 1) {
+    if (!e.vec_ok) {
+        if (!LNF) gemm_epilogue_scalar<T, TM, TN, WN>(acc, M, N, e, m0, n0);
+        return;
+    }
+    if (e.pol | e.pol_res) gemm_epilogue_vec<T, TM, TN, WN, LNF, CpOn>(acc, M, N, e, m0, n0, rsum, rsq, K);
+    else gemm_epilogue_vec<T, TM, TN, WN, LNF, CpOff>(acc, M, N, e, m0, n0, rsum, rsq, K);
 }
 
 template <typename T, typename TA, int TM, int TN>
@@ -248,7 +260,9 @@
         if (!Tile::run(p, a_nrows, m0, n0, smem, acc)) return;
         PK_TL_KERNEL(1);
         gemm_epilogue<T, TM, TN, WN>(acc, p.M, p.N, e, m0, n0);
+#ifdef PK_TIMELINE
         asm volatile("s_waitcnt vmcnt(0)" ::: "memory");
+#endif
         PK_TL_KERNEL(2);
     }
 }
@@ -451,6 +465,8 @@
     bool v = (N % 4 == 0) && (ldc % 4 == 0) && al16(C) && (!bias || al16(bias)) && (!res || (al16(res) && ldr % 4 == 0));
     if (act == ACT_GEGLU) v = v && (ldc % 2 == 0) && ((reinterpret_cast<uintptr_t>(C) & 7) == 0);
     e.vec_ok = v ? 1 : 0;
+    e.pol = cache_policy_for(CPS_GEMM, row_off ? 0 : ((size_t)(M - 1 + dup_rows) * ldc + N) * (size_t)(out_is_f32 || dtype != 1 ? 4 : 2));
+    e.pol_res = cache_policy(CPS_LD_RES);
     if (C2 && (!v || !out_is_f32 || act == ACT_GEGLU || dtype != 1 || (ldc2 & 3) || (reinterpret_cast<uintptr_t>(C2) & 7))) return PK_EINVAL;
     if ((ln_s == nullptr) != (ln_t == nullptr)) return PK_EINVAL;
     if ((row_off == nullptr) != (col_off == nullptr)) return PK_EINVAL;
diff --git a/phenaki_pytorch_amd/csrc/norm.hip b/phenaki_pytorch_amd/csrc/norm.hip
--- a/phenaki_pytorch_amd/csrc/norm.hip
+++ b/phenaki_pytorch_amd/csrc/norm.hip
@@ -11,6 +11,7 @@
     int M, D;
     int grp, gstride, goff;
     int pb, pc;
+    int pol;
 };
 
 template <typename TO, int VMAX>
@@ -57,24 +58,29 @@
         }
     }
     const float rstd = 1.0f / sqrtf(wave_sum(q) / (float)p.D + p.eps);
-#pragma unroll
-    for (int i = 0; i < VMAX; ++i) {
-        const int c = lane + i * 64;
-        if (c < nv) {
-            f32x4 g4, b4;
-            if constexpr (HOIST) { g4 = gm[i]; b4 = bt[i]; }
-            else {
-                g4 = *reinterpret_cast<const f32x4*>(p.gamma + c * 4);
-                b4 = p.beta ? *reinterpret_cast<const f32x4*>(p.beta + c * 4) : f32x4{0, 0, 0, 0};
-            }
-            f32x4 y;
-#pragma unroll
-            for (int r = 0; r < 4; ++r) y[r] = (v[i][r] - mean) * rstd * g4[r] + b4[r];
-            if (out) store4(out + (size_t)orow * p.ldo + c * 4, y);
-            if (p.out2) store4(p.out2 + (size_t)orow * p.ldo2 + c * 4, y);
-            if (raw) store4(raw + (size_t)orow * p.ldraw + c * 4, v[i]);
-        }
-    }
+    auto emit = [&](auto polc) {
+        const int pol = cp_pick(polc, p.pol);
+        const PolOut po = pol_out(p.out, pol), po2 = pol_out(p.out2, pol), por = pol_out(p.raw, pol);
+#pragma unroll
+        for (int i = 0; i < VMAX; ++i) {
+            const int c = lane + i * 64;
+            if (c < nv) {
+                f32x4 g4, b4;
+                if constexpr (HOIST) { g4 = gm[i]; b4 = bt[i]; }
+                else {
+                    g4 = *reinterpret_cast<const f32x4*>(p.gamma + c * 4);
+                    b4 = p.beta ? *reinterpret_cast<const f32x4*>(p.beta + c * 4) : f32x4{0, 0, 0, 0};
+                }
+                f32x4 y;
+#pragma unroll
+                for (int r = 0; r < 4; ++r) y[r] = (v[i][r] - mean) * rstd * g4[r] + b4[r];
+                if (out) store4(po, out, (size_t)orow * p.ldo + c * 4, y);
+                if (p.out2) store4(po2, p.out2, (size_t)orow * p.ldo2 + c * 4, y);
+                if (raw) store4(por, raw, (size_t)orow * p.ldraw + c * 4, v[i]);
+            }
+        }
+    };
+    if (p.pol) emit(CpOn{}); else emit(CpOff{});
 }
 
 template <int VMAX, int R>
@@ -84,6 +90,7 @@
     const int row0 = (blockIdx.x * 4 + (threadIdx.x >> 6)) * R;
     if (row0 >= p.M) return;
     const int nv = p.D >> 2;
+    const PolOut po2 = pol_out(p.out2, p.pol);
     f32x4 y[R][VMAX];
     float mean[R], rstd[R];
 #pragma unroll
@@ -156,7 +163,7 @@
         if (p.out2) {
 #pragma unroll
             for (int i = 0; i < VMAX; ++i)
-                if (lane + i * 64 < nv) store4(p.out2 + (size_t)orow * p.ldo2 + (lane + i * 64) * 4, y[r][i]);
+                if (lane + i * 64 < nv) store4(po2, p.out2, (size_t)orow * p.ldo2 + (lane + i * 64) * 4, y[r][i]);
         }
         float h8[8], h4[4], h2[2], h1;
         {
@@ -192,12 +199,12 @@
         h1 += __shfl_xor(h1, 1, 64);
         const int k = lane >> 2;
         const float val = h1 + (k < cd ? bp[k] : 0.f);
-        if (proj && k < cd && (lane & 3) == 0) proj[(size_t)orow * cd + k] = val;
+        if (proj && k < cd && (lane & 3) == 0) pol_store4(p.pol, proj + (size_t)orow * cd + k, __builtin_bit_cast(uint32_t, val));
         const unsigned long long bal = __ballot(val > 0.f);
         if (lane == 0) {
             long long id = 0;
             for (int kk = 0; kk < cd; ++kk) id |= (long long)((bal >> (4 * kk)) & 1ull) << (cd - 1 - kk);
-            ids[orow] = id;
+            pol_store8(p.pol, ids + orow, __builtin_bit_cast(u32x2, id));
         }
     }
 }
@@ -277,7 +284,8 @@
     if ((D & 3) || (ldx & 3) || (tokens && (ldt & 3))) return PK_EALIGN;
     if (D > 64 * 4 * 8) return PK_EINVAL;
     if (pb > 0 && (pc <= 0 || M % (pb * pc))) return PK_EINVAL;
-    LnArgs p{x, ldx, gamma, beta, eps, nullptr, 0, tokens, ldt, nullptr, 0, M, D, 0, 0, 0, pb, pc};
+    LnArgs p{x, ldx, gamma, beta, eps, nullptr, 0, tokens, ldt, nullptr, 0, M, D, 0, 0, 0, pb, pc,
+             cache_policy_for(CPS_LN, tokens ? (size_t)M * ldt * 4 : 0)};
     hipStream_t s = reinterpret_cast<hipStream_t>(stream);
     dim3 block(256);
     if (D <= 64 * 4 * 2 && M >= 32768) hipLaunchKernelGGL((ln_lfq_kernel<2, 2>), dim3((M + 7) / 8), block, 0, s, p, wp, bp, cd, ids, proj);
@@ -295,7 +303,11 @@
     if (D > 64 * 4 * 8) return PK_EINVAL;
     if (pb > 0 && (pc <= 0 || M % (pb * pc))) return PK_EINVAL;
     if (grp > 0 && pb > 0) return PK_EINVAL;
-    LnArgs p{x, ldx, gamma, beta, eps, out, ldo, out2, ldo2, raw, ldraw, M, D, grp, gstride, goff, pb, pc};
+    const size_t orows = grp > 0 ? (size_t)((M - 1) / grp) * gstride + goff + grp : (size_t)M;
+    size_t ldmax = out ? ldo : 0;
+    if (out2 && (size_t)ldo2 > ldmax) ldmax = ldo2;
+    if (raw && (size_t)ldraw > ldmax) ldmax = ldraw;
+    LnArgs p{x, ldx, gamma, beta, eps, out, ldo, out2, ldo2, raw, ldraw, M, D, grp, gstride, goff, pb, pc, cache_policy_for(CPS_LN, orows * ldmax * 4)};
     hipStream_t s = reinterpret_cast<hipStream_t>(stream);
     dim3 grid((M + 3) / 4), block(256);
     const bool small = D <= 64 * 4 * 2;
diff --git a/phenaki_pytorch_amd/csrc/patch_embed.hip b/phenaki_pytorch_amd/csrc/patch_embed.hip
--- a/phenaki_pytorch_amd/csrc/patch_embed.hip
+++ b/phenaki_pytorch_amd/csrc/patch_embed.hip
@@ -43,6 +43,9 @@
 
 __device__ __forceinline__ void pe_load16(f32x4& dst, uint32_t voff, const u32x4& rsrc, uint32_t soff) {
     asm volatile("buffer_load_dwordx4 %0, %1, %2, %3 offen" : "=v"(dst) : "v"(voff), "s"(rsrc), "s"(soff) : "memory");
+}
+__device__ __forceinline__ void pe_load16_nt(f32x4& dst, uint32_t voff, const u32x4& rsrc, uint32_t soff) {
+    asm volatile("buffer_load_dwordx4 %0, %1, %2, %3 offen nt" : "=v"(dst) : "v"(voff), "s"(rsrc), "s"(soff) : "memory");
 }
 template <int N>
 __device__ __forceinline__ void pe_wait(f32x4 (&r)[4]) {
@@ -279,9 +282,11 @@
     uint32_t video_bytes;
     int ngroups;
     int dbg;
+    int pol;
     PatchWideGroup g[2];
 };
 
+template <bool NTV>
 __device__ __forceinline__ void patch_embed_wide_body(const PatchWideArgs& a, char* smem) {
     const int tid = threadIdx.x, lane = tid & 63;
     const int wave = __builtin_amdgcn_readfirstlane(tid >> 6);
@@ -347,8 +352,13 @@
 #pragma unroll
         for (int half = 0; half < 2; ++half) {
             const uint32_t so = next_soff();
-            pe_load16(r[half * 2 + 0], rowoff[0], rsrc, so);
-            pe_load16(r[half * 2 + 1], rowoff[1], rsrc, so);
+            if constexpr (NTV) {
+                pe_load16_nt(r[half * 2 + 0], rowoff[0], rsrc, so);
+                pe_load16_nt(r[half * 2 + 1], rowoff[1], rsrc, so);
+            } else {
+                pe_load16(r[half * 2 + 0], rowoff[0], rsrc, so);
+                pe_load16(r[half * 2 + 1], rowoff[1], rsrc, so);
+            }
         }
     };
 
@@ -451,25 +461,34 @@
 #pragma unroll
         for (int off = 1; off < 8; off <<= 1) { s += __shfl_xor(s, off, 64); q += __shfl_xor(q, off, 64); }
         const int m = m0 + wave * 16 + hrow * 8 + rr;
-        if (p == 0 && m < G.rows) reinterpret_cast<float2*>(G.stats)[(size_t)slice * G.rows + m] = float2{s, q};
+        if (p == 0 && m < G.rows) store2(a.pol, G.stats, ((size_t)slice * G.rows + m) * 2, s, q);
     }
     float* part = G.part + (size_t)slice * G.rows * a.N;
-#pragma unroll
-    for (int i = 0; i < 4; ++i) {
-        const int m = m0 + wm * 64 + i * 16 + lr;
-        if (m >= G.rows) continue;
-#pragma unroll
-        for (int j = 0; j < 8; ++j) {
-            const int n = wn * 128 + j * 16 + g * 4;
-            if (n < a.N) store4(part + (size_t)m * a.N + n, acc[i][j]);
-        }
-    }
+    auto emit = [&](auto polc) {
+        const PolOut po = pol_out(part, cp_pick(polc, a.pol));
+#pragma unroll
+        for (int i = 0; i < 4; ++i) {
+            const int m = m0 + wm * 64 + i * 16 + lr;
+            if (m >= G.rows) continue;
+#pragma unroll
+            for (int j = 0; j < 8; ++j) {
+                const int n = wn * 128 + j * 16 + g * 4;
+                if (n < a.N) store4(po, part, (size_t)m * a.N + n, acc[i][j]);
+            }
+        }
+    };
+    if (a.pol) emit(CpOn{}); else emit(CpOff{});
 }
 
 __global__ __launch_bounds__(64 * PE_WAVES) __attribute__((amdgpu_waves_per_eu(2, 2)))
 void patch_embed_wide_kernel(const PatchWideArgs a) {
     extern __shared__ __attribute__((aligned(16))) char smem[];
-    patch_embed_wide_body(a, smem);
+    patch_embed_wide_body<false>(a, smem);
+}
+__global__ __launch_bounds__(64 * PE_WAVES) __attribute__((amdgpu_waves_per_eu(2, 2)))
+void patch_embed_wide_nt_kernel(const PatchWideArgs a) {
+    extern __shared__ __attribute__((aligned(16))) char smem[];
+    patch_embed_wide_body<true>(a, smem);
 }
 
 struct PatchFinishArgs {
@@ -478,6 +497,7 @@
     const float* gamma2; const float* beta2; float eps2;
     float* out2; bf16* out; int ldo2, ldo;
     int remap_in, remap_out, remap_off;
+    int pol_st, pol_ld;
 };
 __device__ __forceinline__ void patch_embed_finish_rows(const PatchFinishArgs& a, int block) {
     const int lane = threadIdx.x & 63;
@@ -499,7 +519,7 @@
         y[q] = f32x4{0, 0, 0, 0};
         if (n < a.N) {
             f32x4 acc = f32x4{0, 0, 0, 0};
-            for (int sl = 0; sl < a.nslices; ++sl) acc += *reinterpret_cast<const f32x4*>(a.part + ((size_t)sl * a.rows + row) * a.N + n);
+            for (int sl = 0; sl < a.nslices; ++sl) acc += pol_load16(a.pol_ld, a.part + ((size_t)sl * a.rows + row) * a.N + n);
             const f32x4 s4 = *reinterpret_cast<const f32x4*>(a.s + n), t4 = *reinterpret_cast<const f32x4*>(a.t + n);
 #pragma unroll
             for (int r = 0; r < 4; ++r) { y[q][r] = rstd * (acc[r] - mean * s4[r]) + t4[r]; ls += y[q][r]; }
@@ -514,6 +534,7 @@
             for (int r = 0; r < 4; ++r) { const float d = y[q][r] - m2; lq = fmaf(d, d, lq); }
     const float r2 = 1.0f / sqrtf(wave_sum(lq) / (float)a.N + a.eps2);
     const int orow = a.remap_in > 0 ? (row / a.remap_in) * a.remap_out + a.remap_off + row % a.remap_in : row;
+    const PolOut po2 = pol_out(a.out2, a.pol_st);
 #pragma unroll
     for (int q = 0; q < 2; ++q) {
         const int n = lane * 4 + q * 256;
@@ -522,8 +543,8 @@
         f32x4 v;
 #pragma unroll
         for (int r = 0; r < 4; ++r) v[r] = (y[q][r] - m2) * r2 * g4[r] + b4[r];
-        if (a.out2) store4(a.out2 + (size_t)orow * a.ldo2 + n, v);
-        if (a.out) store4(a.out + (size_t)orow * a.ldo + n, v);
+        if (a.out2) store4(po2, a.out2, (size_t)orow * a.ldo2 + n, v);
+        if (a.out) store4(a.pol_st, a.out, (size_t)orow * a.ldo + n, v);
     }
 }
 __global__ __launch_bounds__(256) void patch_embed_finish_kernel(const PatchFinishArgs a) { patch_embed_finish_rows(a, blockIdx.x); }
@@ -600,6 +621,7 @@
     a.N = N; a.video_bytes = (uint32_t)vbytes; a.ngroups = ngroups;
     static const int dbg_env = [] { const char* e = getenv("PK_PATCH_DBG"); return e ? atoi(e) : 0; }();
     a.dbg = dbg_env;
+    a.pol = cache_policy(CPS_PATCH_WIDE);
     const void* Ws[2] = {W0, W1}; const int ldws[2] = {ldw0, ldw1}; float* parts[2] = {part0, part1}; float* stt[2] = {stats0, stats1};
     const int f0s[2] = {f00, f01}, nts[2] = {nt0, nt1}, pts[2] = {pt0, pt1};
     int work = 0;
@@ -614,12 +636,18 @@
         G.rows = B * nts[gi] * a.nh * a.nw;
         G.mtiles = (G.rows + PE_BM - 1) / PE_BM;
         G.nslices = (G.K + PW_KS - 1) / PW_KS;
+        if ((size_t)G.rows * N * 4 >= 0xFFFFFFF0ull && a.pol == CP_WT) a.pol = CP_PLAIN;
         work += G.mtiles * G.nslices;
     }
     if (ngroups == 1) a.g[1] = a.g[0];
-    static pk::LdsOptIn lds;
-    if (lds.raise(reinterpret_cast<const void*>(&patch_embed_wide_kernel), PW_SMEM) != PK_OK) return PK_ELAUNCH;
-    hipLaunchKernelGGL(patch_embed_wide_kernel, dim3(8 * ((work + 7) / 8)), dim3(64 * PE_WAVES), PW_SMEM, reinterpret_cast<hipStream_t>(stream), a);
+    static pk::LdsOptIn lds, lds_nt;
+    if (cache_policy(CPS_LD_VIDEO) == CP_NT) {
+        if (lds_nt.raise(reinterpret_cast<const void*>(&patch_embed_wide_nt_kernel), PW_SMEM) != PK_OK) return PK_ELAUNCH;
+        hipLaunchKernelGGL(patch_embed_wide_nt_kernel, dim3(8 * ((work + 7) / 8)), dim3(64 * PE_WAVES), PW_SMEM, reinterpret_cast<hipStream_t>(stream), a);
+    } else {
+        if (lds.raise(reinterpret_cast<const void*>(&patch_embed_wide_kernel), PW_SMEM) != PK_OK) return PK_ELAUNCH;
+        hipLaunchKernelGGL(patch_embed_wide_kernel, dim3(8 * ((work + 7) / 8)), dim3(64 * PE_WAVES), PW_SMEM, reinterpret_cast<hipStream_t>(stream), a);
+    }
     PK_CHECK_LAUNCH();
     return PK_OK;
 }
@@ -632,7 +660,9 @@
     if (mis(part) || mis(s) || mis(t) || mis(gamma2) || mis(beta2) || (out2 && (mis(out2) || (ldo2 & 3))) || (out && ((reinterpret_cast<uintptr_t>(out) & 7) || (ldo & 3))) ||
         (reinterpret_cast<uintptr_t>(stats) & 7)) return PK_EALIGN;
     if (remap_in < 0 || (remap_in > 0 && (remap_out < remap_in || remap_off < 0))) return PK_EINVAL;
-    PatchFinishArgs a{part, stats, nslices, rows, N, K, s, t, eps1, gamma2, beta2, eps2, out2, reinterpret_cast<bf16*>(out), ldo2, ldo, remap_in, remap_out, remap_off};
+    const size_t orows = remap_in > 0 ? (size_t)((rows - 1) / remap_in) * remap_out + remap_off + remap_in : (size_t)rows;
+    PatchFinishArgs a{part, stats, nslices, rows, N, K, s, t, eps1, gamma2, beta2, eps2, out2, reinterpret_cast<bf16*>(out), ldo2, ldo, remap_in, remap_out, remap_off,
+                      cache_policy_for(CPS_PATCH_FINISH, out2 ? orows * ldo2 * 4 : 0), cache_policy(CPS_LD_PART)};
     hipLaunchKernelGGL(patch_embed_finish_kernel, dim3((rows + 3) / 4), dim3(256), 0, reinterpret_cast<hipStream_t>(stream), a);
     PK_CHECK_LAUNCH();
     return PK_OK;
@@ -649,7 +679,9 @@
         if (mis(d.part) || mis(d.s) || mis(d.t) || mis(d.gamma2) || mis(d.beta2) || (reinterpret_cast<uintptr_t>(d.stats) & 7)) return PK_EALIGN;
         if (d.remap_in < 0 || (d.remap_in > 0 && (d.remap_out < d.remap_in || d.remap_off < 0))) return PK_EINVAL;
         p.g[i] = PatchFinishArgs{d.part, d.stats, d.nslices, d.rows, N, d.K, d.s, d.t, d.eps1, d.gamma2, d.beta2, d.eps2, out2, reinterpret_cast<bf16*>(out), ldo2, ldo,
-                                 d.remap_in, d.remap_out, d.remap_off};
+                                 d.remap_in, d.remap_out, d.remap_off,
+                                 cache_policy_for(CPS_PATCH_FINISH, out2 ? ((d.remap_in > 0 ? (size_t)((d.rows - 1) / d.remap_in) * d.remap_out + d.remap_off + d.remap_in : (size_t)d.rows) * ldo2 * 4) : 0),
+                                 cache_policy(CPS_LD_PART)};
     }
     if (ngroups == 1) p.g[1] = p.g[0];
     p.blocks0 = (p.g[0].rows + 3) / 4;
diff --git a/phenaki_pytorch_amd/csrc/qkv_attn.hip b/phenaki_pytorch_amd/csrc/qkv_attn.hip
--- a/phenaki_pytorch_amd/csrc/qkv_attn.hip
+++ b/phenaki_pytorch_amd/csrc/qkv_attn.hip
@@ -14,6 +14,7 @@
     void* O; int ldo;
     uint32_t recip;
     const float* q_ln_s;
+    int pol;
 };
 
 template <typename T> using QaTile = GemmDma<T, 1, 4, 4, 1, 2, 128>;
@@ -233,9 +234,13 @@
     }
     if (!qvalid) return;
     const float inv = 1.0f / ls;
-    T* orow = reinterpret_cast<T*>(a.O) + (size_t)(m0 + rq) * a.ldo + hh * 64;
-#pragma unroll
-    for (int df = 0; df < 4; ++df) store4(orow + df * 16 + g * 4, o[df] * inv);
+    const size_t orow = (size_t)(m0 + rq) * a.ldo + hh * 64;
+    auto emit = [&](auto polc) {
+        const PolOut po = pol_out(a.O, cp_pick(polc, a.pol));
+#pragma unroll
+        for (int df = 0; df < 4; ++df) store4(po, reinterpret_cast<T*>(a.O), orow + df * 16 + g * 4, o[df] * inv);
+    };
+    if (a.pol) emit(CpOn{}); else emit(CpOff{});
 }
 
 struct QAttnCachedArgs {
@@ -396,6 +401,7 @@
     a.O = O; a.ldo = ldo;
     a.recip = (65536u + (uint32_t)n - 1u) / (uint32_t)n;
     a.q_ln_s = q_ln_s;
+    a.pol = cache_policy_for(CPS_QKV_ATTN, (size_t)M * ldo * esz);
     if (q_ln_s && mis(q_ln_s)) return PK_EALIGN;
     const int tiles = (S + a.spt - 1) / a.spt;
     dim3 grid(8 * ((tiles + 7) / 8) * h);
```
